# JeffWang987/MVSTER

Hardware: AMD Instinct MI355X
Metric: depth-maps/sec (DTU 512×640, 5-view, 4-stage) at 1/2/4/8 MI355X (higher is better)
Workload: dtype f32; 1 GPU; DTU mid 512x640, 5 views, 4-stage cascade 8/8/4/4 hyp, B=1 eval, 1 depth map(s) per step per GPU; launch=hipGraph replay, parallelism=replicas x1, depth_maps_in_flight_per_gpu=2

## Files before the change

include/mvster_hip.h:

```cpp
#ifndef MVSTER_HIP_H
#define MVSTER_HIP_H

#ifdef __cplusplus
extern "C" {
#endif

#define MVSTER_OK 0
#define MVSTER_ERR_NULL (-1)
#define MVSTER_ERR_SHAPE (-2)
#define MVSTER_ERR_UNSUPPORTED (-3)
#define MVSTER_ERR_LAUNCH (-4)

int mvster_relative_projection(const float* proj_matrices, float* rt, int B, int N, void* stream);

int mvster_relative_projection_multi(const float* const* proj_matrices, int nstage, float* rt, int B, int N,
                                     void* stream);

int mvster_pack_images(const float* const* imgs, int N, float* out, int B, int H, int W, void* stream);

int mvster_pack_images_u8(const unsigned char* imgs, float* out, int V, int H, int W, void* stream);

int mvster_load_pack_images_u8(const unsigned char* buf, long buf_bytes, const int* desc_host, const int* desc, const void* tables,
                               long table_words, float* out, unsigned char* out_u8, int V, int Hd, int Wd, void* stream);

int mvster_forward_prologue(const float* const* imgs, int N, float* packed, int B, int H, int W,
                            const float* const* proj_matrices, int nstage, float* rt, const float* depth_values, int ndv,
                            float* hypo, int D, int h, int w, int inverse, void* stream);

int mvster_warp_agg_fwd(const float* ref_feat, const float* src_feat, const float* rt, const float* hypo,
                        float* out, float* wsum_out, int B, int NV, int C, int G, int D, int h, int w, int Hs,
                        int Ws, long ref_batch_stride, long src_view_stride, long src_batch_stride, int group_cor,
                        int attn_fuse_d, float attn_temp, int variant, void* stream);

int mvster_warp_agg_fwd_indexed(const float* store, const int* views, const float* rt, const float* hypo, float* out,
                                float* wsum_out, int V, int B, int NV, int C, int G, int D, int h, int w, int group_cor,
                                int attn_fuse_d, float attn_temp, int variant, void* stream);

int mvster_warp_agg_fwd_counted(const float* ref_feat, const float* src_feat, const float* rt, const float* hypo,
                                float* out, float* wsum_out, int B, int NV, int C, int G, int D, int h, int w, int Hs,
                                int Ws, long ref_batch_stride, long src_view_stride, long src_batch_stride, int group_cor,
                                int attn_fuse_d, float attn_temp, int variant, const int* nsrc, void* stream);
int mvster_warp_agg_fwd_indexed_counted(const float* store, const int* views, const float* rt, const float* hypo, float* out,
                                        float* wsum_out, int V, int B, int NV, int C, int G, int D, int h, int w,
                                        int group_cor, int attn_fuse_d, float attn_temp, int variant, const int* nsrc,
                                        void* stream);

int mvster_gather_views(const float* store, const int* views, float* out, int V, int B, int N, long map_floats, void* stream);

int mvster_warp_agg_fwd_sched(const float* ref_feat, const float* src_feat, const float* rt, const float* inv_min,
                              const float* inv_max, const float* depth_values, int ndv, float* hypo_out, float* out,
                              float* wsum_out, int B, int NV, int C, int G, int D, int h, int w, int Hs, int Ws,
                              long ref_batch_stride, long src_view_stride, long src_batch_stride, int attn_fuse_d,
                              float attn_temp, int mode, void* stream);

int mvster_warp_agg_bwd(const float* ref_feat, const float* src_feat, const float* rt, const float* hypo,
                        const float* out, const float* wsum, const float* grad_out, float* grad_ref,
                        float* grad_src, float* windows, int* win_org, int B, int NV, int C, int G, int D, int h, int w,
                        int Hs, int Ws, long ref_batch_stride, long src_view_stride, long src_batch_stride, int group_cor,
                        int attn_fuse_d, float attn_temp, void* stream);
int mvster_warp_agg_bwd_scratch(int B, int NV, int C, int G, int D, int h, int w, int attn_fuse_d, long* window_floats,
                                long* origin_ints);

int mvster_warp_agg_bwd_sorted_scratch(int B, int NV, int C, int D, int h, int w, int Hs, int Ws, long* rec_floats, long* ints);
int mvster_warp_agg_bwd_sorted(const float* ref_feat, const float* src_feat, const float* rt, const float* hypo,
                               const float* out, const float* wsum, const float* grad_out, float* grad_ref, float* grad_src,
                               float* rec, int* ints, int B, int NV, int C, int G, int D, int h, int w, int Hs, int Ws,
                               long ref_batch_stride, long src_view_stride, long src_batch_stride, int group_cor,
                               int attn_fuse_d, float attn_temp, void* stream);

int mvster_init_range(const float* depth_values, int ndv, float* out, int B, int D, int h, int w, int inverse,
                      void* stream);

int mvster_schedule_inverse_range(const float* inv_min, const float* inv_max, float* out, int B, int D, int h,
                                  int w, void* stream);

int mvster_schedule_range(const float* cur_depth, const float* interval, float* out, int B, int D, int h, int w,
                          void* stream);

int mvster_select_depth(const float* logits, const float* feat, const float* prob_w, const float* prob_b, int CF,
                        const float* hypo, float* attn, float* depth, float* conf, float* inv_min, float* inv_max,
                        float* logits_out, int B, int D, int h, int w, float split_itv, void* stream);

int mvster_select_depth_bwd(const float* attn, const float* gattn, const float* feat, const float* prob_w, float* dfeat,
                            float* partial, int B, int D, int h, int w, int CF, void* stream);

int mvster_upsample_bilinear(const float* in, float* out, int B, int hi, int wi, int ho, int wo, void* stream);

int mvster_upsample_bilinear_multi(const float* const* ins, float* const* outs, const int* his, const int* wis, int n, int B,
                                   int ho, int wo, void* stream);

int mvster_conv_mfma(const float* in, const float* wpk, const float* scale, const float* shift, const float* skip,
                     const float* zeros, const float* prob_w, const float* prob_b, float* out, const int* geom,
                     int ngeom, const long* woff, int cin, int mt, int nt, int variant, void* stream);

int mvster_conv_small(const float* in, const float* w, const float* scale, const float* shift, const float* skip,
                      float* out, int NB, int H, int W, int cin, int relu, void* stream);

int mvster_conv_narrow(const float* in, const float* w, const float* scale, const float* shift, const float* skip,
                       float* out, int NB, int H, int W, int cin, int relu, int mt, int wpc, void* stream);

int mvster_conv_narrow4(const float* in, const float* w, const float* scale, const float* shift, float* out, int NB, int H,
                        int W, int relu, int mt, int wpc, void* stream);

int mvster_conv_narrow_pair(const float* in, const float* w1, const float* scale1, const float* shift1, const float* w2,
                            const float* scale2, const float* shift2, float* out, int NB, int H, int W, int relu1, int relu2,
                            int wpc, void* stream);

int mvster_deconv_small(const float* in, const float* w, const float* scale, const float* shift, const float* skip,
                        const float* prob_w, const float* prob_b, float* out, int NB, int Hi, int Wi, int cin,
                        int cout, int relu, void* stream);

int mvster_deconv_select(const float* in, const float* w, const float* scale, const float* shift, const float* skip,
                         const float* prob_w, const float* prob_b, const float* hypo, float* attn, float* depth, float* conf,
                         float* inv_min, float* inv_max, float* logits_out, int B, int D, int Hi, int Wi, int cin, int relu,
                         float split_itv, void* stream);

int mvster_fpn_tail_gather(const float* G, const float* vb, float* P, float* workspace, int NB, int H, int W,
                           int CO, void* stream);

int mvster_fpn_tail_gather_bwd(const float* gP, float* gG, int NB, int H, int W, int CO, int pitch, void* stream);

int mvster_fpn_lateral_up(const float* x, const float* A, const float* bias, const float* q, float* out, int NB,
                          int H, int W, int CI, int CO, void* stream);

int mvster_fpn_tail_fused(const float* x, const float* A, const float* bias, const float* q, const float* vb, float* P,
                          int NB, int H, int W, int CI, void* stream);

int mvster_pack_conv_weights(const float* w, float* wpk, int cout, int cin, int cin_pad, int kd, int kh, int kw, long s_n,
                             long s_c, long s_z, long s_y, long s_x, int flip, void* stream);

int mvster_pack_wino_weights(const float* w, float* wpk, int cout, int cin, int cin_pad, int kd, long s_n, long s_c, long s_z,
                             long s_y, long s_x, int flip, void* stream);

int mvster_pack_wino_batch(const void* descs, int ndesc, int total_blocks, void* stream);

int mvster_pack_conv_weights_classes(const float* w, float* wpk, int cout, int cin, int cin_pad, int ktot, int nclass,
                                     const int* ntaps, const long* woff, const int* taps, void* stream);

int mvster_conv_wgrad(const float* x, const float* gy, float* partial, int nblk, int B, int Di, int Hi, int Wi, int CI,
                      int Do, int Ho, int Wo, int CO, int kd, int kh, int kw, int sd, int sh, int sw, int pd, int ph,
                      int pw, int packed, void* stream);

int mvster_conv_wgrad_slots(int CI, int CO, int kd, int kh, int kw, int sd, int sh, int sw, int pd, int ph, int pw, int packed);

int mvster_conv_wgrad_finish(const float* partial, float* dw, int nblk, int ngrp, int cop, int width, int ntaps, int cip,
                             int co_lim, int ci_lim, int swap, int flip, void* stream);

int mvster_conv_wgrad_finish_batch(const void* recs, int count, void* stream);

int mvster_bn_relu_fwd(const float* x, const float* scale, const float* shift, const float* skip, float* y, long rows,
                       int C, int relu, int groups, void* stream);
int mvster_bn_slots(long rows, int C, int groups);
int mvster_bn_relu_bwd_reduce(const float* x, const float* gy, const float* scale, const float* shift, const float* mean,
                              const float* rstd, float* partial, float* sums, float* dgamma, float* dbeta, int* ticket,
                              long rows, int C, int relu, int groups, void* stream);
int mvster_bn_relu_bwd_apply(const float* x, const float* gy, const float* scale, const float* shift, const float* mean,
                             const float* rstd, const float* sums, float* dx, long rows, int C, int relu, int groups,
                             int frozen, void* stream);

int mvster_col_sum(const float* x, float* partial, float* out, int* ticket, long rows, int C, void* stream);

int mvster_bn_train_slots(long rows, int C, int groups);
int mvster_bn_train_fwd(const float* x, const float* weight, const float* bias, float* running_mean, float* running_var,
                        long* num_batches_tracked, const float* skip, float* partial, float* y, float* out, long rows, int C,
                        int relu, int groups, float eps, float momentum, void* stream);
int mvster_bn_train_bwd(const float* x, const float* gy, const float* pack, float* partial, float* dgamma, float* dbeta, float* dx,
                        long rows, int C, int relu, int groups, void* stream);

int mvster_upsample2x_cl_fwd(const float* in, float* out, int B, int h, int w, int C, void* stream);
int mvster_upsample2x_cl_bwd(const float* gout, float* gin, int B, int h, int w, int C, void* stream);
int mvster_upsample2x_nearest_cl(const float* in, float* out, int B, int h, int w, int C, int backward, void* stream);

int mvster_sinkhorn(const float* attn, const float* hypo, const float* gt, float* loss_pix, float* jac, int B, int D,
                    long HW, int iters, float eps, void* stream);
int mvster_sinkhorn_continuous(const float* attn, const float* hypo, const float* gt, const float* mask, float* loss_pix,
                               float* jac, int B, int D, long HW, int iters, float eps, void* stream);

int mvster_stage_loss_terms(const float* hypo, const float* gt, const float* mask, const float* loss_pix,
                            const float* mono, float* terms, int B, int D, long HW, int inverse_depth, void* stream);

int mvster_geo_filter(const float* depth_ref, const float* depth_src, const double* ref_mats, const double* view_mats,
                      int* mask_sum, float* depth_sum, unsigned char* view_mask, float* view_depth, float* x_src,
                      float* y_src, int NS, int H, int W, float pix_thres, float rel_thres, void* stream);


int mvster_geo_scene_blocks(int R, int H, int W);

int mvster_geo_scene_filter(const float* depth, const float* confidence, const int* pairs, const int* ref_view,
                            const double* ref_mats, const double* view_mats, int* mask_sum, double* depth_avg,
                            unsigned char* photo_mask, unsigned char* geo_mask, unsigned char* final_mask, int* wg_counts,
                            long* wg_offsets, int R, int Smax, int V, int H, int W, float conf_thres, int thres_view,
                            float pix_thres, float rel_thres, void* stream);

int mvster_geo_scene_filter_dynamic(const float* depth, const float* confidence, const int* pairs, const int* ref_view,
                                    const double* ref_mats, const double* view_mats, int* mask_sum, double* depth_avg,
                                    unsigned char* photo_mask, unsigned char* geo_mask, unsigned char* final_mask,
                                    unsigned char* geo_level, int* wg_counts, long* wg_offsets, int R, int Smax, int V,
                                    int H, int W, float conf_thres, int thres_view, float pix_base, float rel_base,
                                    void* stream);

int mvster_geo_scene_emit(const double* depth_avg, const unsigned char* final_mask, const int* ref_view,
                          const double* ref_mats, const void* images, int image_kind, const long* wg_offsets, float* points,
                          unsigned char* colors, long M, int R, int V, int H, int W, void* stream);


int mvster_stage_loss_slots(long n);
int mvster_stage_loss_fwd(const float* hypo, const float* gt, const float* mask, const float* loss_pix, const float* mono,
                          const float* total_in, float* planes, float* partial, float* out, int B, int D, long HW,
                          int inverse_depth, float w_l1, float w_ot, float w_stage, void* stream);

int mvster_stage_loss_bwd(const float* jac, const float* planes, const float* out, const float* g_total, const float* g_l1,
                          const float* g_ot, float w_l1, float w_ot, float* g_attn, float* g_mono, int B, int D, long HW,
                          void* stream);

int mvster_mono_depth_fwd(const float* z, const float* dmin, const float* dmax, float* depth, float* sig, int B, long HW,
                          void* stream);
int mvster_mono_depth_bwd(const float* g, const float* depth, const float* sig, const float* dmin, const float* dmax, float* gz,
                          int B, long HW, void* stream);

int mvster_upcat_fwd(const float* a, const float* b, float* out, int NB, int H, int W, int Ca, int Cb, void* stream);
int mvster_upcat_bwd(const float* g, float* ga, float* gb, int NB, int H, int W, int Ca, int Cb, void* stream);

int mvster_fine_weights_fwd(const float* wo, const float* wi, const float* bi, float* wg, float* wc, float* vb, int CO, int CM,
                            int CI, void* stream);
int mvster_fine_weights_bwd(const float* wo, const float* wi, const float* bi, const float* g_wg, const float* g_wc,
                            const float* g_vb, float* g_wo, float* g_wi, float* g_bi, int CO, int CM, int CI, void* stream);

int mvster_fused_adam(const void* const* params, const void* const* grads, const int* sizes, const int* state_offs, int count,
                      float* exp_avg, float* exp_avg_sq, float* step_cells, const float* lr, double beta1, double beta2,
                      double eps, double weight_decay, void* stream);

int mvster_gather_batch(const void* descs, int ndesc, int total_blocks, void* stream);


int mvster_voxel_thin_blocks(long M);

int mvster_voxel_thin_insert(const float* points, long M, float voxel, unsigned long long* keys, int* first, long table_slots,
                             int* slot, int* wg_counts, long* wg_offsets, void* stream);

int mvster_voxel_thin_emit(const float* points, const unsigned char* colors, long M, float voxel, int reduce, int* first,
                           const int* slot, const long* wg_offsets, unsigned long long* sums, float* out_points,
                           unsigned char* out_colors, int* out_counts, long* out_first, long U, void* stream);


int mvster_depth_metrics_slots(long hw);
int mvster_depth_metrics(const float* est, const float* gt, const float* mask, const float* scale, const float* thres, int K,
                         int N, long HW, double* partial, double* raw, float* out, void* stream);

int mvster_pooled_metrics(const float* est, const float* gt, const float* mask, const float* scale, const float* thres, int K,
                          int N, long HW, double* partial, double* raw, float* out, void* stream);

int mvster_scalar_accumulate(const float* row, int n, double* sums, long* count, void* stream);
int mvster_scalar_reset(double* sums, int n, long* count, void* stream);

int mvster_scalar_gather_accumulate(const void* const* ptrs, int n, float* row, double* sums, long* count, void* stream);

const char* mvster_last_kernel(void);

int mvster_build_flags(void);

int mvster_mfma_probe(const float* A, const float* B, float* D, void* stream);

#ifdef __cplusplus
}
#endif
#endif
```

mvster_amd/_lib.py:

```python
import ctypes
import os

_HERE = os.path.dirname(os.path.abspath(__file__))
LIB_PATH = os.environ.get("MVSTER_LIB") or os.path.join(_HERE, "csrc", "libmvster_hip.so")

ERR_NULL, ERR_SHAPE, ERR_UNSUPPORTED, ERR_LAUNCH = -1, -2, -3, -4
ERRORS = {-1: "NULL pointer", -2: "bad shape", -3: "unsupported channel/tile combination", -4: "kernel launch failed"}

_f = ctypes.c_void_p
_i = ctypes.c_int
_l = ctypes.c_long
_fl = ctypes.c_float

SIGNATURES = {
    "mvster_relative_projection": [_f, _f, _i, _i, _f],
    "mvster_relative_projection_multi": [_f, _i, _f, _i, _i, _f],
    "mvster_pack_images": [_f, _i, _f, _i, _i, _i, _f],
    "mvster_pack_images_u8": [_f, _f, _i, _i, _i, _f],
    "mvster_load_pack_images_u8": [_f, _l, _f, _f, _f, _l, _f, _f, _i, _i, _i, _f],
    "mvster_forward_prologue": [_f, _i, _f, _i, _i, _i, _f, _i, _f, _f, _i, _f, _i, _i, _i, _i, _f],
    "mvster_warp_agg_fwd": [_f, _f, _f, _f, _f, _f] + [_i] * 9 + [_l] * 3 + [_i, _i, _fl, _i, _f],
    "mvster_warp_agg_fwd_indexed": [_f, _f, _f, _f, _f, _f] + [_i] * 10 + [_fl, _i, _f],
    "mvster_warp_agg_fwd_counted": [_f, _f, _f, _f, _f, _f] + [_i] * 9 + [_l] * 3 + [_i, _i, _fl, _i, _f, _f],
    "mvster_warp_agg_fwd_indexed_counted": [_f, _f, _f, _f, _f, _f] + [_i] * 10 + [_fl, _i, _f, _f],
    "mvster_gather_views": [_f, _f, _f, _i, _i, _i, _l, _f],
    "mvster_warp_agg_fwd_sched": [_f] * 6 + [_i, _f, _f, _f] + [_i] * 9 + [_l] * 3 + [_i, _fl, _i, _f],
    "mvster_warp_agg_bwd": [_f] * 11 + [_i] * 9 + [_l] * 3 + [_i, _i, _fl, _f],
    "mvster_warp_agg_bwd_scratch": [_i] * 8 + [_f, _f],
    "mvster_warp_agg_bwd_sorted_scratch": [_i] * 8 + [_f, _f],
    "mvster_warp_agg_bwd_sorted": [_f] * 11 + [_i] * 9 + [_l] * 3 + [_i, _i, _fl, _f],
    "mvster_init_range": [_f, _i, _f, _i, _i, _i, _i, _i, _f],
    "mvster_schedule_inverse_range": [_f, _f, _f, _i, _i, _i, _i, _f],
    "mvster_schedule_range": [_f, _f, _f, _i, _i, _i, _i, _f],
    "mvster_select_depth": [_f, _f, _f, _f, _i, _f, _f, _f, _f, _f, _f, _f, _i, _i, _i, _i, _fl, _f],
    "mvster_select_depth_bwd": [_f, _f, _f, _f, _f, _f, _i, _i, _i, _i, _i, _f],
    "mvster_upsample_bilinear": [_f, _f, _i, _i, _i, _i, _i, _f],
    "mvster_upsample_bilinear_multi": [_f, _f, _f, _f, _i, _i, _i, _i, _f],
    "mvster_conv_mfma": [_f, _f, _f, _f, _f, _f, _f, _f, _f, _f, _i, _f, _i, _i, _i, _i, _f],
    "mvster_conv_small": [_f, _f, _f, _f, _f, _f, _i, _i, _i, _i, _i, _f],
    "mvster_conv_narrow": [_f, _f, _f, _f, _f, _f, _i, _i, _i, _i, _i, _i, _i, _f],
    "mvster_conv_narrow4": [_f, _f, _f, _f, _f, _i, _i, _i, _i, _i, _i, _f],
    "mvster_conv_narrow_pair": [_f, _f, _f, _f, _f, _f, _f, _f, _i, _i, _i, _i, _i, _i, _f],
    "mvster_deconv_select": [_f] * 14 + [_i] * 6 + [_fl, _f],
    "mvster_deconv_small": [_f, _f, _f, _f, _f, _f, _f, _f, _i, _i, _i, _i, _i, _i, _f],
    "mvster_fpn_tail_gather": [_f, _f, _f, _f, _i, _i, _i, _i, _f],
    "mvster_fpn_lateral_up": [_f, _f, _f, _f, _f, _i, _i, _i, _i, _i, _f],
    "mvster_fpn_tail_fused": [_f, _f, _f, _f, _f, _f, _i, _i, _i, _i, _f],
    "mvster_fpn_tail_gather_bwd": [_f, _f, _i, _i, _i, _i, _i, _f],
    "mvster_pack_conv_weights": [_f, _f] + [_i] * 6 + [_l] * 5 + [_i, _f],
    "mvster_pack_wino_weights": [_f, _f, _i, _i, _i, _i, _l, _l, _l, _l, _l, _i, _f],
    "mvster_pack_wino_batch": [_f, _i, _i, _f],
    "mvster_pack_conv_weights_classes": [_f, _f, _i, _i, _i, _i, _i, _f, _f, _f, _f],
    "mvster_conv_wgrad": [_f, _f, _f] + [_i] * 20 + [_f],
    "mvster_conv_wgrad_slots": [_i] * 12,
    "mvster_bn_relu_fwd": [_f, _f, _f, _f, _f, _l, _i, _i, _i, _f],
    "mvster_conv_wgrad_finish": [_f, _f] + [_i] * 10 + [_f],
    "mvster_bn_slots": [_l, _i, _i],
    "mvster_col_sum": [_f, _f, _f, _f, _l, _i, _f],
    "mvster_bn_train_slots": [_l, _i, _i],
    "mvster_bn_train_fwd": [_f] * 10 + [_l, _i, _i, _i, _fl, _fl, _f],
    "mvster_bn_train_bwd": [_f] * 7 + [_l, _i, _i, _i, _f],
    "mvster_conv_wgrad_finish_batch": [_f, _i, _f],
    "mvster_bn_relu_bwd_reduce": [_f] * 11 + [_l, _i, _i, _i, _f],
    "mvster_bn_relu_bwd_apply": [_f] * 8 + [_l, _i, _i, _i, _i, _f],
    "mvster_upsample2x_cl_fwd": [_f, _f, _i, _i, _i, _i, _f],
    "mvster_upsample2x_cl_bwd": [_f, _f, _i, _i, _i, _i, _f],
    "mvster_upsample2x_nearest_cl": [_f, _f, _i, _i, _i, _i, _i, _f],
    "mvster_sinkhorn": [_f, _f, _f, _f, _f, _i, _i, _l, _i, _fl, _f],
    "mvster_sinkhorn_continuous": [_f, _f, _f, _f, _f, _f, _i, _i, _l, _i, _fl, _f],
    "mvster_stage_loss_terms": [_f, _f, _f, _f, _f, _f, _i, _i, _l, _i, _f],
    "mvster_stage_loss_slots": [_l],
    "mvster_stage_loss_fwd": [_f] * 9 + [_i, _i, _l, _i, _fl, _fl, _fl, _f],
    "mvster_stage_loss_bwd": [_f] * 6 + [_fl, _fl, _f, _f, _i, _i, _l, _f],
    "mvster_mono_depth_fwd": [_f] * 5 + [_i, _l, _f],
    "mvster_mono_depth_bwd": [_f] * 6 + [_i, _l, _f],
    "mvster_upcat_fwd": [_f, _f, _f, _i, _i, _i, _i, _i, _f],
    "mvster_upcat_bwd": [_f, _f, _f, _i, _i, _i, _i, _i, _f],
    "mvster_fine_weights_fwd": [_f] * 6 + [_i, _i, _i, _f],
    "mvster_fine_weights_bwd": [_f] * 9 + [_i, _i, _i, _f],
    "mvster_fused_adam": [_f, _f, _f, _f, _i, _f, _f, _f, _f] + [ctypes.c_double] * 4 + [_f],
    "mvster_geo_filter": [_f] * 10 + [_i, _i, _i, _fl, _fl, _f],
    "mvster_geo_scene_blocks": [_i, _i, _i],
    "mvster_geo_scene_filter": [_f] * 13 + [_i] * 5 + [_fl, _i, _fl, _fl, _f],
    "mvster_geo_scene_filter_dynamic": [_f] * 14 + [_i] * 5 + [_fl, _i, _fl, _fl, _f],
    "mvster_geo_scene_emit": [_f] * 5 + [_i, _f, _f, _f, _l, _i, _i, _i, _i, _f],
    "mvster_voxel_thin_blocks": [_l],
    "mvster_voxel_thin_insert": [_f, _l, _fl, _f, _f, _l, _f, _f, _f, _f],
    "mvster_voxel_thin_emit": [_f, _f, _l, _fl, _i] + [_f] * 8 + [_l, _f],
    "mvster_depth_metrics_slots": [_l],
    "mvster_depth_metrics": [_f] * 5 + [_i, _i, _l, _f, _f, _f, _f],
    "mvster_pooled_metrics": [_f] * 5 + [_i, _i, _l, _f, _f, _f, _f],
    "mvster_scalar_accumulate": [_f, _i, _f, _f, _f],
    "mvster_scalar_gather_accumulate": [_f, _i, _f, _f, _f, _f],
    "mvster_scalar_reset": [_f, _i, _f, _f],
    "mvster_mfma_probe": [_f, _f, _f, _f],
    "mvster_gather_batch": [_f, _i, _i, _f],
    "mvster_last_kernel": [],
    "mvster_build_flags": [],
}
RESTYPES = {"mvster_last_kernel": ctypes.c_char_p}

_lib = None


def load():
    global _lib
    if _lib is None:
        if not os.path.exists(LIB_PATH):
            raise RuntimeError(
                "mvster_amd: %s not found. Build it with `python -c 'import __graft_entry__ as g; g.build()'` "
                "(hipcc --offload-arch=gfx950). There is no PyTorch fallback for the HIP path." % LIB_PATH)
        lib = ctypes.CDLL(LIB_PATH)
        lax = bool(os.environ.get("MVSTER_LIB")) and bool(os.environ.get("MVSTER_LIB_LAX"))
        for name, argtypes in SIGNATURES.items():
            if lax and not hasattr(lib, name):
                continue
            fn = getattr(lib, name)
            fn.argtypes = argtypes
            fn.restype = RESTYPES.get(name, ctypes.c_int)
        _lib = lib
    return _lib


def check(rc, what):
    if rc != 0:
        raise RuntimeError("%s failed: %s (code %d)" % (what, ERRORS.get(rc, "unknown error"), rc))


def has_probes():
    lib = load()
    return hasattr(lib, "mvster_build_flags") and bool(lib.mvster_build_flags() & 1)


def last_kernel():
    return load().mvster_last_kernel().decode()
```

mvster_amd/conv_plan.py:

```python
import ctypes

import numpy as np
import torch

from . import _lib, ops

GEOM = ("B", "Di", "Hi", "Wi", "Do", "Ho", "Wo", "DoF", "HoF", "WoF", "sd", "sh", "sw", "cout", "ntile_total", "relu",
        "skip_mode", "osd", "osh", "osw", "nclass")
GEOM_CLASS = ("kd", "kh", "kw", "pd", "ph", "pw", "od", "oh", "ow", "nsteps")

SKIP_NONE, SKIP_ADD, SKIP_UPSAMPLE_ADD = 0, 1, 2


def _pack_gemm(wk):
    K, N = wk.shape
    Kp, Np = (K + 15) // 16 * 16, (N + 15) // 16 * 16
    full = wk.new_zeros(Kp, Np)
    full[:K, :N] = wk
    return full.view(Kp // 16, 4, 4, Np // 16, 16).permute(0, 3, 1, 4, 2).contiguous().view(-1), Kp // 16


def fold_bn(bn, cout, device):
    if bn is None:
        return torch.ones(cout, device=device), torch.zeros(cout, device=device)
    scale = bn.weight.detach() / torch.sqrt(bn.running_var.detach() + bn.eps)
    shift = bn.bias.detach() - bn.running_mean.detach() * scale
    return scale.float(), shift.float()


_TUNING = None


def _tuning():
    global _TUNING
    if _TUNING is None:
        import json
        import os
        path = os.environ.get("MVSTER_TUNING") or os.path.join(os.path.dirname(os.path.abspath(__file__)), "tuning_gfx950.json")
        try:
            with open(path) as f:
                _TUNING = json.load(f)
        except (OSError, ValueError):
            _TUNING = {}
    return _TUNING


def layer_signature(layer, B, Di, Hi, Wi, skip_mode):
    return "%s%d-%d_k%dx%dx%d_s%dx%dx%d_%dx%dx%dx%d_sk%d" % (
        "T" if layer.transposed else "C", layer.cin, layer.cout, *layer.kernel, *layer.stride, B, Di, Hi, Wi, skip_mode)


FAMILY_REACH = 2.0
_FAMILIES = None
_SIG = None


def _families():
    global _FAMILIES, _SIG
    if _FAMILIES is None:
        import math
        import re
        _SIG = re.compile(r"^([CT]\d+-\d+_k\dx\dx\d_s\dx\dx\d)_(\d+)x(\d+)x(\d+)x(\d+)_sk([012])$")
        fam = {}
        for sig, val in _tuning().items():
            m = _SIG.match(sig)
            if not m:
                continue
            B, D, H, W = (int(m.group(i)) for i in (2, 3, 4, 5))
            fam.setdefault((m.group(1), int(m.group(6))), []).append((math.log2(B * D * H * W), math.log2(D), math.log2(B), list(val)))
        for lst in fam.values():
            lst.sort(key=lambda e: e[:3])
        _FAMILIES = fam
    return _FAMILIES


def tuned_choice(layer, B, Di, Hi, Wi, skip_mode):
    import math
    sig = layer_signature(layer, B, Di, Hi, Wi, skip_mode)
    hit = _tuning().get(sig)
    if hit:
        return hit, "exact"
    if skip_mode == SKIP_ADD:
        hit = _tuning().get(sig[:-1] + "0")
        if hit:
            return hit, "exact (without skip)"
    lst = _families().get((sig[:sig.index("_", sig.index("_s") + 1)], skip_mode))
    if lst:
        lv, ld, lb = math.log2(max(1, B * Di * Hi * Wi)), math.log2(max(1, Di)), math.log2(max(1, B))
        d, val = min(((abs(e[0] - lv) + abs(e[1] - ld) + 0.25 * abs(e[2] - lb), e[3]) for e in lst), key=lambda t: t[0])
        if d <= FAMILY_REACH:
            return list(val), "family"
    return None, None


FUSE_TAIL = True
FUSE_SELECT = True
LDS_BUDGET = 12 * 256 * 16
FORCE_VARIANT = None
TPERS16_MIN_VOXELS = 40960
FUSE_CONV0 = True
NARROW_PAIR_WPC = 1
NARROW_PAIR_MIN_PIXELS = 512 * 14 * 64
NARROW_MIN_VOXELS = 64 * 256


def _lds_plan(B, Do, Ho, Wo, kernel, stride, ntile_total):
    kd, kh, kw = kernel
    if kw not in (3, 5) or Wo < 24:
        return None
    for mt in (4, 2):
        ty = 2 * mt
        patch = kd * ((ty - 1) * stride[1] + kh) * (31 * stride[2] + kw) * 64
        if patch > LDS_BUDGET or (mt == 4 and Ho < 6):
            continue
        blocks = -(-Wo // 32) * -(-Ho // ty) * Do * B
        nt = max(n for n in (4, 2, 1) if n <= ntile_total and ntile_total % n == 0)
        while nt > 1 and blocks * (ntile_total // nt) < 512:
            nt //= 2
        return mt, nt
    return None


WINO_RING_INSTANCES = {(0, 1, 3), (0, 2, 3), (1, 2, 3), (2, 2, 3), (0, 4, 3), (1, 4, 3), (2, 4, 3),
                       (0, 4, 1), (1, 4, 1), (2, 4, 1), (0, 2, 1), (1, 2, 1), (2, 2, 1), (0, 1, 1), (2, 1, 1)}
WINO_INSTANCES = {(1, 1), (2, 1), (2, 2), (1, 2)}


def _wino_plan(layer, B, Do, Ho, Wo):
    tiles = B * Do * -(-Ho // 8) * -(-Wo // 32)
    kd = layer.kernel[0]
    if kd == 1 and layer.cin in (16, 32):
        nt = 2 if layer.ntile_total % 2 == 0 else 1
        if tiles * (layer.ntile_total // nt) >= 192:
            return 8 | (1 << 8), 2, nt
        return None
    nt = 2 if (layer.ntile_total % 2 == 0 and tiles * (layer.ntile_total // 2) >= 224) else 1
    if (1, layer.cin // 16, kd) not in WINO_RING_INSTANCES:
        nt = 1
    if tiles * (layer.ntile_total // nt) >= 160 and (0 if nt == 1 else 1, layer.cin // 16, kd) in WINO_RING_INSTANCES:
        return 9, 2, nt
    return None


def _tiles(M, ntile_total, nclass):
    best = None
    for nt in (5, 4, 3, 2, 1):
        if nt > ntile_total or ntile_total % nt:
            continue
        for mt in (4, 2, 1):
            waves = -(-M // (16 * mt)) * (ntile_total // nt) * nclass
            if waves >= 2048:
                return mt, nt
            if best is None or waves > best[0]:
                best = (waves, mt, nt)
    return best[1], best[2]


class ConvLayer:

    def __init__(self, weight, transposed, stride, padding, bn=None, bias=None, relu=False, cin_pad=None, prob=None):
        w = weight.detach().float()
        dev = w.device
        if w.dim() == 4:
            w = w.unsqueeze(2)
            stride = (1,) + tuple(stride)
            padding = (0,) + tuple(padding)
        self.transposed = transposed
        self.stride = tuple(stride)
        self.padding = tuple(padding)
        if transposed:
            cin, cout = w.shape[0], w.shape[1]
        else:
            cout, cin = w.shape[0], w.shape[1]
        self.cin = cin_pad or cin
        if self.cin not in (4, 8, 16, 32, 64, 80):
            raise RuntimeError("conv_mfma: unsupported input channel count %d" % self.cin)
        self.cout = cout
        self.relu = relu
        kd, kh, kw = w.shape[2:]
        self.kernel = (kd, kh, kw)
        self._cin_raw = cin
        self.classes, self.woff = self._class_table()
        self.wpk = None
        self.w_small = self.w_small4 = self.w_deconv = self.wpk_wino = self.wpk_b3 = self._b3_src = None
        self._pack(w)
        self.ntile_total = (cout + 15) // 16
        npad = self.ntile_total * 16
        scale, shift = fold_bn(bn, cout, dev)
        if bias is not None:
            shift = shift + bias.detach().float() * scale
        self.scale = torch.zeros(npad, device=dev)
        self.shift = torch.zeros(npad, device=dev)
        self.scale[:cout] = scale
        self.shift[:cout] = shift
        self.zeros = torch.zeros(64, device=dev)
        self._geom_cache = {}
        self.prob = None
        if prob is not None:
            if cout != 8:
                raise RuntimeError("conv_mfma: the fused prob head needs 8 channels")
            self.prob = (prob[0].detach().float().reshape(-1).contiguous().to(dev),
                         prob[1].detach().float().reshape(-1).contiguous().to(dev))
    @staticmethod
    def _axis_classes(k, s, p):
        if s == 1:
            if k != 1 or p != 0:
                raise RuntimeError("conv_mfma: transposed stride-1 axis must have kernel 1")
            return [(0, [0], 0)]
        if (k, s, p) not in ((3, 2, 1), (5, 2, 2)):
            raise RuntimeError("conv_mfma: transposed conv must be k=3, s=2, p=1 or k=5, s=2, p=2")
        out = []
        for phase in range(s):
            taps = sorted(((phase + p - kk) // s, kk) for kk in range(k) if (phase + p - kk) % s == 0)
            out.append((phase, [kk for _, kk in taps], -taps[0][0]))
        return out

    def _class_table(self):
        kd, kh, kw = self.kernel
        if not self.transposed:
            nsteps = (kd * kh * kw * self.cin + 15) // 16
            return [dict(kd=kd, kh=kh, kw=kw, pd=self.padding[0], ph=self.padding[1], pw=self.padding[2], od=0, oh=0,
                         ow=0, nsteps=nsteps, taps=None)], np.zeros(1, dtype=np.int64)
        classes, woff, off = [], [], 0
        npad = (self.cout + 15) // 16 * 16
        for pz, kzs, qz in self._axis_classes(kd, self.stride[0], self.padding[0]):
            for py, kys, qy in self._axis_classes(kh, self.stride[1], self.padding[1]):
                for px, kxs, qx in self._axis_classes(kw, self.stride[2], self.padding[2]):
                    nsteps = (len(kzs) * len(kys) * len(kxs) * self.cin + 15) // 16
                    classes.append(dict(kd=len(kzs), kh=len(kys), kw=len(kxs), pd=qz, ph=qy, pw=qx, od=pz, oh=py,
                                        ow=px, nsteps=nsteps, taps=(kzs, kys, kxs)))
                    woff.append(off)
                    off += nsteps * 16 * npad
        return classes, np.asarray(woff, dtype=np.int64)

    def _pack(self, w):
        dev = w.device
        kd, kh, kw = self.kernel
        cin, cout = self._cin_raw, self.cout
        packed = []
        if not self.transposed:
            wk = w.permute(2, 3, 4, 1, 0)
            if self.cin != cin:
                wk = torch.nn.functional.pad(wk, (0, 0, 0, self.cin - cin))
            packed.append(_pack_gemm(wk.reshape(kd * kh * kw * self.cin, cout))[0])
        else:
            if self.cin != cin:
                w = torch.nn.functional.pad(w, (0, 0, 0, 0, 0, 0, 0, 0, 0, self.cin - cin))
            wf = w.reshape(w.shape[0], w.shape[1], kd * kh * kw)
            for c in self.classes:
                idx = c.get("tap_index")
                if idx is None or idx.device != dev:
                    kzs, kys, kxs = c["taps"]
                    idx = c["tap_index"] = torch.tensor([(z * kh + y) * kw + x for z in kzs for y in kys for x in kxs],
                                                        dtype=torch.long, device=dev)
                sub = wf.index_select(2, idx)
                packed.append(_pack_gemm(sub.permute(2, 0, 1).reshape(-1, cout))[0])
        self.wpk = torch.cat(packed).contiguous()
        self.w_deconv = None
        if (self.transposed and self.kernel == (1, 3, 3) and self.stride == (1, 2, 2) and self.padding == (0, 1, 1)
                and (self.cin, cout) in ((16, 8),)):
            self.w_deconv = w[:, :, 0].permute(2, 3, 0, 1).contiguous().to(dev)
        self.w_small = None
        if (not self.transposed and self.kernel == (1, 3, 3) and self.stride == (1, 1, 1) and self.padding == (0, 1, 1)
                and cout == 8 and self.cin in (4, 8)):
            ws = w[:, :, 0].permute(2, 3, 1, 0)
            if self.cin != cin:
                ws = torch.nn.functional.pad(ws, (0, 0, 0, self.cin - cin))
            self.w_small = ws.contiguous().to(dev)
        self.w_small4 = None
        if (not self.transposed and self.kernel == (1, 3, 3) and self.stride == (1, 1, 1) and self.padding == (0, 1, 1)
                and cout == 4 and self.cin == 8):
            ws = w[:, :, 0].permute(2, 3, 1, 0)
            ws = torch.nn.functional.pad(ws, (0, 4, 0, self.cin - cin))
            self.w_small4 = ws.contiguous().to(dev)
        self._pack_wino(w)
        self._pack_b3(w)

    def b3_eligible(self):
        return (not self.transposed and self.kernel in ((1, 3, 3), (3, 3, 3)) and self.stride == (1, 1, 1)
                and self.padding == (self.kernel[0] // 2, 1, 1) and self.cin in (16, 32, 64) and self.cout in (16, 32, 64))

    def _pack_b3(self, w):
        self.wpk_b3 = None
        self._b3_src = w if (self.b3_eligible() and w.is_cuda) else None

    def wino_eligible(self):
        return (not self.transposed and self.kernel in ((1, 3, 3), (3, 3, 3)) and self.stride == (1, 1, 1)
                and self.padding == (self.kernel[0] // 2, 1, 1) and self.cin in (16, 32, 64) and self.cout % 16 == 0)

    def _pack_wino(self, w, swap=False, flip=False):
        if not self.wino_eligible() or not w.is_cuda:
            self.wpk_wino = None
            return
        if self.wpk_wino is None:
            self.wpk_wino = torch.empty(self.kernel[0] * 16 * self.cin * ((self.cout + 15) // 16) * 16, device=w.device,
                                        dtype=torch.float32)
        st = w.stride()
        s_n, s_c = (st[1], st[0]) if swap else (st[0], st[1])
        rc = _lib.load().mvster_pack_wino_weights(w.data_ptr(), self.wpk_wino.data_ptr(), self.cout, self._cin_raw, self.cin,
                                                  self.kernel[0], s_n, s_c, st[2], st[3], st[4], int(flip), ops._stream())
        _lib.check(rc, "pack_wino_weights")

    def repack_on_device(self, weight, swap=False, flip=False):
        w = weight.detach()
        if w.dim() == 4:
            w = w.unsqueeze(2)
        if w.dtype != torch.float32 or not w.is_cuda:
            raise RuntimeError("repack_on_device: fp32 CUDA parameter expected")
        if self.transposed:
            return self._repack_classes_on_device(w)
        st = w.stride()
        s_n, s_c = (st[1], st[0]) if swap else (st[0], st[1])
        kd, kh, kw = self.kernel
        rc = _lib.load().mvster_pack_conv_weights(w.data_ptr(), self.wpk.data_ptr(), self.cout, self._cin_raw, self.cin, kd,
                                                  kh, kw, s_n, s_c, st[2], st[3], st[4], int(flip),
                                                  ops._stream())
        _lib.check(rc, "pack_conv_weights")
        self.wpk_b3 = self._b3_src = None
        if self.wpk_wino is not None:
            self._pack_wino(w, swap, flip)
        if self.w_small is not None:
            wv = w.transpose(0, 1) if swap else w
            if flip:
                wv = wv.flip(2, 3, 4)
            ws = wv[:, :, 0].permute(2, 3, 1, 0)
            if self.cin != self._cin_raw:
                ws = torch.nn.functional.pad(ws, (0, 0, 0, self.cin - self._cin_raw))
            self.w_small.copy_(ws)
        if getattr(self, "w_small4", None) is not None:
            wv = w.transpose(0, 1) if swap else w
            if flip:
                wv = wv.flip(2, 3, 4)
            self.w_small4[:, :, :self._cin_raw, :4].copy_(wv[:, :, 0].permute(2, 3, 1, 0))

    def _repack_classes_on_device(self, w):
        kd, kh, kw = self.kernel
        if not w.is_contiguous() or tuple(w.shape[:2]) != (self._cin_raw, self.cout):
            raise RuntimeError("repack_on_device: contiguous [cin, cout, kd, kh, kw] weight expected")
        tab = getattr(self, "_class_pack", None)
        if tab is None:
            ntaps = np.zeros(len(self.classes), dtype=np.int32)
            taps = np.zeros((len(self.classes), 27), dtype=np.int32)
            for i, c in enumerate(self.classes):
                kzs, kys, kxs = c["taps"]
                flat = [(z * kh + y) * kw + x for z in kzs for y in kys for x in kxs]
                ntaps[i] = len(flat)
                taps[i, :len(flat)] = flat
            tab = self._class_pack = (ntaps, np.ascontiguousarray(self.woff, dtype=np.int64), taps)
        ntaps, woff, taps = tab
        rc = _lib.load().mvster_pack_conv_weights_classes(
            w.data_ptr(), self.wpk.data_ptr(), self.cout, self._cin_raw, self.cin, kd * kh * kw, len(self.classes),
            ntaps.ctypes.data_as(ctypes.c_void_p), woff.ctypes.data_as(ctypes.c_void_p), taps.ctypes.data_as(ctypes.c_void_p),
            ops._stream())
        _lib.check(rc, "pack_conv_weights_classes")
        if self.w_deconv is not None:
            self.w_deconv.copy_(w[:, :, 0].permute(2, 3, 0, 1))

    def repack(self, weight, bias=None):
        w = weight.detach().float()
        if w.dim() == 4:
            w = w.unsqueeze(2)
        self._pack(w)
        if bias is not None:
            self.shift[:self.cout] = bias.detach().float() * self.scale[:self.cout]

    def out_shape(self, B, Di, Hi, Wi):
        kd, kh, kw = self.kernel
        s, p = self.stride, self.padding
        if self.transposed:
            return (B, Di * s[0], Hi * s[1], Wi * s[2])
        return (B, (Di + 2 * p[0] - kd) // s[0] + 1, (Hi + 2 * p[1] - kh) // s[1] + 1, (Wi + 2 * p[2] - kw) // s[2] + 1)

    def _geom(self, B, Di, Hi, Wi, skip_mode):
        key = (B, Di, Hi, Wi, skip_mode)
        g = self._geom_cache.get(key)
        if g is None:
            _, DoF, HoF, WoF = self.out_shape(B, Di, Hi, Wi)
            s = self.stride
            if self.transposed:
                Do, Ho, Wo = Di, Hi, Wi
                sd = sh = sw = 1
                osd, osh, osw = s
            else:
                Do, Ho, Wo = DoF, HoF, WoF
                sd, sh, sw = s
                osd = osh = osw = 1
            vals = dict(B=B, Di=Di, Hi=Hi, Wi=Wi, Do=Do, Ho=Ho, Wo=Wo, DoF=DoF, HoF=HoF, WoF=WoF, sd=sd, sh=sh, sw=sw,
                        cout=self.cout, ntile_total=self.ntile_total, relu=int(self.relu), skip_mode=skip_mode,
                        osd=osd, osh=osh, osw=osw, nclass=len(self.classes))
            arr = [vals[k] for k in GEOM]
            for c in self.classes:
                arr += [c[k] for k in GEOM_CLASS]
            mt, nt = _tiles(B * Do * Ho * Wo, self.ntile_total, len(self.classes))
            variant = 0
            lds = None
            if not self.transposed and self.cin % 16 == 0 and skip_mode in (SKIP_NONE, SKIP_ADD):
                lds = _lds_plan(B, Do, Ho, Wo, self.kernel, self.stride, self.ntile_total)
            if lds is not None and FORCE_VARIANT != 0:
                variant, (mt, nt) = 1, lds
            if variant == 0 and self.cin >= 16 and FORCE_VARIANT is None:
                tiles16 = -(-(B * Do * Ho * Wo) // 16)
                waves = -(-tiles16 // mt) * (self.ntile_total // nt) * len(self.classes)
                if waves < 1024 and min(c["nsteps"] for c in self.classes) >= 8:
                    variant, mt = 2, 1
                    nt = 1
                    for cand in (4, 2):
                        if self.ntile_total % cand == 0 and tiles16 * (self.ntile_total // cand) * len(self.classes) >= 512:
                            nt = cand
                            break
            if (FORCE_VARIANT is None and self.wpk_wino is not None and self.prob is None
                    and skip_mode in (SKIP_NONE, SKIP_ADD)):
                wv = _wino_plan(self, B, Do, Ho, Wo)
                if wv is not None:
                    variant, mt, nt = wv
            tuned = tuned_choice(self, B, Di, Hi, Wi, skip_mode)[0] if FORCE_VARIANT is None else None
            if tuned and (tuned[0] & 0xff) in (8, 9) and (self.wpk_wino is None or self.prob is not None):
                tuned = None
            if tuned:
                variant, mt, nt = tuned
            if self.w_small is not None and skip_mode in (SKIP_NONE, SKIP_ADD) and FORCE_VARIANT in (None, 3, 10):
                if FORCE_VARIANT is not None:
                    variant, mt, nt = FORCE_VARIANT, 0, 0
                elif tuned and tuned[0] in (3, 10):
                    variant, mt, nt = tuned
                else:
                    variant, mt, nt = (10, 0, 0) if B * Do * Ho * Wo >= NARROW_MIN_VOXELS else (3, 0, 0)
                if variant == 10 and not hasattr(_lib.load(), "mvster_conv_narrow"):
                    variant = 3
            if (getattr(self, "w_small4", None) is not None and skip_mode == SKIP_NONE and FORCE_VARIANT is None
                    and self.prob is None and B * Do * Ho * Wo >= NARROW_MIN_VOXELS and hasattr(_lib.load(), "mvster_conv_narrow4")):
                variant, mt, nt = 10, 0, 0
            if self.w_deconv is not None and skip_mode in (SKIP_NONE, SKIP_ADD) and FORCE_VARIANT in (None, 4):
                variant = 4
                if (FORCE_VARIANT is None and self.prob is None and self.cin == 16 and self.cout == 8
                        and B * Di * Hi * Wi >= TPERS16_MIN_VOXELS):
                    variant, mt, nt = 5, 2, 1
            if (FORCE_VARIANT is None and self.transposed and self.kernel == (1, 5, 5) and self.stride == (1, 2, 2)
                    and self.padding == (0, 2, 2) and self.cin in (16, 32) and self.prob is None
                    and skip_mode in (SKIP_NONE, SKIP_ADD) and B * Di * Hi * Wi >= TPERS16_MIN_VOXELS):
                variant, mt, nt = 5, 2, 1
            g = (np.asarray(arr, dtype=np.int32), mt, nt, (B, DoF, HoF, WoF), variant)
            self._geom_cache[key] = g
        return g

    def __call__(self, x, skip=None, skip_mode=SKIP_NONE, tiles=None):
        B, Di, Hi, Wi, C = x.shape
        if C != self.cin or not x.is_contiguous() or x.dtype != torch.float32 or not x.is_cuda:
            raise RuntimeError("conv_mfma: bad input (shape %s, cin %d)" % (tuple(x.shape), self.cin))
        if skip is None:
            skip_mode = SKIP_NONE
        geom, mt, nt, oshape, variant = self._geom(B, Di, Hi, Wi, skip_mode)
        if tiles is not None:
            mt, nt = tiles[0], tiles[1]
            variant = tiles[2] if len(tiles) > 2 else 0
        if variant == 4:
            if self.w_deconv is None or skip_mode == SKIP_UPSAMPLE_ADD:
                raise RuntimeError("deconv_small: layer not eligible")
            out = torch.empty(oshape + ((self.cout,) if self.prob is None else ()), device=x.device, dtype=torch.float32)
            if skip is not None and tuple(skip.shape) != tuple(oshape + (self.cout,)):
                raise RuntimeError("deconv_small: skip shape %s" % (tuple(skip.shape),))
            rc = _lib.load().mvster_deconv_small(
                x.data_ptr(), self.w_deconv.data_ptr(), self.scale.data_ptr(), self.shift.data_ptr(),
                None if skip is None else skip.data_ptr(),
                None if self.prob is None else self.prob[0].data_ptr(), None if self.prob is None else self.prob[1].data_ptr(),
                out.data_ptr(), B * Di, Hi, Wi, self.cin, self.cout, int(self.relu), ops._stream())
            _lib.check(rc, "deconv_small")
            return out
        if self.prob is not None and variant in (1, 3, 10):
            variant = 0
            mt, nt = _tiles(B * geom[4] * geom[5] * geom[6], self.ntile_total, len(self.classes))
        out = torch.empty(oshape + ((self.cout,) if self.prob is None else ()), device=x.device, dtype=torch.float32)
        if skip is not None:
            if not skip.is_contiguous():
                raise RuntimeError("conv_mfma: skip must be contiguous")
            want = (oshape + (self.cout,)) if skip_mode == SKIP_ADD else (B, 1, oshape[2] // 2, oshape[3] // 2, self.cout)
            if tuple(skip.shape) != tuple(want):
                raise RuntimeError("conv_mfma: skip shape %s, expected %s" % (tuple(skip.shape), tuple(want)))
        if variant == 10 and self.w_small is None and getattr(self, "w_small4", None) is not None:
            if skip is not None:
                raise RuntimeError("conv_narrow4: the four-channel form has no skip path")
            rc = _lib.load().mvster_conv_narrow4(
                x.data_ptr(), self.w_small4.data_ptr(), self.scale.data_ptr(), self.shift.data_ptr(), out.data_ptr(), B * Di, Hi, Wi,
                int(self.relu), mt if mt in (2, 4) else 0, nt & 31, ops._stream())
            _lib.check(rc, "conv_narrow4")
            return out
        if variant == 10:
            if self.w_small is None or skip_mode == SKIP_UPSAMPLE_ADD:
                raise RuntimeError("conv_narrow: layer not eligible")
            rc = _lib.load().mvster_conv_narrow(
                x.data_ptr(), self.w_small.data_ptr(), self.scale.data_ptr(), self.shift.data_ptr(),
                None if skip is None else skip.data_ptr(), out.data_ptr(), B * Di, Hi, Wi, self.cin, int(self.relu),
                mt if mt in (2, 4) else 0, nt & 31, ops._stream())
            _lib.check(rc, "conv_narrow")
            return out
        if variant == 3:
            if self.w_small is None or skip_mode == SKIP_UPSAMPLE_ADD:
                raise RuntimeError("conv_small: layer not eligible")
            rc = _lib.load().mvster_conv_small(
                x.data_ptr(), self.w_small.data_ptr(), self.scale.data_ptr(), self.shift.data_ptr(),
                None if skip is None else skip.data_ptr(), out.data_ptr(), B * Di, Hi, Wi, self.cin, int(self.relu),
                ops._stream())
            _lib.check(rc, "conv_small")
            return out
        wpk = self.wpk
        if (variant & 0xff) in (8, 9):
            if self.wpk_wino is None:
                raise RuntimeError("conv_wino: layer not eligible")
            wpk = self.wpk_wino
        if (variant & 0xff) == 11:
            if self._b3_src is None or skip_mode == SKIP_UPSAMPLE_ADD or self.prob is not None:
                raise RuntimeError("conv_b3: layer not eligible")
            stamp = (self._b3_src._version, self._b3_src.data_ptr())
            if self.wpk_b3 is None or getattr(self, "_b3_stamp", None) != stamp:
                self.wpk_b3 = pack_b3(self._b3_src, self.cin, self.cout, self.kernel[0])
                self._b3_stamp = stamp
            wpk, nt = self.wpk_b3, 1
        rc = _lib.load().mvster_conv_mfma(
            x.data_ptr(), wpk.data_ptr(), self.scale.data_ptr(), self.shift.data_ptr(),
            None if skip is None else skip.data_ptr(), self.zeros.data_ptr(),
            None if self.prob is None else self.prob[0].data_ptr(), None if self.prob is None else self.prob[1].data_ptr(),
            out.data_ptr(), geom.ctypes.data_as(ctypes.c_void_p), int(geom.size), self.woff.ctypes.data_as(ctypes.c_void_p), self.cin,
            mt, nt, variant, ops._stream())
        if rc == _lib.ERR_UNSUPPORTED and tiles is None and variant != 0:
            mt, nt = _tiles(B * geom[4] * geom[5] * geom[6], self.ntile_total, len(self.classes))
            rc = _lib.load().mvster_conv_mfma(
                x.data_ptr(), self.wpk.data_ptr(), self.scale.data_ptr(), self.shift.data_ptr(),
                None if skip is None else skip.data_ptr(), self.zeros.data_ptr(),
                None if self.prob is None else self.prob[0].data_ptr(), None if self.prob is None else self.prob[1].data_ptr(),
                out.data_ptr(), geom.ctypes.data_as(ctypes.c_void_p), int(geom.size), self.woff.ctypes.data_as(ctypes.c_void_p),
                self.cin, mt, nt, 0, ops._stream())
        _lib.check(rc, "conv_mfma")
        return out

    def flops(self, B, Di, Hi, Wi):
        _, Do, Ho, Wo = self.out_shape(B, Di, Hi, Wi)
        kd, kh, kw = self.kernel
        if self.transposed:
            return 2 * B * Di * Hi * Wi * kd * kh * kw * self.cin * self.cout
        return 2 * B * Do * Ho * Wo * kd * kh * kw * self.cin * self.cout


def pack_b3(w, cin, cout, kd):
    if w.shape[1] != cin:
        w = torch.nn.functional.pad(w, (0, 0, 0, 0, 0, 0, 0, cin - w.shape[1]))
    w = w.reshape(cout, cin, kd, 9).float()
    w1 = w.to(torch.bfloat16)
    r = w - w1.float()
    w2 = r.to(torch.bfloat16)
    w3 = (r - w2.float()).to(torch.bfloat16)
    planes = torch.nn.functional.pad(torch.stack([w1, w2, w3]), (0, 1))
    ntw = 1 if cout == 16 else 2
    nsplit = cout // (16 * ntw)
    t = planes.reshape(3, nsplit, ntw, 16, cin // 16, 2, 8, kd, 5, 2).permute(7, 4, 1, 8, 2, 0, 9, 5, 3, 6)
    t = t.reshape(kd, cin // 16, nsplit, 5 * ntw * 3 * 64 * 8)
    return torch.nn.functional.pad(t, (0, 1024 * ntw * 8 - t.shape[-1])).contiguous()


def _cbr3d(m, **kw):
    return ConvLayer(m.conv.weight, False, m.conv.stride, m.conv.padding, bn=m.bn, relu=True, **kw)


def _up3d(seq, prob=None):
    ct, bn = seq[0], seq[1]
    return ConvLayer(ct.weight, True, ct.stride, ct.padding, bn=bn, relu=True, prob=prob)


def fused_conv11_select(L, t, c0, hypo, split_itv, inverse_depth, want_logits=False):
    B, D, hi, wi, _ = t.shape
    dev = t.device
    hypo = hypo.contiguous()
    attn = torch.empty(B, D, 2 * hi, 2 * wi, device=dev, dtype=torch.float32)
    depth = torch.empty(B, 2 * hi, 2 * wi, device=dev, dtype=torch.float32)
    conf = torch.empty_like(depth)
    imin = torch.empty_like(depth) if inverse_depth else None
    imax = torch.empty_like(depth) if inverse_depth else None
    lo = torch.empty_like(attn) if want_logits else None
    rc = _lib.load().mvster_deconv_select(
        t.data_ptr(), L.w_deconv.data_ptr(), L.scale.data_ptr(), L.shift.data_ptr(), c0.data_ptr(),
        L.prob[0].data_ptr(), L.prob[1].data_ptr(), hypo.data_ptr(), attn.data_ptr(), depth.data_ptr(), conf.data_ptr(),
        None if imin is None else imin.data_ptr(), None if imax is None else imax.data_ptr(),
        None if lo is None else lo.data_ptr(), B, D, hi, wi, L.cin, int(L.relu), float(split_itv), ops._stream())
    _lib.check(rc, "deconv_select")
    out = {"attn_weight": attn, "depth": depth, "conf": conf}
    if inverse_depth:
        out["inverse_min_depth"], out["inverse_max_depth"] = imin, imax
    if want_logits:
        out["logits"] = lo
    return out


class Reg2dPlan:

    def __init__(self, m, fuse_prob_into_conv11=True):
        self.conv0, self.conv1, self.conv2 = _cbr3d(m.conv0), _cbr3d(m.conv1), _cbr3d(m.conv2)
        self.conv3, self.conv4 = _cbr3d(m.conv3), _cbr3d(m.conv4)
        self.conv5, self.conv6 = _cbr3d(m.conv5), _cbr3d(m.conv6)
        self.conv7, self.conv9 = _up3d(m.conv7), _up3d(m.conv9)
        self.prob_w = m.prob.weight.detach().float().reshape(-1).contiguous()
        self.prob_b = m.prob.bias.detach().float().reshape(-1).contiguous()
        self.conv11 = _up3d(m.conv11, prob=(self.prob_w, self.prob_b) if fuse_prob_into_conv11 else None)
        self.fused_prob = not fuse_prob_into_conv11

    def layers(self):
        return [self.conv0, self.conv1, self.conv2, self.conv3, self.conv4, self.conv5, self.conv6, self.conv7,
                self.conv9, self.conv11]

    def __call__(self, x):
        c0 = self.conv0(x)
        c2 = self.conv2(self.conv1(c0))
        c4 = self.conv4(self.conv3(c2))
        t = self.conv6(self.conv5(c4))
        t = self.conv7(t, skip=c4, skip_mode=SKIP_ADD)
        t = self.conv9(t, skip=c2, skip_mode=SKIP_ADD)
        return self.conv11(t, skip=c0, skip_mode=SKIP_ADD)

    def select(self, x, hypo, split_itv, inverse_depth, want_logits=False):
        c0 = self.conv0(x)
        c2 = self.conv2(self.conv1(c0))
        c4 = self.conv4(self.conv3(c2))
        t = self.conv6(self.conv5(c4))
        t = self.conv7(t, skip=c4, skip_mode=SKIP_ADD)
        t = self.conv9(t, skip=c2, skip_mode=SKIP_ADD)
        L = self.conv11
        B, D, hi, wi, _ = t.shape
        if (FUSE_SELECT and L.w_deconv is not None and L.prob is not None and L.cin == 16 and FORCE_VARIANT in (None, 4)
                and 2 <= D <= 16 and t.is_contiguous() and c0.is_contiguous()):
            return fused_conv11_select(L, t, c0, hypo, split_itv, inverse_depth, want_logits)
        res = self.conv11(t, skip=c0, skip_mode=SKIP_ADD)
        if self.fused_prob:
            return ops.select_depth(hypo, split_itv, inverse_depth, feat_cl=res, prob_w=self.prob_w, prob_b=self.prob_b,
                                    want_logits=want_logits)
        return ops.select_depth(hypo, split_itv, inverse_depth, logits=res, want_logits=want_logits)

    def flops(self, B, D, h, w):
        tot, shp = 0, None
        dims = {"conv0": (D, h, w), "conv1": (D, h, w), "conv2": (D, h // 2, w // 2), "conv3": (D, h // 2, w // 2),
                "conv4": (D, h // 4, w // 4), "conv5": (D, h // 4, w // 4), "conv6": (D, h // 8, w // 8),
                "conv7": (D, h // 8, w // 8), "conv9": (D, h // 4, w // 4), "conv11": (D, h // 2, w // 2)}
        for k, (d_, h_, w_) in dims.items():
            tot += getattr(self, k).flops(B, d_, h_, w_)
        return tot + 2 * B * D * h * w * 8


class Reg3dPlan:

    def __init__(self, m):
        self.down_size = m.down_size
        self.conv0, self.conv1, self.conv2 = _cbr3d(m.conv0), _cbr3d(m.conv1), _cbr3d(m.conv2)
        if m.down_size >= 2:
            self.conv3, self.conv4 = _cbr3d(m.conv3), _cbr3d(m.conv4)
            self.conv9 = _up3d(m.conv9)
        if m.down_size >= 3:
            self.conv5, self.conv6 = _cbr3d(m.conv5), _cbr3d(m.conv6)
            self.conv7 = _up3d(m.conv7)
        self.conv11 = _up3d(m.conv11)
        self.prob = ConvLayer(m.prob.weight, False, m.prob.stride, m.prob.padding)
        self.fused_prob = False

    def __call__(self, x):
        c0 = self.conv0(x)
        c2 = self.conv2(self.conv1(c0))
        if self.down_size == 3:
            c4 = self.conv4(self.conv3(c2))
            t = self.conv6(self.conv5(c4))
            t = self.conv7(t, skip=c4, skip_mode=SKIP_ADD)
            t = self.conv9(t, skip=c2, skip_mode=SKIP_ADD)
        elif self.down_size == 2:
            t = self.conv4(self.conv3(c2))
            t = self.conv9(t, skip=c2, skip_mode=SKIP_ADD)
        else:
            t = c2
        t = self.conv11(t, skip=c0, skip_mode=SKIP_ADD)
        return self.prob(t).squeeze(-1)


def _cbr2d(m, **kw):
    c = m.conv
    return ConvLayer(c.weight, False, c.stride, c.padding, bn=m.bn, relu=m.relu, **kw)


def _plain2d(c):
    return ConvLayer(c.weight, False, c.stride, c.padding, bias=c.bias)


class FpnPlan:

    def __init__(self, m):
        self.conv0 = [_cbr2d(m.conv0[0], cin_pad=4), _cbr2d(m.conv0[1])]
        self.conv1 = [_cbr2d(l) for l in m.conv1]
        self.conv2 = [_cbr2d(l) for l in m.conv2]
        self.conv3 = [_cbr2d(l) for l in m.conv3]
        self.inner1 = _plain2d(m.inner1)
        self.out1, self.out2 = _plain2d(m.out1), _plain2d(m.out2)
        w2 = m.inner2.weight.detach().double()[:, :, 0, 0]
        b2 = m.inner2.bias.detach().double()
        self.mid_g, self.mid_c, self.mid_vb, _ = self._reassociate(m.out3, w2, b2)
        w3 = m.inner3.weight.detach().double()[:, :, 0, 0]
        b3 = m.inner3.bias.detach().double()
        self.tail_g, self.tail_c, self.tail_vb, wg4 = self._reassociate(m.out4, w3, b3)
        self.tail_a = (wg4 @ w2).float().contiguous()
        self.tail_ab = (wg4 @ b2).float().contiguous()

    @staticmethod
    def _reassociate(out, wi, bi):
        wo = out.weight.detach().double()
        co = wo.shape[0]
        wg = wo.permute(2, 3, 0, 1).reshape(9 * co, wo.shape[1])
        wc = torch.einsum("ocyx,ci->oiyx", wo, wi)
        g = ConvLayer(wg.float().reshape(9 * co, wo.shape[1], 1, 1), False, (1, 1), (0, 0))
        c = ConvLayer(wc.float(), False, (1, 1), (1, 1), bias=out.bias)
        vb = torch.einsum("ocyx,c->yxo", wo, bi).reshape(9, co).float().contiguous()
        return g, c, vb, wg

    @staticmethod
    def _seq(layers, x):
        for l in layers:
            x = l(x)
        return x

    def trunk(self, x):
        c0 = self._conv0(x)
        c1 = self._seq(self.conv1, c0)
        c2 = self._seq(self.conv2, c1)
        c3 = self._seq(self.conv3, c2)
        f1 = self.inner1(c2, skip=c3, skip_mode=SKIP_UPSAMPLE_ADD)
        return c0, c1, c3, f1

    def _conv0(self, x):
        a, b = self.conv0
        N, D, H, W, _ = x.shape
        if (FUSE_CONV0 and FORCE_VARIANT is None and a.w_small is not None and b.w_small is not None and a.cin == 4 and b.cin == 8
                and D == 1 and N * H * W >= NARROW_PAIR_MIN_PIXELS and x.is_cuda and a.w_small.device == x.device and x.is_contiguous() and x.dtype == torch.float32
                and hasattr(_lib.load(), "mvster_conv_narrow_pair")):
            out = torch.empty((N, 1, H, W, 8), device=x.device, dtype=torch.float32)
            rc = _lib.load().mvster_conv_narrow_pair(
                x.data_ptr(), a.w_small.data_ptr(), a.scale.data_ptr(), a.shift.data_ptr(), b.w_small.data_ptr(),
                b.scale.data_ptr(), b.shift.data_ptr(), out.data_ptr(), N, H, W, int(a.relu), int(b.relu), NARROW_PAIR_WPC, ops._stream())
            _lib.check(rc, "conv_narrow_pair")
            return out
        return self._seq(self.conv0, x)

    def coarse(self, c3, f1):
        return self.out1(c3), self.out2(f1)

    def head(self, x):
        c0, c1, c3, f1 = self.trunk(x)
        o1, o2 = self.coarse(c3, f1)
        return c0, c1, f1, o1, o2

    def tail(self, c0, c1, f1):
        return self.tail_mid(c0, c1, f1), self.tail_fine(c0, c1, f1)

    def tail_mid(self, c0, c1, f1):
        H, W = c0.shape[2], c0.shape[3]
        p3 = ops.fpn_tail_gather(self.mid_g(f1), self.mid_vb, H // 2, W // 2)
        return self.mid_c(c1, skip=p3, skip_mode=SKIP_ADD)

    def tail_fine(self, c0, c1, f1):
        H, W = c0.shape[2], c0.shape[3]
        q4 = self.tail_g(f1)
        p4 = ops.fpn_tail_fused(c1, self.tail_a, self.tail_ab, q4, self.tail_vb, H, W) if FUSE_TAIL else None
        if p4 is None:
            p4 = ops.fpn_tail_gather(ops.fpn_lateral_up(c1, self.tail_a, self.tail_ab, q4), self.tail_vb, H, W)
        return self.tail_c(c0, skip=p4, skip_mode=SKIP_ADD)

    def __call__(self, x):
        c0, c1, f1, o1, o2 = self.head(x)
        o3, o4 = self.tail(c0, c1, f1)
        return [o1, o2, o3, o4]
```

mvster_amd/csrc/conv_args.hpp:

```cpp
#pragma once
#include "common.hpp"
#include "conv_taps.h"

namespace mvconv {

typedef float f32x4v __attribute__((ext_vector_type(4)));

constexpr int kMaxTaps = 128;
constexpr int kMaxClasses = 8;

struct ConvArgs {
    const float* in;
    const float* wpk;
    const float* scale;
    const float* shift;
    const float* skip;
    const float* zeros;
    const float* prob_w;
    const float* prob_b;
    float* out;
    int B, Di, Hi, Wi;
    int Do, Ho, Wo;
    int DoF, HoF, WoF;
    int sd, sh, sw;
    int cin;
    int cout;
    int ntile_total;
    int relu;
    int skip_mode;
    int nclass;
    int kd[kMaxClasses], kh[kMaxClasses], kw[kMaxClasses];
    int pd[kMaxClasses], ph[kMaxClasses], pw[kMaxClasses];
    int od[kMaxClasses], oh[kMaxClasses], ow[kMaxClasses];
    int osd, osh, osw;
    int nsteps[kMaxClasses];
    int all_inside[kMaxClasses];
    long woff[kMaxClasses];
    unsigned div_mul[3], div_shr[3];
    unsigned in_bytes;
    mvtaps::TapDivs tapdiv[kMaxClasses];
};

__device__ __forceinline__ unsigned fast_div(unsigned n, unsigned d, unsigned mul, unsigned shr) {
    return d == 1 ? n : (__umulhi(n, mul) >> shr);
}

static inline void find_divisor(unsigned d, unsigned& mul, unsigned& shr) {
    if (d <= 1) { mul = 0; shr = 0; return; }
    int lg = 31 - __builtin_clz(d);
    if (d & (d - 1)) ++lg;
    const int p = 31 + lg;
    mul = (unsigned)(((1ull << p) + d - 1) / d);
    shr = (unsigned)(p - 32);
}

typedef __attribute__((address_space(3))) void lds_void;
typedef unsigned u32x4v __attribute__((ext_vector_type(4)));

struct PersArgs {
    unsigned tiles_x, tiles_y, ntiles;
    unsigned out_bytes;
    int prio;
    unsigned mul[3], shr[3], one[3];
};

struct TilePos { int b, zo, ty0, tx0; };

template <int MT, int KW, int SW, int KD>
struct PersGeom {
    static constexpr int TY = 2 * MT;
    static constexpr int KH = KW;
    static constexpr int PW = 31 * SW + KW;
    static constexpr int PH = (TY - 1) * SW + KH;
    static constexpr int ROWS = KD * PH;
    static constexpr int PWH = (PW + 1) / 2;
    static constexpr int ROWSLOTS = SW == 1 ? PW * 2 : PWH * 4;
    static constexpr int USED = ROWS * ROWSLOTS;
    static constexpr int NBLK = (USED + 63) / 64;
    static constexpr int PLANE = ((NBLK * 64 + 7) & ~7) + 4;
};

static inline bool fill_pers_args(const ConvArgs& a, int TY, PersArgs& p) {
    p.tiles_x = (unsigned)((a.Wo + 31) / 32);
    p.tiles_y = (unsigned)((a.Ho + TY - 1) / TY);
    const long ntiles = (long)p.tiles_x * p.tiles_y * a.Do * a.B;
    const long out_bytes = (long)a.B * a.DoF * a.HoF * a.WoF * a.cout * 4;
    if (ntiles >= (1L << 30) || a.in_bytes >= (1u << 31) || out_bytes >= (1L << 31)) return false;
    p.ntiles = (unsigned)ntiles;
    p.out_bytes = (unsigned)out_bytes;
    p.prio = 0;
    const unsigned divisors[3] = {p.tiles_x, p.tiles_y, (unsigned)a.Do};
    for (int i = 0; i < 3; ++i) {
        find_divisor(divisors[i], p.mul[i], p.shr[i]);
        p.one[i] = divisors[i] == 1 ? ~0u : 0u;
    }
    return true;
}

int num_cus();

static inline bool allow_big_lds(const void* kern, unsigned long& done) {
    int dev = 0;
    if (hipGetDevice(&dev) != hipSuccess) return false;
    if (dev >= 0 && dev < 64 && ((done >> dev) & 1ul)) return true;
    if (hipFuncSetAttribute(kern, hipFuncAttributeMaxDynamicSharedMemorySize, 160 * 1024) != hipSuccess) return false;
    if (dev >= 0 && dev < 64) done |= 1ul << dev;
    return true;
}

int dispatch_pers(const ConvArgs& a, int mt, int nt, int wpc, hipStream_t s);
int dispatch_pp(const ConvArgs& a, int mt, int nt, hipStream_t s);
int dispatch_wino(const ConvArgs& a, int nt, int wpc, bool ring, hipStream_t s);
int dispatch_b3(const ConvArgs& a, int mt, int wpc, hipStream_t s);
int dispatch_1x1(const ConvArgs& a, int mt, int wpc, hipStream_t s);

int dispatch_deconv_select_mfma(const float* in, const float* w, const float* scale, const float* shift, const float* skip,
                                const float* prob_w, const float* prob_b, const float* hypo, float* attn, float* depth,
                                float* conf, float* inv_min, float* inv_max, float* logits_out, int B, int D, int Hi, int Wi,
                                int relu, float split_itv, hipStream_t s);

}
```

mvster_amd/csrc/conv_narrow.hip:

```cpp
#include "conv_args.hpp"

namespace {

using mvconv::f32x4v;
using mvconv::lds_void;
using mvconv::u32x4v;

struct NarrowArgs {
    const float* in;
    const float* w;
    const float* scale;
    const float* shift;
    const float* skip;
    float* out;
    int NB, H, W, relu;
    unsigned in_bytes, out_bytes, ntiles;
    FastDiv tiles_x, tiles_y;
};

template <int CIN, int MT, int R, bool SKIP>
struct NarrowGeom {
    static constexpr int Q = CIN / 4;
    static constexpr int TY = 4 * MT, PH = TY + 2, PW = 34;
    static constexpr int PSLOTS = PH * PW * Q;
    static constexpr int NBLK = (PSLOTS + 63) / 64;
    static constexpr int SBLK = SKIP ? TY : 0;
    static constexpr int NI = NBLK + SBLK;
    static constexpr int NIW = (NI + 3) / 4;
    static constexpr int STAGE = NI * 64;
    static constexpr size_t LDS = (size_t)(R * STAGE + 64) * 16;
};

template <int CIN, int MT, int R, bool SKIP, bool CO4 = false>
__global__ void __launch_bounds__(512) conv_narrow_kernel(NarrowArgs a) {
    static_assert(!(CO4 && SKIP), "the four-channel form has no skip path");
    using G = NarrowGeom<CIN, MT, R, SKIP>;
    constexpr int Q = G::Q, TY = G::TY, PW = G::PW, NBLK = G::NBLK, NI = G::NI, NIW = G::NIW;
    constexpr int NKS = 3 * Q;
    static_assert((R - 2) * NIW <= 63, "vmcnt is a 6-bit counter");
    extern __shared__ __attribute__((aligned(16))) float lds_raw[];
    f32x4v* const lds = reinterpret_cast<f32x4v*>(lds_raw);
    f32x4v* const scratch = lds + R * G::STAGE;

    const int lane = threadIdx.x & 63;
    const int wave8 = __builtin_amdgcn_readfirstlane(threadIdx.x >> 6);
    const int wave = wave8 & 3;
    const bool loader = wave8 >= 4;
    const int lm = lane & 15, lq = lane >> 4;
    const unsigned nwg = gridDim.x;
    unsigned tile = xcd_remap(blockIdx.x, nwg);

    auto decode = [&](unsigned t, int& nb, int& y0, int& x0) {
        unsigned txu, tyu;
        nb = (int)fdivmod(fdivmod(t, a.tiles_x, txu), a.tiles_y, tyu);
        y0 = (int)tyu * TY;
        x0 = (int)txu * 32;
    };

    if (loader) {
        const __amdgpu_buffer_rsrc_t in_rsrc =
            __builtin_amdgcn_make_buffer_rsrc(const_cast<float*>(a.in), (short)0, (int)a.in_bytes, 0x00020000);
        const __amdgpu_buffer_rsrc_t skip_rsrc = __builtin_amdgcn_make_buffer_rsrc(
            const_cast<float*>(SKIP ? a.skip : a.in), (short)0, SKIP ? (int)a.out_bytes : 0, 0x00020000);
        unsigned dbase[NIW];
        int dpos[NIW];
#pragma unroll
        for (int n = 0; n < NIW; ++n) {
            const int i = wave + 4 * n;
            if (i < NBLK) {
                const int s = i * 64 + lane;
                const int quad = s % Q, pp = s / Q;
                const int prow = pp / PW, pl = pp - prow * PW;
                const int px = CIN == 8 ? pl ^ ((pl >> 3) & 1) : pl;
                dpos[n] = px | (prow << 8);
                dbase[n] = s < G::PSLOTS ? (unsigned)(((prow * a.W + px) * CIN + quad * 4) * 4) : 0x80000000u;
            } else {
                const int s = (i - NBLK) * 64 + lane;
                const int row = s >> 6, x = (s >> 1) & 31, quad = s & 1;
                dpos[n] = x | (row << 8);
                dbase[n] = i < NI ? (unsigned)(((row * a.W + x) * 8 + quad * 4) * 4) : 0x80000000u;
            }
        }
        auto dma_tile = [&](unsigned t, int stage, bool live) {
            int nb, y0, x0;
            decode(t, nb, y0, x0);
            const unsigned porigin = (unsigned)((((nb * a.H + y0 - 1) * a.W) + x0 - 1) * (CIN * 4));
            const unsigned sorigin = (unsigned)((((nb * a.H + y0) * a.W) + x0) * 32);
            const unsigned wlim = live ? (unsigned)a.W : 0u;
            f32x4v* const dst0 = lds + stage * G::STAGE;
#pragma unroll
            for (int n = 0; n < NIW; ++n) {
                const int i = wave + 4 * n;
                const bool sk = SKIP && i >= NBLK;
                const int ix = x0 + (dpos[n] & 255) - (sk ? 0 : 1), iy = y0 + (dpos[n] >> 8) - (sk ? 0 : 1);
                const bool ok = (unsigned)iy < (unsigned)a.H && (unsigned)ix < wlim;
                const unsigned off = ok ? dbase[n] + (sk ? sorigin : porigin) : 0x80000000u;
                f32x4v* const dst = i < NI ? dst0 + i * 64 : scratch;
                if (sk) {
                    __builtin_amdgcn_raw_ptr_buffer_load_lds(skip_rsrc, (lds_void*)dst, 16, off, 0, 0, 0);
                } else {
                    __builtin_amdgcn_raw_ptr_buffer_load_lds(in_rsrc, (lds_void*)dst, 16, off, 0, 0, 0);
                }
            }
        };
#pragma unroll
        for (int k = 0; k < R - 1; ++k) {
            const unsigned t = tile + (unsigned)k * nwg;
            dma_tile(t < a.ntiles ? t : 0u, k, t < a.ntiles);
        }
        asm volatile("s_waitcnt vmcnt(%0)" ::"n"((R - 2) * NIW) : "memory");
        __builtin_amdgcn_s_barrier();
        int st = R - 1;
        for (; tile < a.ntiles; tile += nwg) {
            const unsigned t = tile + (unsigned)(R - 1) * nwg;
            dma_tile(t < a.ntiles ? t : 0u, st, t < a.ntiles);
            st = st + 1 == R ? 0 : st + 1;
            asm volatile("s_waitcnt vmcnt(%0)" ::"n"((R - 2) * NIW) : "memory");
            __builtin_amdgcn_s_barrier();
        }
        return;
    }

    f32x4v wfrag[NKS];
    int toff[NKS];
    {
        const int delta = lm >> 3, co = lm & 7;
#pragma unroll
        for (int s = 0; s < NKS; ++s) {
            int ky, kxp, c0;
            if (CIN == 8) {
                const int t = 2 * s + (lq >> 1);
                ky = t >> 2; kxp = t & 3; c0 = (lq & 1) * 4;
                const int pxl = 2 * lm + kxp;
                toff[s] = (ky * PW + (pxl ^ ((pxl >> 3) & 1))) * 2 + (lq & 1);
            } else {
                ky = s; kxp = lq; c0 = 0;
                toff[s] = ky * PW + 2 * lm + kxp;
            }
            const int kx = kxp - delta;
            const bool nz = kx >= 0 && kx <= 2;
#pragma unroll
            for (int j = 0; j < 4; ++j) {
                const float v = a.w[nz ? ((ky * 3 + kx) * CIN + c0 + j) * 8 + co : 0];
                wfrag[s][j] = nz ? v : 0.0f;
            }
        }
    }
    const f32x4v scv = *reinterpret_cast<const f32x4v*>(a.scale + (lq & 1) * 4);
    const f32x4v shv = *reinterpret_cast<const f32x4v*>(a.shift + (lq & 1) * 4);
    const int col = 2 * lm + (lq >> 1);
    const __amdgpu_buffer_rsrc_t out_rsrc = __builtin_amdgcn_make_buffer_rsrc(a.out, (short)0, (int)a.out_bytes, 0x00020000);
    __builtin_amdgcn_s_barrier();
    int st = 0;
    for (; tile < a.ntiles; tile += nwg) {
        int nb, y0, x0;
        decode(tile, nb, y0, x0);
        const f32x4v* const stage = lds + st * G::STAGE;
        st = st + 1 == R ? 0 : st + 1;
        f32x4v acc[MT], skv[MT];
#pragma unroll
        for (int mt = 0; mt < MT; ++mt) {
            acc[mt] = (f32x4v){0.f, 0.f, 0.f, 0.f};
            skv[mt] = SKIP ? stage[NBLK * 64 + (wave * MT + mt) * 64 + 4 * lm + lq] : (f32x4v){0.f, 0.f, 0.f, 0.f};
        }
#pragma unroll
        for (int h = 0; h < MT; h += 2) {
            f32x4v A[2][NKS];
#pragma unroll
            for (int s = 0; s < NKS; ++s)
#pragma unroll
                for (int m = 0; m < 2; ++m) A[m][s] = stage[(wave * MT + h + m) * PW * Q + toff[s]];
            __builtin_amdgcn_sched_barrier(0);
#pragma unroll
            for (int s = 0; s < NKS; ++s)
#pragma unroll
                for (int j = 0; j < 4; ++j) {
#pragma unroll
                    for (int m = 0; m < 2; ++m)
                        acc[h + m] = __builtin_amdgcn_mfma_f32_16x16x4f32(wfrag[s][j], A[m][s][j], acc[h + m], 0, 0, 0);
                    __builtin_amdgcn_sched_barrier(0);
                }
        }
        const unsigned oorigin = (unsigned)((((nb * a.H + y0) * a.W) + x0) * (CO4 ? 16 : 32));
#pragma unroll
        for (int mt = 0; mt < MT; ++mt) {
            const int row = wave * MT + mt;
            f32x4v v = acc[mt];
#pragma unroll
            for (int j = 0; j < 4; ++j) {
                v[j] = fmaf(v[j], scv[j], shv[j]);
                if (a.relu) v[j] = fmaxf(v[j], 0.0f);
                if (SKIP) v[j] += skv[mt][j];
            }
            const bool ok = y0 + row < a.H && x0 + col < a.W && !(CO4 && (lq & 1));
            const unsigned off = ok ? oorigin + (unsigned)(((row * a.W + col) * (CO4 ? 4 : 8) + (lq & 1) * 4) * 4) : 0x80000000u;
            __builtin_amdgcn_raw_buffer_store_b128(__builtin_bit_cast(u32x4v, v), out_rsrc, off, 0, MV_STORE_AUX);
        }
        __builtin_amdgcn_s_waitcnt(0xc07f);
        __builtin_amdgcn_s_barrier();
    }
}

template <int CIN, int MT, int R, bool SKIP, bool CO4 = false>
int launch_narrow(NarrowArgs& a, int wpc, hipStream_t s) {
    using G = NarrowGeom<CIN, MT, R, SKIP>;
    auto kern = conv_narrow_kernel<CIN, MT, R, SKIP, CO4>;
    static unsigned long attr_done = 0;
    if (G::LDS > 64 * 1024 && !mvconv::allow_big_lds(reinterpret_cast<const void*>(kern), attr_done)) return MVSTER_ERR_LAUNCH;
    const int ncu = mvconv::num_cus();
    if (ncu <= 0) return MVSTER_ERR_LAUNCH;
    const unsigned tx = (unsigned)((a.W + 31) / 32), ty = (unsigned)((a.H + G::TY - 1) / G::TY);
    const long ntiles = (long)tx * ty * a.NB;
    if (ntiles >= (1L << 30)) return MVSTER_ERR_SHAPE;
    a.ntiles = (unsigned)ntiles;
    a.tiles_x = mv_fastdiv(tx);
    a.tiles_y = mv_fastdiv(ty);
    const int by_lds = (int)((160 * 1024) / G::LDS);
    int per_cu = wpc > 0 ? wpc : 2;
    if (per_cu > by_lds) per_cu = by_lds;
    if (per_cu > 2) per_cu = 2;
    if (per_cu < 1) per_cu = 1;
    const long gmax = (long)ncu * per_cu;
    const long rounds = (ntiles + gmax - 1) / gmax;
    const long gx = (ntiles + rounds - 1) / rounds;
    if (CO4) {
        MV_NOTE_KERNEL("conv_narrow_kernel<%d, %d, %d, false, true>", CIN, MT, R);
    } else {
        MV_NOTE_KERNEL("conv_narrow_kernel<%d, %d, %d, %s>", CIN, MT, R, SKIP ? "true" : "false");
    }
    hipLaunchKernelGGL(kern, dim3((unsigned)gx), dim3(512), G::LDS, s, a);
    return mv_check_launch();
}


#define PAIR_DBG DBG
struct NarrowPairArgs {
    const float* in;
    const float* w1;
    const float* scale1;
    const float* shift1;
    const float* w2;
    const float* scale2;
    const float* shift2;
    float* out;
    int NB, H, W, relu1, relu2, dbg;
    unsigned in_bytes, out_bytes, ntiles;
    FastDiv tiles_x, tiles_y;
};

struct PairGeom {
    static constexpr int TY = 14, TX = 64;
    static constexpr int MH = TY + 2, MW = TX + 2;
    static constexpr int PH = TY + 4, PW = TX + 4;
    static constexpr int PSLOTS = PH * PW;
    static constexpr int NIW = ((PSLOTS + 63) / 64 + 3) / 4;
    static constexpr int STAGE = NIW * 4 * 64;
    static constexpr int R = 2;
    static constexpr int MID = MH * MW * 2;
    static constexpr size_t LDS = (size_t)(R * STAGE + MID + 8) * 16;
};

template <int DBG>
__global__ void __launch_bounds__(512, 4) conv_narrow_pair_kernel(NarrowPairArgs a) {
    using G = PairGeom;
    constexpr int TY = G::TY, PW = G::PW, MW = G::MW, NIW = G::NIW;
    static_assert(G::MH == 16, "the extra pixel pairs of the mid tile's rows form exactly one 16-row MFMA unit");
    extern __shared__ __attribute__((aligned(16))) float lds_raw[];
    f32x4v* const lds = reinterpret_cast<f32x4v*>(lds_raw);
    f32x4v* const mid = lds + G::R * G::STAGE;

    const int lane = threadIdx.x & 63;
    const int wave8 = __builtin_amdgcn_readfirstlane(threadIdx.x >> 6);
    const int wave = wave8 & 3;
    const bool loader = wave8 >= 4;
    const int lm = lane & 15, lq = lane >> 4;
    const unsigned nwg = gridDim.x;
    unsigned tile = xcd_remap(blockIdx.x, nwg);
    if (PAIR_DBG & 16) tile = a.ntiles;

    auto decode = [&](unsigned t, int& nb, int& y0, int& x0) {
        unsigned txu, tyu;
        nb = (int)fdivmod(fdivmod(t, a.tiles_x, txu), a.tiles_y, tyu);
        y0 = (int)tyu * TY;
        x0 = (int)txu * G::TX;
    };

    if (loader) {
        const __amdgpu_buffer_rsrc_t in_rsrc =
            __builtin_amdgcn_make_buffer_rsrc(const_cast<float*>(a.in), (short)0, (int)a.in_bytes, 0x00020000);
        unsigned dbase[NIW];
        int dpos[NIW];
#pragma unroll
        for (int n = 0; n < NIW; ++n) {
            const int s = (wave + 4 * n) * 64 + lane;
            const int prow = s / PW, pl = s - prow * PW;
            dpos[n] = s < G::PSLOTS ? (pl | (prow << 8)) : -1;
            dbase[n] = (unsigned)((prow * a.W + pl) * 16);
        }
        auto dma_tile = [&](unsigned t, int stage, bool live) {
            int nb, y0, x0;
            decode(t, nb, y0, x0);
            const unsigned porigin = (unsigned)((((nb * a.H + y0 - 2) * a.W) + x0 - 2) * 16);
            const unsigned wlim = live ? (unsigned)a.W : 0u;
            f32x4v* const dst0 = lds + stage * G::STAGE;
#pragma unroll
            for (int n = 0; n < NIW; ++n) {
                const int ix = x0 + (dpos[n] & 255) - 2, iy = y0 + (dpos[n] >> 8) - 2;
                const bool ok = dpos[n] >= 0 && (unsigned)iy < (unsigned)a.H && (unsigned)ix < wlim && !(PAIR_DBG & 8);
                const unsigned off = ok ? dbase[n] + porigin : 0x80000000u;
                f32x4v* const dst = dst0 + (wave + 4 * n) * 64;
                __builtin_amdgcn_raw_ptr_buffer_load_lds(in_rsrc, (lds_void*)dst, 16, off, 0, 0, 0);
            }
        };
        dma_tile(tile < a.ntiles ? tile : 0u, 0, tile < a.ntiles);
        {
            const unsigned t = tile + nwg;
            dma_tile(t < a.ntiles ? t : 0u, 1, t < a.ntiles);
        }
        asm volatile("s_waitcnt vmcnt(%0)" ::"n"(NIW) : "memory");
        int st = 0;
        for (; tile < a.ntiles; tile += nwg) {
            __builtin_amdgcn_s_barrier();
            __builtin_amdgcn_s_barrier();
            const unsigned t = tile + 2u * nwg;
            dma_tile(t < a.ntiles ? t : 0u, st, t < a.ntiles);
            st ^= 1;
            asm volatile("s_waitcnt vmcnt(%0)" ::"n"(NIW) : "memory");
        }
        return;
    }

    const int delta = lm >> 3, co = lm & 7;
    const int half = wave & 1, grp = wave >> 1;
    f32x4v wf1[3];
    const int p1 = 32 * half + 2 * lm + lq;
    const int px1 = lm * PW + 64 + lq;
#pragma unroll
    for (int s = 0; s < 3; ++s) {
        const int kx = lq - delta;
        const bool nz = kx >= 0 && kx <= 2;
#pragma unroll
        for (int j = 0; j < 4; ++j) {
            const float v = a.w1[nz ? ((s * 3 + kx) * 4 + j) * 8 + co : 0];
            wf1[s][j] = nz ? v : 0.0f;
        }
    }
    f32x4v wf2[6];
    int p2[2];
#pragma unroll
    for (int e = 0; e < 2; ++e) {
        const int pxl = 2 * lm + 2 * e + (lq >> 1);
        p2[e] = 64 * half + (pxl ^ ((pxl >> 3) & 1)) * 2 + (lq & 1);
    }
#pragma unroll
    for (int s = 0; s < 6; ++s) {
        const int t = 2 * s + (lq >> 1);
        const int ky = t >> 2, kxp = t & 3, c0 = (lq & 1) * 4;
        const int kx = kxp - delta;
        const bool nz = kx >= 0 && kx <= 2;
#pragma unroll
        for (int j = 0; j < 4; ++j) {
            const float v = a.w2[nz ? ((ky * 3 + kx) * 8 + c0 + j) * 8 + co : 0];
            wf2[s][j] = nz ? v : 0.0f;
        }
    }
    f32x4v* const consts = mid + G::MID;
    if (wave == 0 && lane < 32) {
        const float* const src = lane < 8 ? a.scale1 : lane < 16 ? a.shift1 : lane < 24 ? a.scale2 : a.shift2;
        reinterpret_cast<float*>(consts)[lane] = src[lane & 7];
        __builtin_amdgcn_s_waitcnt(0xc07f);
    }
    const int hi = lq & 1;
    const float floor1 = a.relu1 ? 0.0f : -__builtin_inff(), floor2 = a.relu2 ? 0.0f : -__builtin_inff();
    const int col = 32 * half + 2 * lm + (lq >> 1);
    const int pc = 2 * lm + (lq >> 1);
    const int mcol = 64 * half + (pc ^ ((pc >> 3) & 1)) * 2 + hi;
    const unsigned ocol = (unsigned)((col * 8 + hi * 4) * 4);
    const __amdgpu_buffer_rsrc_t out_rsrc = __builtin_amdgcn_make_buffer_rsrc(a.out, (short)0, (int)a.out_bytes, 0x00020000);
    int st = 0;
    unsigned turn = 0;
    for (; tile < a.ntiles; tile += nwg, ++turn) {
        int nb, y0, x0;
        decode(tile, nb, y0, x0);
        const f32x4v* const stage = lds + st * G::STAGE;
        st ^= 1;
        const bool colok1 = (unsigned)(x0 - 1 + col) < (unsigned)a.W;
        const bool colok2 = x0 + col < a.W;
        __builtin_amdgcn_s_barrier();
        {
            const int R0 = grp * 8;
            const f32x4v* const xs = stage + R0 * PW + p1;
            f32x4v* const ms = mid + R0 * MW * 2 + mcol;
            f32x4v X[4], N[2], pend[2], sc, sh;
#pragma unroll
            for (int i = 0; i < 4; ++i) X[i] = xs[i * PW];
            auto epi1 = [&](int q, int row) {
                if (PAIR_DBG & 32) return;
                if (q == 0) { sc = consts[hi]; sh = consts[2 + hi]; }
                if (q == 2 || q == 4) {
                    f32x4v& v = pend[(q - 2) >> 1];
#pragma unroll
                    for (int j = 0; j < 4; ++j) v[j] = fmaxf(fmaf(v[j], sc[j], sh[j]), floor1);
                }
                if (q == 3 || q == 5) {
                    const int m = (q - 3) >> 1;
                    const bool in_img = colok1 && (unsigned)(y0 - 1 + R0 + row + m) < (unsigned)a.H;
                    ms[(row + m) * MW * 2] = in_img ? pend[m] : (f32x4v){0.f, 0.f, 0.f, 0.f};
                }
            };
#pragma unroll
            for (int k = 0; k < 4; ++k) {
                if (k < 3) {
                    N[0] = xs[(2 * k + 4) * PW];
                    N[1] = xs[(2 * k + 5) * PW];
                }
                f32x4v acc[2];
                acc[0] = acc[1] = (f32x4v){0.f, 0.f, 0.f, 0.f};
                __builtin_amdgcn_sched_barrier(0);
#pragma unroll
                for (int s = 0; s < 3; ++s)
#pragma unroll
                    for (int j = 0; j < 4; ++j) {
                        if (!(PAIR_DBG & 1)) {
                            acc[0] = __builtin_amdgcn_mfma_f32_16x16x4f32(wf1[s][j], X[s][j], acc[0], 0, 0, 0);
                            acc[1] = __builtin_amdgcn_mfma_f32_16x16x4f32(wf1[s][j], X[s + 1][j], acc[1], 0, 0, 0);
                        }
                        if (k > 0) epi1(s * 4 + j, 2 * (k - 1));
                        __builtin_amdgcn_sched_barrier(0);
                    }
                pend[0] = acc[0];
                pend[1] = acc[1];
                X[0] = X[2];
                X[1] = X[3];
                X[2] = N[0];
                X[3] = N[1];
            }
            if (wave == (int)(turn & 3)) {
                f32x4v E[3], acc = (f32x4v){0.f, 0.f, 0.f, 0.f};
#pragma unroll
                for (int s = 0; s < 3; ++s) E[s] = stage[s * PW + px1];
                __builtin_amdgcn_sched_barrier(0);
#pragma unroll
                for (int s = 0; s < 3; ++s)
#pragma unroll
                    for (int j = 0; j < 4; ++j) {
                        if (!(PAIR_DBG & 1)) acc = __builtin_amdgcn_mfma_f32_16x16x4f32(wf1[s][j], E[s][j], acc, 0, 0, 0);
                        epi1(s * 4 + j, 6);
                        __builtin_amdgcn_sched_barrier(0);
                    }
                if (!(PAIR_DBG & 32)) {
#pragma unroll
                    for (int j = 0; j < 4; ++j) acc[j] = fmaxf(fmaf(acc[j], sc[j], sh[j]), floor1);
                    const bool in_img = (unsigned)(y0 - 1 + lm) < (unsigned)a.H && (unsigned)(x0 + 63 + (lq >> 1)) < (unsigned)a.W;
                    mid[lm * MW * 2 + (64 + (lq >> 1)) * 2 + hi] = in_img ? acc : (f32x4v){0.f, 0.f, 0.f, 0.f};
                }
            } else {
#pragma unroll
                for (int q = 0; q < 6; ++q) epi1(q, 6);
            }
        }
        __builtin_amdgcn_s_waitcnt(0xc07f);
        __builtin_amdgcn_s_barrier();
        {
            const int Q0 = grp * 7;
            const f32x4v* const ys = mid + Q0 * MW * 2;
            const unsigned oorigin = (unsigned)((((nb * a.H + y0 + Q0) * a.W) + x0) * 32) + ocol;
            f32x4v Y[4][2], N[2][2], pend[2], sc, sh;
#pragma unroll
            for (int i = 0; i < 4; ++i)
#pragma unroll
                for (int e = 0; e < 2; ++e) Y[i][e] = ys[i * MW * 2 + p2[e]];
            auto epi2 = [&](int q, int row, int nrows) {
                if (PAIR_DBG & 32) return;
                if (q == 0) { sc = consts[4 + hi]; sh = consts[6 + hi]; }
                if (q == 2 || (q == 4 && nrows == 2)) {
                    f32x4v& v = pend[(q - 2) >> 1];
#pragma unroll
                    for (int j = 0; j < 4; ++j) v[j] = fmaxf(fmaf(v[j], sc[j], sh[j]), floor2);
                }
                if (q == 3 || (q == 5 && nrows == 2)) {
                    const int m = (q - 3) >> 1;
                    const bool ok = colok2 && y0 + Q0 + row + m < a.H && !(PAIR_DBG & 4);
                    const unsigned off = ok ? oorigin + (unsigned)((row + m) * a.W * 32) : 0x80000000u;
                    __builtin_amdgcn_raw_buffer_store_b128(__builtin_bit_cast(u32x4v, pend[m]), out_rsrc, off, 0, MV_STORE_AUX);
                }
            };
#pragma unroll
            for (int k = 0; k < 4; ++k) {
                if (k < 2) {
#pragma unroll
                    for (int i = 0; i < 2; ++i)
#pragma unroll
                        for (int e = 0; e < 2; ++e) N[i][e] = ys[(2 * k + 4 + i) * MW * 2 + p2[e]];
                } else if (k == 2) {
#pragma unroll
                    for (int e = 0; e < 2; ++e) N[0][e] = ys[8 * MW * 2 + p2[e]];
                }
                f32x4v acc[2];
                acc[0] = acc[1] = (f32x4v){0.f, 0.f, 0.f, 0.f};
                __builtin_amdgcn_sched_barrier(0);
#pragma unroll
                for (int s = 0; s < 6; ++s)
#pragma unroll
                    for (int j = 0; j < 4; ++j) {
                        if (!(PAIR_DBG & 2)) {
                            acc[0] = __builtin_amdgcn_mfma_f32_16x16x4f32(wf2[s][j], Y[s >> 1][s & 1][j], acc[0], 0, 0, 0);
                            if (k < 3)
                                acc[1] = __builtin_amdgcn_mfma_f32_16x16x4f32(wf2[s][j], Y[(s >> 1) + 1][s & 1][j], acc[1], 0, 0, 0);
                        }
                        if (k > 0) epi2(s * 4 + j, 2 * (k - 1), 2);
                        __builtin_amdgcn_sched_barrier(0);
                    }
                pend[0] = acc[0];
                pend[1] = acc[1];
#pragma unroll
                for (int e = 0; e < 2; ++e) {
                    Y[0][e] = Y[2][e];
                    Y[1][e] = Y[3][e];
                    Y[2][e] = N[0][e];
                    Y[3][e] = N[1][e];
                }
            }
#pragma unroll
            for (int q = 0; q < 4; ++q) epi2(q, 6, 1);
        }
        __builtin_amdgcn_s_waitcnt(0xc07f);
    }
}

int launch_narrow_pair(NarrowPairArgs& a, int wpc, hipStream_t s) {
    using G = PairGeom;
    auto kern = conv_narrow_pair_kernel<0>;
    int slot = 0;
#ifdef MVSTER_PROBES
    switch (a.dbg) {
#define PAIR_CASE(n, m) case m: kern = conv_narrow_pair_kernel<m>; slot = n; break;
        PAIR_CASE(1, 1) PAIR_CASE(2, 2) PAIR_CASE(3, 3) PAIR_CASE(4, 4) PAIR_CASE(5, 8) PAIR_CASE(6, 12) PAIR_CASE(7, 15)
        PAIR_CASE(8, 16) PAIR_CASE(9, 32) PAIR_CASE(10, 35) PAIR_CASE(11, 47) PAIR_CASE(12, 44)
#undef PAIR_CASE
        case 0: break;
        default: return MVSTER_ERR_UNSUPPORTED;
    }
#endif
    static unsigned long attr_done_all[13] = {0};
    unsigned long& attr_done = attr_done_all[slot];
    if (G::LDS > 64 * 1024 && !mvconv::allow_big_lds(reinterpret_cast<const void*>(kern), attr_done)) return MVSTER_ERR_LAUNCH;
    const int ncu = mvconv::num_cus();
    if (ncu <= 0) return MVSTER_ERR_LAUNCH;
    const unsigned tx = (unsigned)((a.W + G::TX - 1) / G::TX), ty = (unsigned)((a.H + G::TY - 1) / G::TY);
    const long ntiles = (long)tx * ty * a.NB;
    if (ntiles >= (1L << 30)) return MVSTER_ERR_SHAPE;
    a.ntiles = (unsigned)ntiles;
    a.tiles_x = mv_fastdiv(tx);
    a.tiles_y = mv_fastdiv(ty);
    const int by_lds = (int)((160 * 1024) / G::LDS);
    int per_cu = wpc > 0 ? wpc : 2;
    if (per_cu > by_lds) per_cu = by_lds;
    if (per_cu > 2) per_cu = 2;
    if (per_cu < 1) per_cu = 1;
    const long gmax = (long)ncu * per_cu;
    const long rounds = (ntiles + gmax - 1) / gmax;
    const long gx = (ntiles + rounds - 1) / rounds;
    MV_NOTE_KERNEL("conv_narrow_pair_kernel");
    hipLaunchKernelGGL(kern, dim3((unsigned)gx), dim3(512), G::LDS, s, a);
    return mv_check_launch();
}

}

extern "C" int mvster_conv_narrow(const float* in, const float* w, const float* scale, const float* shift,
                                  const float* skip, float* out, int NB, int H, int W, int cin, int relu, int mt,
                                  int wpc, void* stream) {
    if (!in || !w || !scale || !shift || !out) return MVSTER_ERR_NULL;
    if (NB <= 0 || H <= 0 || W <= 0) return MVSTER_ERR_SHAPE;
    if (cin != 4 && cin != 8) return MVSTER_ERR_UNSUPPORTED;
    const long in_bytes = (long)NB * H * W * cin * 4, out_bytes = (long)NB * H * W * 32;
    if (in_bytes >= (1L << 31) || out_bytes >= (1L << 31)) return MVSTER_ERR_SHAPE;
    NarrowArgs a;
    a.in = in; a.w = w; a.scale = scale; a.shift = shift; a.skip = skip; a.out = out;
    a.NB = NB; a.H = H; a.W = W; a.relu = relu;
    a.in_bytes = (unsigned)in_bytes; a.out_bytes = (unsigned)out_bytes;
    if (mt == 0) mt = (long)NB * H * W >= (1L << 20) ? 4 : 2;
    hipStream_t s = (hipStream_t)stream;
    if (cin == 8) {
        if (mt == 2) return skip ? launch_narrow<8, 2, 4, true>(a, wpc, s) : launch_narrow<8, 2, 4, false>(a, wpc, s);
        if (mt == 4) return skip ? launch_narrow<8, 4, 3, true>(a, wpc, s) : launch_narrow<8, 4, 3, false>(a, wpc, s);
    } else {
        if (mt == 2) return skip ? launch_narrow<4, 2, 4, true>(a, wpc, s) : launch_narrow<4, 2, 4, false>(a, wpc, s);
        if (mt == 4) return skip ? launch_narrow<4, 4, 4, true>(a, wpc, s) : launch_narrow<4, 4, 4, false>(a, wpc, s);
    }
    return MVSTER_ERR_UNSUPPORTED;
}

extern "C" int mvster_conv_narrow4(const float* in, const float* w, const float* scale, const float* shift, float* out, int NB,
                                   int H, int W, int relu, int mt, int wpc, void* stream) {
    if (!in || !w || !scale || !shift || !out) return MVSTER_ERR_NULL;
    if (NB <= 0 || H <= 0 || W <= 0) return MVSTER_ERR_SHAPE;
    const long in_bytes = (long)NB * H * W * 32, out_bytes = (long)NB * H * W * 16;
    if (in_bytes >= (1L << 31)) return MVSTER_ERR_SHAPE;
    NarrowArgs a;
    a.in = in; a.w = w; a.scale = scale; a.shift = shift; a.skip = nullptr; a.out = out;
    a.NB = NB; a.H = H; a.W = W; a.relu = relu;
    a.in_bytes = (unsigned)in_bytes; a.out_bytes = (unsigned)out_bytes;
    if (mt == 0) mt = (long)NB * H * W >= (1L << 20) ? 4 : 2;
    hipStream_t s = (hipStream_t)stream;
    if (mt == 2) return launch_narrow<8, 2, 4, false, true>(a, wpc, s);
    if (mt == 4) return launch_narrow<8, 4, 3, false, true>(a, wpc, s);
    return MVSTER_ERR_UNSUPPORTED;
}

extern "C" int mvster_conv_narrow_pair(const float* in, const float* w1, const float* scale1, const float* shift1,
                                       const float* w2, const float* scale2, const float* shift2, float* out, int NB, int H,
                                       int W, int relu1, int relu2, int wpc, void* stream) {
    if (!in || !w1 || !scale1 || !shift1 || !w2 || !scale2 || !shift2 || !out) return MVSTER_ERR_NULL;
    if (NB <= 0 || H <= 0 || W <= 0) return MVSTER_ERR_SHAPE;
    const long in_bytes = (long)NB * H * W * 16, out_bytes = (long)NB * H * W * 32;
    if (out_bytes >= (1L << 31)) return MVSTER_ERR_SHAPE;
    NarrowPairArgs a;
    a.in = in; a.w1 = w1; a.scale1 = scale1; a.shift1 = shift1; a.w2 = w2; a.scale2 = scale2; a.shift2 = shift2; a.out = out;
    a.NB = NB; a.H = H; a.W = W; a.relu1 = relu1; a.relu2 = relu2;
    a.in_bytes = (unsigned)in_bytes; a.out_bytes = (unsigned)out_bytes;
    a.dbg = wpc >> 4;
    return launch_narrow_pair(a, wpc & 15, (hipStream_t)stream);
}
```

mvster_amd/csrc/conv_small.hip:

```cpp
#include "conv_args.hpp"

namespace {

typedef float f32x4v __attribute__((ext_vector_type(4)));
typedef float f32x2v __attribute__((ext_vector_type(2)));

struct SmallArgs {
    const float* in;
    const float* w;
    const float* scale;
    const float* shift;
    const float* skip;
    float* out;
    int NB, H, W, relu;
    unsigned in_bytes;
};

template <int CIN>
__global__ void __launch_bounds__(256) conv_small_kernel(SmallArgs a, FastDiv tiles_x, FastDiv tiles_y) {
    constexpr int TY = 8, TX = 32, PH = TY + 2, PW = TX + 2, Q = CIN / 4;
    __shared__ f32x4v patch[PH * PW * Q];
    unsigned txu, tyu;
    const int nb = (int)fdivmod(fdivmod(xcd_remap(blockIdx.x, gridDim.x), tiles_x, txu), tiles_y, tyu);
    const int y0 = (int)tyu * TY, x0 = (int)txu * TX;
    const int tx = threadIdx.x & 31, ty = threadIdx.x >> 5;

    const __amdgpu_buffer_rsrc_t rsrc =
        __builtin_amdgcn_make_buffer_rsrc(const_cast<float*>(a.in), (short)0, (int)a.in_bytes, 0x00020000);
    constexpr int NST = (PH * PW * Q + 255) / 256;
    f32x4v tmp[NST];
#pragma unroll
    for (int i = 0; i < NST; ++i) {
        const int idx = threadIdx.x + i * 256;
        const int q = idx % Q, pix = idx / Q;
        const int px = pix % PW, py = pix / PW;
        const int iy = y0 - 1 + py, ix = x0 - 1 + px;
        const bool ok = idx < PH * PW * Q && (unsigned)iy < (unsigned)a.H && (unsigned)ix < (unsigned)a.W;
        const unsigned off = ok ? (unsigned)(((nb * a.H + iy) * a.W + ix) * CIN + q * 4) * 4u : 0xFFFFFFF0u;
        tmp[i] = __builtin_bit_cast(f32x4v, __builtin_amdgcn_raw_buffer_load_b128(rsrc, off, 0, 0));
    }
#pragma unroll
    for (int i = 0; i < NST; ++i) {
        const int idx = threadIdx.x + i * 256;
        if (idx < PH * PW * Q) patch[(idx % Q) * (PH * PW) + idx / Q] = tmp[i];
    }
    __syncthreads();

    f32x2v acc[4];
#pragma unroll
    for (int j = 0; j < 4; ++j) acc[j] = (f32x2v){0.f, 0.f};
    const f32x2v* w2 = reinterpret_cast<const f32x2v*>(a.w);
#pragma unroll
    for (int ky = 0; ky < 3; ++ky)
#pragma unroll
        for (int kx = 0; kx < 3; ++kx) {
            const f32x4v* p = patch + (ty + ky) * PW + tx + kx;
#pragma unroll
            for (int q = 0; q < Q; ++q) {
                const f32x4v xv = p[q * (PH * PW)];
#pragma unroll
                for (int c = 0; c < 4; ++c) {
                    const int ci = q * 4 + c;
                    const f32x2v xx = {xv[c], xv[c]};
                    const f32x2v* wr = w2 + ((ky * 3 + kx) * CIN + ci) * 4;
#pragma unroll
                    for (int j = 0; j < 4; ++j) acc[j] = __builtin_elementwise_fma(xx, wr[j], acc[j]);
                }
            }
        }

    const int y = y0 + ty, x = x0 + tx;
    if (y >= a.H || x >= a.W) return;
    const long o = (((long)nb * a.H + y) * a.W + x) * 8;
    float v[8];
#pragma unroll
    for (int j = 0; j < 4; ++j) { v[2 * j] = acc[j][0]; v[2 * j + 1] = acc[j][1]; }
#pragma unroll
    for (int c = 0; c < 8; ++c) {
        v[c] = fmaf(v[c], a.scale[c], a.shift[c]);
        if (a.relu) v[c] = fmaxf(v[c], 0.0f);
    }
    if (a.skip) {
        const f32x4v s0 = ld4(a.skip + o), s1 = ld4(a.skip + o + 4);
#pragma unroll
        for (int c = 0; c < 4; ++c) { v[c] += s0[c]; v[4 + c] += s1[c]; }
    }
    st4(a.out + o, (f32x4v){v[0], v[1], v[2], v[3]});
    st4(a.out + o + 4, (f32x4v){v[4], v[5], v[6], v[7]});
}

}

extern "C" int mvster_conv_small(const float* in, const float* w, const float* scale, const float* shift,
                                 const float* skip, float* out, int NB, int H, int W, int cin, int relu,
                                 void* stream) {
    if (!in || !w || !scale || !shift || !out) return MVSTER_ERR_NULL;
    if (NB <= 0 || H <= 0 || W <= 0) return MVSTER_ERR_SHAPE;
    const long in_elems = (long)NB * H * W * cin;
    if (in_elems >= (1L << 30)) return MVSTER_ERR_SHAPE;
    SmallArgs a;
    a.in = in; a.w = w; a.scale = scale; a.shift = shift; a.skip = skip; a.out = out;
    a.NB = NB; a.H = H; a.W = W; a.relu = relu; a.in_bytes = (unsigned)(in_elems * 4);
    const int tiles_x = (W + 31) / 32, tiles_y = (H + 7) / 8;
    const long blocks = (long)tiles_x * tiles_y * NB;
    if (blocks >= (1L << 31)) return MVSTER_ERR_SHAPE;
    dim3 grid((unsigned)blocks), block(256);
    if (cin == 8) {
        MV_NOTE_KERNEL("conv_small_kernel<8>");
        hipLaunchKernelGGL(conv_small_kernel<8>, grid, block, 0, (hipStream_t)stream, a, mv_fastdiv(tiles_x), mv_fastdiv(tiles_y));
    } else if (cin == 4) {
        MV_NOTE_KERNEL("conv_small_kernel<4>");
        hipLaunchKernelGGL(conv_small_kernel<4>, grid, block, 0, (hipStream_t)stream, a, mv_fastdiv(tiles_x), mv_fastdiv(tiles_y));
    } else {
        return MVSTER_ERR_UNSUPPORTED;
    }
    return mv_check_launch();
}

namespace {

struct DeconvArgs {
    const float* in;
    const float* w;
    const float* scale;
    const float* shift;
    const float* skip;
    const float* prob_w;
    const float* prob_b;
    float* out;
    int NB, Hi, Wi, relu;
    unsigned in_bytes;
};

template <int CIN, int COUT>
__device__ __forceinline__ void deconv_voxel(const DeconvArgs& a, int nb, int i, int j, float (&v)[4][COUT]) {
    const __amdgpu_buffer_rsrc_t rsrc =
        __builtin_amdgcn_make_buffer_rsrc(const_cast<float*>(a.in), (short)0, (int)a.in_bytes, 0x00020000);
    const unsigned base = (unsigned)((nb * a.Hi + i) * a.Wi + j) * CIN * 4u;
    const bool jn = j + 1 < a.Wi, in_ = i + 1 < a.Hi;
    const unsigned o01 = jn ? base + CIN * 4u : 0xFFFFFFF0u;
    const unsigned o10 = in_ ? base + (unsigned)a.Wi * CIN * 4u : 0xFFFFFFF0u;
    const unsigned o11 = (jn && in_) ? base + (unsigned)(a.Wi + 1) * CIN * 4u : 0xFFFFFFF0u;

    f32x2v acc[4][COUT / 2];
#pragma unroll
    for (int q = 0; q < 4; ++q)
#pragma unroll
        for (int c = 0; c < COUT / 2; ++c) acc[q][c] = (f32x2v){0.f, 0.f};

    const f32x2v* w2 = reinterpret_cast<const f32x2v*>(a.w);
    auto wrow = [&](int ky, int kx, int ci) { return w2 + ((ky * 3 + kx) * CIN + ci) * (COUT / 2); };
    auto load4 = [&](int c4, f32x4v (&x)[4]) {
        const unsigned c4b = (unsigned)c4 * 4u;
        x[0] = __builtin_bit_cast(f32x4v, __builtin_amdgcn_raw_buffer_load_b128(rsrc, base + c4b, 0, 0));
        x[1] = __builtin_bit_cast(f32x4v, __builtin_amdgcn_raw_buffer_load_b128(rsrc, o01 == 0xFFFFFFF0u ? o01 : o01 + c4b, 0, 0));
        x[2] = __builtin_bit_cast(f32x4v, __builtin_amdgcn_raw_buffer_load_b128(rsrc, o10 == 0xFFFFFFF0u ? o10 : o10 + c4b, 0, 0));
        x[3] = __builtin_bit_cast(f32x4v, __builtin_amdgcn_raw_buffer_load_b128(rsrc, o11 == 0xFFFFFFF0u ? o11 : o11 + c4b, 0, 0));
    };
    f32x4v xn[4];
    load4(0, xn);
#pragma unroll 1
    for (int c4 = 0; c4 < CIN; c4 += 4) {
        const f32x4v x00 = xn[0], x01 = xn[1], x10 = xn[2], x11 = xn[3];
        load4(c4 + 4 < CIN ? c4 + 4 : c4, xn);
#pragma unroll
        for (int k = 0; k < 4; ++k) {
            const int ci = c4 + k;
            const f32x2v a00 = {x00[k], x00[k]}, a01 = {x01[k], x01[k]}, a10 = {x10[k], x10[k]}, a11 = {x11[k], x11[k]};
#pragma unroll
            for (int co = 0; co < COUT / 2; ++co) {
                acc[0][co] = __builtin_elementwise_fma(a00, wrow(1, 1, ci)[co], acc[0][co]);
                acc[1][co] = __builtin_elementwise_fma(a00, wrow(1, 2, ci)[co], acc[1][co]);
                acc[1][co] = __builtin_elementwise_fma(a01, wrow(1, 0, ci)[co], acc[1][co]);
                acc[2][co] = __builtin_elementwise_fma(a00, wrow(2, 1, ci)[co], acc[2][co]);
                acc[2][co] = __builtin_elementwise_fma(a10, wrow(0, 1, ci)[co], acc[2][co]);
                acc[3][co] = __builtin_elementwise_fma(a00, wrow(2, 2, ci)[co], acc[3][co]);
                acc[3][co] = __builtin_elementwise_fma(a01, wrow(2, 0, ci)[co], acc[3][co]);
                acc[3][co] = __builtin_elementwise_fma(a10, wrow(0, 2, ci)[co], acc[3][co]);
                acc[3][co] = __builtin_elementwise_fma(a11, wrow(0, 0, ci)[co], acc[3][co]);
            }
        }
    }
    const int Ho = 2 * a.Hi, Wo = 2 * a.Wi;
#pragma unroll
    for (int q = 0; q < 4; ++q) {
        const int oy = 2 * i + (q >> 1), ox = 2 * j + (q & 1);
        const long opix = ((long)nb * Ho + oy) * Wo + ox;
#pragma unroll
        for (int c = 0; c < COUT; ++c) {
            v[q][c] = fmaf(acc[q][c >> 1][c & 1], a.scale[c], a.shift[c]);
            if (a.relu) v[q][c] = fmaxf(v[q][c], 0.0f);
        }
        if (a.skip) {
#pragma unroll
            for (int c = 0; c < COUT; c += 4) {
                const f32x4v s4 = ld4(a.skip + opix * COUT + c);
#pragma unroll
                for (int k = 0; k < 4; ++k) v[q][c + k] += s4[k];
            }
        }
    }
}

__device__ __forceinline__ float prob_logit(const float (&v)[8], const float* prob_w, const float* prob_b) {
    float lo = v[0] * prob_w[0], hi = v[4] * prob_w[4];
#pragma unroll
    for (int k = 1; k < 4; ++k) { lo = fmaf(v[k], prob_w[k], lo); hi = fmaf(v[4 + k], prob_w[4 + k], hi); }
    return (lo + hi) + prob_b[0];
}

template <int CIN, int COUT>
__global__ void __launch_bounds__(256) deconv_small_kernel(DeconvArgs a) {
    const int pix = xcd_remap(blockIdx.x, gridDim.x) * 256 + threadIdx.x;
    const int nb = blockIdx.y;
    if (pix >= a.Hi * a.Wi) return;
    const int i = pix / a.Wi, j = pix - i * a.Wi;
    float v[4][COUT];
    deconv_voxel<CIN, COUT>(a, nb, i, j, v);
    const int Ho = 2 * a.Hi, Wo = 2 * a.Wi;
#pragma unroll
    for (int q = 0; q < 4; ++q) {
        const int oy = 2 * i + (q >> 1), ox = 2 * j + (q & 1);
        const long opix = ((long)nb * Ho + oy) * Wo + ox;
        if constexpr (COUT == 8) {
            if (a.prob_w) {
                a.out[opix] = prob_logit(v[q], a.prob_w, a.prob_b);
                continue;
            }
        }
#pragma unroll
        for (int c = 0; c < COUT; c += 4) st4(a.out + opix * COUT + c, (f32x4v){v[q][c], v[q][c + 1], v[q][c + 2], v[q][c + 3]});
    }
}

struct SelectOut {
    const float* hypo;
    float *attn, *depth, *conf, *inv_min, *inv_max, *logits_out;
    int D;
    float split_itv;
};

template <int CIN>
__global__ void __launch_bounds__(1024) deconv_select_kernel(DeconvArgs a, SelectOut so) {
    __shared__ float lg[mv::kSelMaxD][4][64];
    const int px = threadIdx.x, d = threadIdx.y;
    const int pix = xcd_remap(blockIdx.x, gridDim.x) * 64 + px;
    const int b = blockIdx.y;
    const bool inside = pix < a.Hi * a.Wi;
    const int pc = inside ? pix : a.Hi * a.Wi - 1;
    const int i = pc / a.Wi, j = pc - i * a.Wi;
    {
        float v[4][8];
        deconv_voxel<CIN, 8>(a, b * so.D + d, i, j, v);
#pragma unroll
        for (int q = 0; q < 4; ++q) lg[d][q][px] = prob_logit(v[q], a.prob_w, a.prob_b);
    }
    __syncthreads();
    if (!inside) return;
    const int Ho = 2 * a.Hi, Wo = 2 * a.Wi;
    const long hw = (long)Ho * Wo;
    auto finish = [&](int q) {
        const long p = (long)(2 * i + (q >> 1)) * Wo + (2 * j + (q & 1));
        float l[mv::kSelMaxD];
#pragma unroll
        for (int dd = 0; dd < mv::kSelMaxD; ++dd) {
            if (dd >= so.D) break;
            l[dd] = lg[dd][q][px];
            if (so.logits_out) so.logits_out[((long)b * so.D + dd) * hw + p] = l[dd];
        }
        const long vol = (long)b * so.D * hw, img = (long)b * hw;
        mv::select_from_logits(l, so.hypo + vol, so.attn + vol, so.depth + img, so.conf ? so.conf + img : nullptr,
                               so.inv_min ? so.inv_min + img : nullptr, so.inv_max ? so.inv_max + img : nullptr, so.D, hw, p,
                               so.split_itv);
    };
    if (d < 4) finish(d);
    if (d + so.D < 4) finish(d + so.D);
}

}

extern "C" int mvster_deconv_small(const float* in, const float* w, const float* scale, const float* shift,
                                   const float* skip, const float* prob_w, const float* prob_b, float* out, int NB,
                                   int Hi, int Wi, int cin, int cout, int relu, void* stream) {
    if (!in || !w || !scale || !shift || !out) return MVSTER_ERR_NULL;
    if ((prob_w == nullptr) != (prob_b == nullptr)) return MVSTER_ERR_NULL;
    if (NB <= 0 || Hi <= 0 || Wi <= 0) return MVSTER_ERR_SHAPE;
    if (prob_w && cout != 8) return MVSTER_ERR_UNSUPPORTED;
    const long in_elems = (long)NB * Hi * Wi * cin;
    if (in_elems >= (1L << 30) || (long)NB * Hi * Wi * 4 * cout >= (1L << 31)) return MVSTER_ERR_SHAPE;
    DeconvArgs a;
    a.in = in; a.w = w; a.scale = scale; a.shift = shift; a.skip = skip; a.prob_w = prob_w; a.prob_b = prob_b;
    a.out = out; a.NB = NB; a.Hi = Hi; a.Wi = Wi; a.relu = relu; a.in_bytes = (unsigned)(in_elems * 4);
    dim3 grid((Hi * Wi + 255) / 256, NB), block(256);
    hipStream_t s = (hipStream_t)stream;
    if (cin == 16 && cout == 8) {
        MV_NOTE_KERNEL("deconv_small_kernel<16, 8>");
        hipLaunchKernelGGL((deconv_small_kernel<16, 8>), grid, block, 0, s, a);
    } else if (cin == 32 && cout == 16) {
        MV_NOTE_KERNEL("deconv_small_kernel<32, 16>");
        hipLaunchKernelGGL((deconv_small_kernel<32, 16>), grid, block, 0, s, a);
    } else {
        return MVSTER_ERR_UNSUPPORTED;
    }
    return mv_check_launch();
}

extern "C" int mvster_deconv_select(const float* in, const float* w, const float* scale, const float* shift, const float* skip,
                                    const float* prob_w, const float* prob_b, const float* hypo, float* attn, float* depth,
                                    float* conf, float* inv_min, float* inv_max, float* logits_out, int B, int D, int Hi,
                                    int Wi, int cin, int relu, float split_itv, void* stream) {
    if (!in || !w || !scale || !shift || !prob_w || !prob_b || !hypo || !attn || !depth) return MVSTER_ERR_NULL;
    if ((inv_min == nullptr) != (inv_max == nullptr)) return MVSTER_ERR_NULL;
    if (B <= 0 || D < 2 || D > mv::kSelMaxD || Hi <= 0 || Wi <= 0 || (inv_min && D < 3)) return MVSTER_ERR_SHAPE;
    if (cin != 16) return MVSTER_ERR_UNSUPPORTED;
    const long in_elems = (long)B * D * Hi * Wi * cin;
    if (in_elems >= (1L << 30) || (long)B * D * Hi * Wi * 4 * 8 >= (1L << 31)) return MVSTER_ERR_SHAPE;
    {
        const int rc = mvconv::dispatch_deconv_select_mfma(in, w, scale, shift, skip, prob_w, prob_b, hypo, attn, depth, conf, inv_min,
                                                           inv_max, logits_out, B, D, Hi, Wi, relu, split_itv, (hipStream_t)stream);
        if (rc != MVSTER_ERR_UNSUPPORTED) return rc;
    }
    DeconvArgs a;
    a.in = in; a.w = w; a.scale = scale; a.shift = shift; a.skip = skip; a.prob_w = prob_w; a.prob_b = prob_b;
    a.out = nullptr; a.NB = B * D; a.Hi = Hi; a.Wi = Wi; a.relu = relu; a.in_bytes = (unsigned)(in_elems * 4);
    SelectOut so;
    so.hypo = hypo; so.attn = attn; so.depth = depth; so.conf = conf; so.inv_min = inv_min; so.inv_max = inv_max;
    so.logits_out = logits_out; so.D = D; so.split_itv = split_itv;
    MV_NOTE_KERNEL("deconv_select_kernel<16>");
    hipLaunchKernelGGL(deconv_select_kernel<16>, dim3((Hi * Wi + 63) / 64, B), dim3(64, D), 0, (hipStream_t)stream, a, so);
    return mv_check_launch();
}
```

mvster_amd/csrc/deconv_select.hip:

```cpp
#include "conv_args.hpp"

namespace {

using mvconv::f32x4v;
using mvconv::lds_void;
using mvconv::u32x4v;

struct DselArgs {
    const float *in, *w, *scale, *shift, *skip, *prob_w, *prob_b, *hypo;
    float *attn, *depth, *conf, *inv_min, *inv_max, *logits_out;
    int B, Hi, Wi, relu;
    float split_itv;
    unsigned in_bytes, skip_bytes, ntiles;
    FastDiv tiles_x, tiles_y;
};

template <int D, int RI, int R>
struct DselGeom {
    static constexpr int PSL = (RI + 1) * 17 * 4;
    static constexpr int PSLOTS = D * PSL;
    static constexpr int NBLK = (PSLOTS + 63) / 64;
    static constexpr int SBLK = D * 2 * RI;
    static constexpr int NI = NBLK + SBLK;
    static constexpr int NIW = (NI + 3) / 4;
    static constexpr int STAGE = NI * 64;
    static constexpr int LG = D * 2 * RI * 32;
    static constexpr size_t LDS = (size_t)(R * STAGE + 64) * 16 + (size_t)2 * LG * 4;
};

template <int D, int RI, int R>
__global__ void __launch_bounds__(512) deconv_select_mfma_kernel(DselArgs a) {
    using G = DselGeom<D, RI, R>;
    constexpr int NBLK = G::NBLK, NI = G::NI, NIW = G::NIW, PSL = G::PSL;
    constexpr int SPW = D / 4;
    static_assert(D % 4 == 0 && D <= mv::kSelMaxD && RI <= 4 && (R - 2) * NIW <= 63, "");
    extern __shared__ __attribute__((aligned(16))) float lds_raw[];
    f32x4v* const lds = reinterpret_cast<f32x4v*>(lds_raw);
    f32x4v* const scratch = lds + R * G::STAGE;
    float* const lgbuf = lds_raw + (size_t)(R * G::STAGE + 64) * 4;

    const int lane = threadIdx.x & 63;
    const int wave8 = __builtin_amdgcn_readfirstlane(threadIdx.x >> 6);
    const int wave = wave8 & 3;
    const bool loader = wave8 >= 4;
    const int lm = lane & 15, lq = lane >> 4;
    const int Ho = 2 * a.Hi, Wo = 2 * a.Wi;
    const unsigned nwg = gridDim.x;
    unsigned tile = xcd_remap(blockIdx.x, nwg);

    auto decode = [&](unsigned t, int& b, int& i0, int& j0) {
        unsigned txu, tyu;
        b = (int)fdivmod(fdivmod(t, a.tiles_x, txu), a.tiles_y, tyu);
        i0 = (int)tyu * RI;
        j0 = (int)txu * 16;
    };

    if (loader) {
        const __amdgpu_buffer_rsrc_t in_rsrc =
            __builtin_amdgcn_make_buffer_rsrc(const_cast<float*>(a.in), (short)0, (int)a.in_bytes, 0x00020000);
        const __amdgpu_buffer_rsrc_t skip_rsrc = __builtin_amdgcn_make_buffer_rsrc(
            const_cast<float*>(a.skip ? a.skip : a.in), (short)0, a.skip ? (int)a.skip_bytes : 0, 0x00020000);
        unsigned dbase[NIW];
        int dpos[NIW];
#pragma unroll
        for (int n = 0; n < NIW; ++n) {
            const int i = wave + 4 * n;
            if (i < NBLK) {
                const int s = i * 64 + lane;
                const int d = s / PSL, r1 = s - d * PSL;
                const int prow = r1 / 68, r2 = r1 - prow * 68;
                const int v = r2 >> 2, quad = (r2 & 3) ^ ((v >> 2) & 3);
                dpos[n] = v | (prow << 8);
                dbase[n] = s < G::PSLOTS ? (unsigned)((((d * a.Hi + prow) * a.Wi + v) * 16 + quad * 4) * 4) : 0x80000000u;
            } else {
                const int s = (i - NBLK) * 64 + lane;
                const int rowall = s >> 6, d = rowall / (2 * RI), orow = rowall - d * 2 * RI;
                const int ox = (s >> 1) & 31, half = s & 1;
                dpos[n] = ox | (orow << 8);
                dbase[n] = i < NI ? (unsigned)((((d * Ho + orow) * Wo + ox) * 8 + half * 4) * 4) : 0x80000000u;
            }
        }
        auto dma_tile = [&](unsigned t, int stage, bool live) {
            int b, i0, j0;
            decode(t, b, i0, j0);
            const unsigned porigin = (unsigned)((((b * D * a.Hi + i0) * a.Wi) + j0) * 64);
            const unsigned sorigin = (unsigned)((((b * D * Ho + 2 * i0) * Wo) + 2 * j0) * 32);
            const unsigned wlim = live ? (unsigned)a.Wi : 0u;
            f32x4v* const dst0 = lds + stage * G::STAGE;
#pragma unroll
            for (int n = 0; n < NIW; ++n) {
                const int i = wave + 4 * n;
                const bool sk = i >= NBLK;
                const int cx = dpos[n] & 255, cy = dpos[n] >> 8;
                const bool ok = sk ? (2 * i0 + cy < Ho && (unsigned)(2 * j0 + cx) < 2 * wlim) : (i0 + cy < a.Hi && (unsigned)(j0 + cx) < wlim);
                const unsigned off = ok ? dbase[n] + (sk ? sorigin : porigin) : 0x80000000u;
                f32x4v* const dst = i < NI ? dst0 + i * 64 : scratch;
                if (sk) {
                    __builtin_amdgcn_raw_ptr_buffer_load_lds(skip_rsrc, (lds_void*)dst, 16, off, 0, 0, 0);
                } else {
                    __builtin_amdgcn_raw_ptr_buffer_load_lds(in_rsrc, (lds_void*)dst, 16, off, 0, 0, 0);
                }
            }
        };
#pragma unroll
        for (int k = 0; k < R - 1; ++k) {
            const unsigned t = tile + (unsigned)k * nwg;
            dma_tile(t < a.ntiles ? t : 0u, k, t < a.ntiles);
        }
        asm volatile("s_waitcnt vmcnt(%0)" ::"n"((R - 2) * NIW) : "memory");
        __builtin_amdgcn_s_barrier();
        int st = R - 1;
        for (; tile < a.ntiles; tile += nwg) {
            const unsigned t = tile + (unsigned)(R - 1) * nwg;
            dma_tile(t < a.ntiles ? t : 0u, st, t < a.ntiles);
            st = st + 1 == R ? 0 : st + 1;
            asm volatile("s_waitcnt vmcnt(%0)" ::"n"((R - 2) * NIW) : "memory");
            __builtin_amdgcn_s_barrier();
        }
        return;
    }

    f32x4v wf[2][4];
    {
        const int dx = lm >> 3, co = lm & 7, di = lq >> 1, dj = lq & 1;
#pragma unroll
        for (int dy = 0; dy < 2; ++dy) {
            const int ky = dy + 1 - 2 * di, kx = dx + 1 - 2 * dj;
            const bool nz = ky >= 0 && ky <= 2 && kx >= 0 && kx <= 2;
#pragma unroll
            for (int s = 0; s < 4; ++s)
#pragma unroll
                for (int j = 0; j < 4; ++j) {
                    const float v = a.w[nz ? ((ky * 3 + kx) * 16 + 4 * s + j) * 8 + co : 0];
                    wf[dy][s][j] = nz ? v : 0.0f;
                }
        }
    }
    const int c0 = (lq & 1) * 4;
    const f32x4v scv = *reinterpret_cast<const f32x4v*>(a.scale + c0), shv = *reinterpret_cast<const f32x4v*>(a.shift + c0);
    const f32x4v pwv = *reinterpret_cast<const f32x4v*>(a.prob_w + c0);
    const float pb = a.prob_b[0];
    const int vpos = lm + (lq & 1);
    const int abase = ((lq >> 1) * 17 + vpos) * 4, aswz = (vpos >> 2) & 3;
    const int tsel = wave * 64 + lane, sy = tsel >> 5, sx = tsel & 31;
    const long hw = (long)Ho * Wo;
    const bool has_skip = a.skip != nullptr;

    __builtin_amdgcn_s_barrier();
    int st = 0, it = 0;
    for (; tile < a.ntiles; tile += nwg, ++it) {
        int b, i0, j0;
        decode(tile, b, i0, j0);
        const f32x4v* const stage = lds + st * G::STAGE;
        st = st + 1 == R ? 0 : st + 1;
        float* const lg = lgbuf + (it & 1) * G::LG;
        const int oy = 2 * i0 + sy, ox = 2 * j0 + sx;
        const bool sel = tsel < 64 * RI && oy < Ho && ox < Wo;
        const long p = (long)oy * Wo + ox, vol = (long)b * D * hw;
        float hv[mv::kSelMaxD];
#pragma unroll
        for (int d = 0; d < D; ++d) hv[d] = sel ? a.hypo[vol + d * hw + p] : 1.0f;

#pragma unroll
        for (int sl = 0; sl < SPW; ++sl) {
            const int d = wave + 4 * sl;
            const f32x4v* const patch = stage + d * PSL;
#pragma unroll
            for (int r = 0; r < RI; ++r) {
                f32x4v X[4];
#pragma unroll
                for (int s = 0; s < 4; ++s) X[s] = patch[r * 68 + abase + (s ^ aswz)];
                f32x4v sk[2];
#pragma unroll
                for (int dy = 0; dy < 2; ++dy)
                    sk[dy] = has_skip ? stage[NBLK * 64 + (d * 2 * RI + 2 * r + dy) * 64 + 4 * lm + lq] : (f32x4v){0.f, 0.f, 0.f, 0.f};
                f32x4v acc[2] = {(f32x4v){0.f, 0.f, 0.f, 0.f}, (f32x4v){0.f, 0.f, 0.f, 0.f}};
#pragma unroll
                for (int s = 0; s < 4; ++s)
#pragma unroll
                    for (int j = 0; j < 4; ++j)
#pragma unroll
                        for (int dy = 0; dy < 2; ++dy)
                            acc[dy] = __builtin_amdgcn_mfma_f32_16x16x4f32(wf[dy][s][j], X[s][j], acc[dy], 0, 0, 0);
#pragma unroll
                for (int dy = 0; dy < 2; ++dy) {
                    float v[4];
#pragma unroll
                    for (int k = 0; k < 4; ++k) {
                        v[k] = fmaf(acc[dy][k], scv[k], shv[k]);
                        if (a.relu) v[k] = fmaxf(v[k], 0.0f);
                        if (has_skip) v[k] += sk[dy][k];
                    }
                    float part = v[0] * pwv[0];
#pragma unroll
                    for (int k = 1; k < 4; ++k) part = fmaf(v[k], pwv[k], part);
                    const float other = __shfl_xor(part, 16);
                    const float logit = ((lq & 1) ? other + part : part + other) + pb;
                    if (!(lq & 1)) lg[(d * 2 * RI + 2 * r + dy) * 32 + 2 * lm + (lq >> 1)] = logit;
                }
            }
        }
        __builtin_amdgcn_s_waitcnt(0xc07f);
        __builtin_amdgcn_s_barrier();
        if (sel) {
            float l[mv::kSelMaxD];
#pragma unroll
            for (int d = 0; d < D; ++d) {
                l[d] = lg[(d * 2 * RI + sy) * 32 + sx];
                if (a.logits_out) a.logits_out[vol + d * hw + p] = l[d];
            }
            const long img = (long)b * hw;
            mv::select_from_logits_vals(l, hv, a.attn + vol, a.depth + img, a.conf ? a.conf + img : nullptr,
                                        a.inv_min ? a.inv_min + img : nullptr, a.inv_max ? a.inv_max + img : nullptr, D, hw, p,
                                        a.split_itv);
        }
    }
}

template <int D, int RI, int R>
int launch_dsel(DselArgs& a, hipStream_t s) {
    using G = DselGeom<D, RI, R>;
    auto kern = deconv_select_mfma_kernel<D, RI, R>;
    static unsigned long attr_done = 0;
    if (G::LDS > 160 * 1024) return MVSTER_ERR_UNSUPPORTED;
    if (G::LDS > 64 * 1024 && !mvconv::allow_big_lds(reinterpret_cast<const void*>(kern), attr_done)) return MVSTER_ERR_LAUNCH;
    const int ncu = mvconv::num_cus();
    if (ncu <= 0) return MVSTER_ERR_LAUNCH;
    const unsigned tx = (unsigned)((a.Wi + 15) / 16), ty = (unsigned)((a.Hi + RI - 1) / RI);
    const long ntiles = (long)tx * ty * a.B;
    if (ntiles >= (1L << 30)) return MVSTER_ERR_SHAPE;
    a.ntiles = (unsigned)ntiles;
    a.tiles_x = mv_fastdiv(tx);
    a.tiles_y = mv_fastdiv(ty);
    int per_cu = (int)((160 * 1024) / G::LDS);
    if (per_cu > 2) per_cu = 2;
    const long gmax = (long)ncu * per_cu;
    const long rounds = (ntiles + gmax - 1) / gmax;
    const long gx = (ntiles + rounds - 1) / rounds;
    MV_NOTE_KERNEL("deconv_select_mfma_kernel<%d, %d, %d>", D, RI, R);
    hipLaunchKernelGGL(kern, dim3((unsigned)gx), dim3(512), G::LDS, s, a);
    return mv_check_launch();
}

}

namespace mvconv {

int dispatch_deconv_select_mfma(const float* in, const float* w, const float* scale, const float* shift, const float* skip,
                                const float* prob_w, const float* prob_b, const float* hypo, float* attn, float* depth,
                                float* conf, float* inv_min, float* inv_max, float* logits_out, int B, int D, int Hi, int Wi,
                                int relu, float split_itv, hipStream_t s) {
    const long in_bytes = (long)B * D * Hi * Wi * 64, skip_bytes = (long)B * D * Hi * Wi * 4 * 32;
    if (in_bytes >= (1L << 31) || skip_bytes >= (1L << 31)) return MVSTER_ERR_UNSUPPORTED;
    DselArgs a;
    a.in = in; a.w = w; a.scale = scale; a.shift = shift; a.skip = skip; a.prob_w = prob_w; a.prob_b = prob_b; a.hypo = hypo;
    a.attn = attn; a.depth = depth; a.conf = conf; a.inv_min = inv_min; a.inv_max = inv_max; a.logits_out = logits_out;
    a.B = B; a.Hi = Hi; a.Wi = Wi; a.relu = relu; a.split_itv = split_itv;
    a.in_bytes = (unsigned)in_bytes; a.skip_bytes = (unsigned)skip_bytes;
    const int ncu = num_cus();
    if (D == 4) {
        const long t4 = (long)((Wi + 15) / 16) * ((Hi + 3) / 4) * B;
        return t4 >= 2L * ncu ? launch_dsel<4, 2, 2>(a, s) : launch_dsel<4, 2, 3>(a, s);
    }
    if (D == 8) {
        const long t2 = (long)((Wi + 15) / 16) * ((Hi + 1) / 2) * B;
        return t2 >= ncu ? launch_dsel<8, 2, 2>(a, s) : launch_dsel<8, 1, 2>(a, s);
    }
    return MVSTER_ERR_UNSUPPORTED;
}

}
```

mvster_amd/net.py:

```python
import contextlib

import torch
import torch.nn as nn
import torch.nn.functional as F

from . import ops
from .conv_plan import FpnPlan, Reg2dPlan, Reg3dPlan
from .modules import FPN4, mono_depth_decoder, reg2d, reg3d


class _WarpAggPyr(torch.autograd.Function):

    @staticmethod
    def forward(ctx, pyr, B, rt, hypo, G, group_cor, attn_fuse_d, attn_temp):
        pyr = pyr.contiguous()
        ref_cl, src_cl = _WarpAggPyr._parts(pyr, B)
        out, wsum = ops.warp_agg_fwd_cl(ref_cl, src_cl, rt, hypo, G, group_cor, attn_fuse_d, attn_temp, want_wsum=True)
        ctx.save_for_backward(pyr, rt, hypo, out, wsum)
        ctx.cfg = (B, G, group_cor, attn_fuse_d, attn_temp)
        ctx.set_materialize_grads(False)
        return out, pyr[:B]

    @staticmethod
    def _parts(pyr, B):
        n, _, h, w, C = pyr.shape
        return pyr[:B].view(B, h, w, C), pyr[B:].view(n // B - 1, B, h, w, C)

    @staticmethod
    def backward(ctx, grad, grad_ref_maps):
        pyr, rt, hypo, out, wsum = ctx.saved_tensors
        B, G, group_cor, attn_fuse_d, attn_temp = ctx.cfg
        if pyr.is_cuda:
            pyr.record_stream(torch.cuda.current_stream(pyr.device))
        if grad is None:
            g_pyr = torch.zeros_like(pyr)
        else:
            g_pyr = torch.empty_like(pyr)
            g_ref, g_src = _WarpAggPyr._parts(g_pyr, B)
            ref_cl, src_cl = _WarpAggPyr._parts(pyr, B)
            n_src, _, hs, ws, c_ = src_cl.shape
            if not (ops.SORTED_SCATTER and ops.warp_agg_bwd_sorted_scratch(B, n_src, c_, hypo.shape[1], hypo.shape[2],
                                                                           hypo.shape[3], hs, ws) is not None):
                g_src.zero_()
            ops.warp_agg_bwd_cl(ref_cl, src_cl, rt, hypo, out, wsum, grad.contiguous(), G, group_cor, attn_fuse_d,
                                attn_temp, into=(g_ref, g_src))
        if grad_ref_maps is not None:
            g_pyr[:B].add_(grad_ref_maps)
        return g_pyr, None, None, None, None, None, None, None


class _SelectDepthCL(torch.autograd.Function):

    @staticmethod
    def forward(ctx, feat_cl, prob_w, prob_b, hypo, split_itv, inverse_depth):
        feat_cl = feat_cl.contiguous()
        w = prob_w.detach().reshape(-1).contiguous()
        sel = ops.select_depth(hypo, split_itv, inverse_depth, feat_cl=feat_cl, prob_w=w, prob_b=prob_b.detach().reshape(-1))
        ctx.save_for_backward(sel["attn_weight"], feat_cl, w)
        ctx.shapes = (prob_w.shape, prob_b.shape)
        ctx.set_materialize_grads(False)
        outs = (sel["attn_weight"], sel["depth"]) + ((sel["inverse_min_depth"], sel["inverse_max_depth"]) if inverse_depth else ())
        ctx.mark_non_differentiable(*outs[1:])
        return outs

    @staticmethod
    def backward(ctx, gattn, *unused):
        if gattn is None:
            return (None,) * 6
        attn, feat_cl, w = ctx.saved_tensors
        dfeat, dw, db = ops.select_depth_bwd(attn, gattn, feat_cl, w)
        return dfeat, dw.reshape(ctx.shapes[0]), db.reshape(ctx.shapes[1]), None, None, None


def _invalidate_after_load(module, incompatible):
    module.invalidate_plans()


class MVS4net(nn.Module):
    MAX_HYPOTHESES = 64
    MAX_HYPOTHESES_TRAIN = 16
    _stream_warning_off = False

    def __init__(self, arch_mode="fpn", reg_net="reg2d", num_stage=4, fpn_base_channel=8, reg_channel=8,
                 stage_splits=[8, 8, 4, 4], depth_interals_ratio=[0.5, 0.5, 0.5, 1], group_cor=False,
                 group_cor_dim=[8, 8, 8, 8], inverse_depth=False, agg_type="ConvBnReLU3D", dcn=False, pos_enc=0,
                 mono=False, asff=False, attn_temp=2, attn_fuse_d=True, vis_ETA=False, vis_mono=False):
        super().__init__()
        if arch_mode != "fpn":
            raise NotImplementedError("arch_mode %r (only 'fpn' exists in the reference too)" % arch_mode)
        if dcn or asff or pos_enc or vis_ETA or vis_mono:
            raise NotImplementedError("dcn / asff / pos_enc / vis_* ablation switches are out of scope "
                                      "(SURVEY.md section 2, #10): not enabled by the shipped scripts")
        lo = 3 if inverse_depth else 2
        if max(stage_splits) > self.MAX_HYPOTHESES or min(stage_splits) < lo:
            raise NotImplementedError("stage_splits %r: the kernels take %d..%d depth hypotheses per stage in evaluation "
                                      "(3..%d in training; the shipped cascade uses 8/8/4/4)"
                                      % (stage_splits, lo, self.MAX_HYPOTHESES, self.MAX_HYPOTHESES_TRAIN))
        if not group_cor:
            for s_, d_ in enumerate(stage_splits[:num_stage]):
                if d_ > 8 and fpn_base_channel * 2 ** (3 - s_) >= 32:
                    raise NotImplementedError("stage_splits %r with group_cor=False: stages with 32 or more feature channels "
                                              "take at most 8 hypotheses (stage %d has %d)" % (stage_splits, s_ + 1, d_))
        self.arch_mode = arch_mode
        self.num_stage = num_stage
        self.depth_interals_ratio = list(depth_interals_ratio)
        self.group_cor = group_cor
        self.group_cor_dim = list(group_cor_dim)
        self.inverse_depth = inverse_depth
        self.stage_splits = list(stage_splits)
        self.mono = mono
        self.attn_temp = attn_temp
        self.attn_fuse_d = attn_fuse_d
        self.reg_net = reg_net
        self.feature = FPN4(base_channels=fpn_base_channel)
        self.attn_ob = nn.ModuleList()
        self.pos_enc_func = nn.ModuleList()
        self.reg = nn.ModuleList()
        if self.mono:
            self.mono_depth_decoder = mono_depth_decoder()
        down_size = [3, 3, 2, 2]
        for idx in range(num_stage):
            in_dim = self.group_cor_dim[idx] if group_cor else self.feature.out_channels[idx]
            if reg_net == "reg2d":
                self.reg.append(reg2d(input_channel=in_dim, base_channel=reg_channel, conv_name=agg_type))
            elif reg_net == "reg3d":
                self.reg.append(reg3d(in_channels=in_dim, base_channels=reg_channel, down_size=down_size[idx]))
            else:
                raise NotImplementedError("reg_net %r" % reg_net)
        self._plans = {}
        self.overlap_streams = True
        self.train_side_stages = (0, 1, 2)
        self.train_side_separate = False
        self.train_fpn_tail_stream = True
        self._side_streams = {}
        self.warp_variant = 0
        self.fuse_hypotheses = False
        self.merge_launches = True
        self.graph_cache = True
        from .graph import ForwardCache
        self._fwd_cache = ForwardCache()
        self.register_load_state_dict_post_hook(_invalidate_after_load)

    def __getstate__(self):
        from .graph import ForwardCache
        state = dict(self.__dict__)
        state["_plans"], state["_side_streams"], state["_fwd_cache"] = {}, {}, ForwardCache()
        return state

    def invalidate_plans(self):
        self._plans.clear()
        self._fwd_cache.clear()
        from . import train_ops
        train_ops.CACHE.clear()

    def train(self, mode=True):
        if mode != self.training:
            self._plans.clear()
        return super().train(mode)

    def _apply(self, fn, *args, **kwargs):
        self._plans.clear()
        self._fwd_cache.clear()
        return super()._apply(fn, *args, **kwargs)

    def _state_stamp(self):
        import itertools
        from . import train_ops
        cells = train_ops.CACHE.cells
        acc = train_ops.CACHE.stat_writes * 15485863
        for t in itertools.chain(self.feature.parameters(), self.feature.buffers(), self.reg.parameters(), self.reg.buffers()):
            acc = (acc * 1000003 + t._version * 7919 + t.data_ptr()) & 0xFFFFFFFFFFFF
            if cells:
                c = cells.get(t)
                if c is not None:
                    acc += c[0] * 104729
        return acc

    def _get_plans(self):
        dev = next(self.parameters()).device
        hit = self._plans.get(dev)
        stamp = hit[2] if hit is not None and torch.cuda.is_current_stream_capturing() else self._state_stamp()
        if hit is None or hit[2] != stamp:
            with torch.no_grad():
                fpn = FpnPlan(self.feature)
                regs = [Reg2dPlan(m) if isinstance(m, reg2d) else Reg3dPlan(m) for m in self.reg]
            hit = self._plans[dev] = (fpn, regs, stamp)
        return hit[0], hit[1]

    def _hypotheses(self, stage_idx, depth_values, depth_interval, prev, H, W):
        D = self.stage_splits[stage_idx]
        if stage_idx == 0:
            return ops.init_range(depth_values, D, H, W, inverse=self.inverse_depth)
        if self.inverse_depth:
            return ops.schedule_inverse_range(prev["inverse_min_depth"].detach(), prev["inverse_max_depth"].detach(), D,
                                              H, W)
        return ops.schedule_range(prev["depth"].detach(), D, self.depth_interals_ratio[stage_idx] * depth_interval, H, W)

    def _check_inputs(self, imgs, proj_matrices, depth_values):
        if len(imgs) == 0 or not torch.is_tensor(imgs[0]):
            raise RuntimeError("imgs: a non-empty list of [B,3,H,W] tensors expected")
        if imgs[0].dim() != 4 or imgs[0].shape[1] != 3:
            raise RuntimeError("imgs: a list of [B,3,H,W] tensors expected, got %s" % (tuple(imgs[0].shape),))
        B, _, H, W = imgs[0].shape
        if H % 64 or W % 64:
            raise RuntimeError("image size %dx%d: H and W must be multiples of 64 (stage-1 is H/8 and reg2d "
                               "halves three more times)" % (H, W))
        N = len(imgs)
        for i, im in enumerate(imgs):
            if tuple(im.shape) != (B, 3, H, W) or im.device != imgs[0].device or im.dtype != torch.float32:
                raise RuntimeError("imgs[%d]: %s %s on %s, expected [%d,3,%d,%d] float32 (the path is fp32-only, like the "
                                   "reference's) on %s" % (i, tuple(im.shape), im.dtype, im.device, B, H, W, imgs[0].device))
        for s in range(self.num_stage):
            name = "stage%d" % (s + 1)
            if name not in proj_matrices:
                raise RuntimeError("proj_matrices has no %r entry (keys: %s)" % (name, sorted(proj_matrices.keys())))
            pm = proj_matrices[name]
            if tuple(pm.shape) != (B, N, 2, 4, 4):
                raise RuntimeError("proj_matrices[%r]: shape %s, expected [%d,%d,2,4,4] (batch, views = len(imgs))"
                                   % (name, tuple(pm.shape), B, N))
            if not pm.dtype.is_floating_point:
                raise RuntimeError("proj_matrices[%r]: floating-point tensor expected, got %s" % (name, pm.dtype))
        if N < 2:
            raise RuntimeError("at least one source view is needed (len(imgs) = %d)" % N)
        if depth_values.dim() != 2 or depth_values.shape[0] != B or depth_values.shape[1] < 2:
            raise RuntimeError("depth_values: shape %s, expected [%d, D >= 2] (the range is read from its first and last "
                               "column)" % (tuple(depth_values.shape), B))
        if not imgs[0].is_cuda:
            raise RuntimeError("mvster_amd.MVS4net runs on MI355X only: move the model and inputs to the GPU "
                               "(there is no CPU fallback; the CPU oracle lives in oracle/ for tests)")

    @torch.no_grad()
    def _forward_eval(self, imgs, proj_matrices, depth_values, teacher=None, capture=None):
        N = len(imgs)
        B, _, H, W = imgs[0].shape
        dev = imgs[0].device
        fpn, regs = self._get_plans()
        depth_values = depth_values.to(dev, torch.float32)
        depth_interval = None
        if not self.inverse_depth:
            depth_interval = (depth_values[:, -1] - depth_values[:, 0]) / depth_values.size(1)
        names = ["stage%d" % (s + 1) for s in range(self.num_stage)]
        pms = [proj_matrices[n].to(dev, torch.float32) for n in names]
        hypo0 = None
        if self.merge_launches and (teacher is None or "stage1" not in teacher) and not self.fuse_hypotheses:
            packed, rts, hypo0 = ops.forward_prologue(imgs, pms, depth_values, self.stage_splits[0], H // 8, W // 8,
                                                      self.inverse_depth)
        else:
            packed, rts = ops.pack_images(imgs), ops.relative_projection_multi(pms)
        c0, c1, c3, f1 = fpn.trunk(packed)
        main = torch.cuda.current_stream()
        side = None
        if self.overlap_streams and self.num_stage > 2:
            side = self._side_streams.get(dev)
            if side is None:
                side = self._side_streams[dev] = torch.cuda.Stream(device=dev)
            side.wait_stream(main)
            with torch.cuda.stream(side):
                o3, o4 = fpn.tail(c0, c1, f1)
            o1, o2 = fpn.coarse(c3, f1)
        else:
            o1, o2 = fpn.coarse(c3, f1)
            o3, o4 = fpn.tail(c0, c1, f1) if self.num_stage > 2 else (None, None)
        join = None
        if side is not None:
            def join():
                main.wait_stream(side)
                if not torch.cuda.is_current_stream_capturing():
                    for t in (o3, o4):
                        t.record_stream(main)
        return self._cascade_eval([o1, o2, o3, o4], regs, N, B, H, W, rts, depth_values, depth_interval, hypo0=hypo0,
                                  teacher=teacher, capture=capture, join=join)

    @torch.no_grad()
    def _cascade_eval(self, pyramid, regs, N, B, H, W, rts, depth_values, depth_interval, hypo0=None, teacher=None,
                      capture=None, join=None, views=None, nsrc=None):
        outputs = {}
        prev = None
        for s in range(self.num_stage):
            name = "stage%d" % (s + 1)
            if s == 2 and join is not None:
                join()
            f = pyramid[s]
            if views is None:
                h, w, C = f.shape[2], f.shape[3], f.shape[4]
                f = f.view(N, B, h, w, C)
                ref_cl, src_cl = f[0], f[1:]
            else:
                h, w, C = f.shape[1], f.shape[2], f.shape[3]
                ref_cl = src_cl = None
            G = self.group_cor_dim[s] if self.group_cor else C
            rt = rts[s]
            cor = hypo = None
            if teacher is not None and name in teacher:
                hypo = teacher[name].contiguous()
            elif (views is None and nsrc is None and self.inverse_depth and self.group_cor and self.warp_variant == 0
                  and self.fuse_hypotheses):
                fused = ops.warp_agg_fwd_sched_cl(
                    ref_cl.contiguous(), src_cl.contiguous(), rt, G, self.stage_splits[s], self.attn_fuse_d, float(self.attn_temp),
                    inv_min=None if s == 0 else prev["inverse_min_depth"], inv_max=None if s == 0 else prev["inverse_max_depth"],
                    depth_values=depth_values.contiguous() if s == 0 else None)
                if fused is not None:
                    cor, hypo = fused
            if hypo is None and s == 0 and hypo0 is not None:
                hypo = hypo0
            if hypo is None:
                hypo = self._hypotheses(s, depth_values, depth_interval, prev, h, w)
            if cor is None and views is not None:
                cor = ops.warp_agg_fwd_indexed_cl(f, views, rt, hypo, G, self.group_cor, self.attn_fuse_d,
                                                  float(self.attn_temp), variant=self.warp_variant, nsrc=nsrc)
            elif cor is None:
                cor = ops.warp_agg_fwd_cl(ref_cl, src_cl, rt, hypo, G, self.group_cor, self.attn_fuse_d,
                                          float(self.attn_temp), variant=self.warp_variant, nsrc=nsrc)
            plan = regs[s]
            want_logits = capture is not None
            if isinstance(plan, Reg2dPlan):
                sel = plan.select(cor, hypo, self.depth_interals_ratio[s], self.inverse_depth, want_logits=want_logits)
            elif plan.fused_prob:
                sel = ops.select_depth(hypo, self.depth_interals_ratio[s], self.inverse_depth, feat_cl=plan(cor),
                                       prob_w=plan.prob_w, prob_b=plan.prob_b, want_logits=want_logits)
            else:
                sel = ops.select_depth(hypo, self.depth_interals_ratio[s], self.inverse_depth, logits=plan(cor),
                                       want_logits=want_logits)
            if capture is not None:
                capture[name] = {"cor_feats": cor.permute(0, 4, 1, 2, 3), "logits": sel["logits"]}
                if views is None:
                    capture[name]["feats_cl"] = f
            if s == 3 or self.merge_launches:
                conf = sel["conf"]
            else:
                conf = ops.upsample_bilinear(sel["conf"], 2 ** (3 - s))
            st = {"depth": sel["depth"], "photometric_confidence": conf, "hypo_depth": hypo,
                  "attn_weight": sel["attn_weight"]}
            if self.inverse_depth:
                st["inverse_min_depth"] = sel["inverse_min_depth"]
                st["inverse_max_depth"] = sel["inverse_max_depth"]
            if self.mono and views is None:
                st["mono_feat"] = ref_cl.permute(0, 3, 1, 2)
            prev = st
            outputs[name] = st
            outputs.update(st)
        if self.merge_launches:
            coarse = [outputs["stage%d" % (k + 1)] for k in range(min(3, self.num_stage))]
            ups = ops.upsample_bilinear_multi([st["photometric_confidence"] for st in coarse], H, W)
            for st, u in zip(coarse, ups):
                st["photometric_confidence"] = u
            if self.num_stage < 4:
                outputs["photometric_confidence"] = ups[-1]
        return outputs

    def _stage_outputs(self, s, logits, hypo, dev):
        attn = F.softmax(logits, dim=1)
        idx = attn.max(1, keepdim=True)[1]
        depth = torch.gather(hypo, 1, idx).squeeze(1)
        if self.training:
            conf = torch.zeros((), dtype=torch.float32, device=dev)
        else:
            with torch.no_grad():
                conf = ops.upsample_bilinear(attn.max(1)[0].contiguous(), 2 ** (3 - s))
        st = {"depth": depth, "photometric_confidence": conf, "hypo_depth": hypo, "attn_weight": attn}
        if self.inverse_depth:
            itv = 1.0 / hypo[:, 2] - 1.0 / hypo[:, 1]
            st["inverse_min_depth"] = 1 / depth + self.depth_interals_ratio[s] * itv
            st["inverse_max_depth"] = 1 / depth - self.depth_interals_ratio[s] * itv
        return st

    @staticmethod
    def _no_stream_warning():
        if not MVS4net._stream_warning_off:
            off = getattr(torch.autograd.graph, "set_warn_on_accumulate_grad_stream_mismatch", None)
            if off is not None:
                off(False)
            MVS4net._stream_warning_off = True

    def _train_stream(self, dev):
        from .train_ops import side_stream
        return side_stream(dev, avoid=[torch.cuda.current_stream(dev)] + list(self._side_streams.values()))

    def _forward_train(self, imgs, proj_matrices, depth_values, teacher=None):
        dev = imgs[0].device
        depth_values = depth_values.to(dev, torch.float32)
        depth_interval = (depth_values[:, -1] - depth_values[:, 0]) / depth_values.size(1)
        nv, B = len(imgs), imgs[0].shape[0]
        if any(img.requires_grad for img in imgs):
            x = torch.cat([img.permute(0, 2, 3, 1).unsqueeze(1) for img in imgs], 0)
        else:
            x = ops.pack_images([img.to(dev, torch.float32) for img in imgs])
        tail = None
        if self.train_fpn_tail_stream and x.is_cuda and isinstance(self.feature, FPN4) and self.num_stage >= 3:
            tail = self._side_streams.get(("fpn_tail", dev))
            if tail is None:
                tail = self._side_streams[("fpn_tail", dev)] = self._train_stream(dev)
            self._no_stream_warning()
        if isinstance(self.feature, FPN4):
            self.feature.tail_stream = tail
        pyramid = self.feature.forward_cl(x, groups=nv)
        tail = getattr(self.feature, "tail_pending", None)
        if isinstance(self.feature, FPN4):
            self.feature.tail_stream = self.feature.tail_pending = None
        outputs = {}
        prev = None
        ref_feats = []
        for s in range(self.num_stage):
            name = "stage%d" % (s + 1)
            if tail is not None and s >= 2:
                torch.cuda.current_stream(dev).wait_stream(tail)
                tail = None
            pyr = pyramid[name]
            _, _, h, w, C = pyr.shape
            G = self.group_cor_dim[s] if self.group_cor else C
            side = cur = None
            if s in self.train_side_stages and pyr.is_cuda:
                self._no_stream_warning()
                cur = torch.cuda.current_stream(dev)
                key = ("train", dev, s if self.train_side_separate else 0)
                side = self._side_streams.get(key)
                if side is None:
                    side = self._side_streams[key] = self._train_stream(dev)
                side.wait_stream(cur)
            with (torch.cuda.stream(side) if side is not None else contextlib.nullcontext()):
                with torch.no_grad():
                    rt = ops.relative_projection(proj_matrices[name].to(dev, torch.float32))
                    if teacher is not None and name in teacher:
                        hypo = teacher[name].detach().contiguous()
                    else:
                        hypo = self._hypotheses(s, depth_values, depth_interval, prev, h, w)
                cor, ref_maps = _WarpAggPyr.apply(pyr, B, rt, hypo, G, self.group_cor, self.attn_fuse_d, float(self.attn_temp))
                reg = self.reg[s]
                if isinstance(reg, reg2d) and self.training and self.stage_splits[s] >= (3 if self.inverse_depth else 1):
                    res = _SelectDepthCL.apply(reg.forward_cl(cor, return_features=True), reg.prob.weight, reg.prob.bias, hypo,
                                               float(self.depth_interals_ratio[s]), self.inverse_depth)
                    st = {"depth": res[1], "photometric_confidence": torch.zeros((), dtype=torch.float32, device=dev),
                          "hypo_depth": hypo, "attn_weight": res[0]}
                    if self.inverse_depth:
                        st["inverse_min_depth"], st["inverse_max_depth"] = res[2], res[3]
                else:
                    st = self._stage_outputs(s, reg.forward_cl(cor), hypo, dev)
            if side is not None:
                cur.wait_stream(side)
            if self.mono:
                st["mono_feat"] = ref_maps.reshape(B, h, w, C).permute(0, 3, 1, 2)
                ref_feats.append(ref_maps)
            prev = st
            outputs[name] = st
            outputs.update(st)
        if self.mono and self.training:
            outputs = self.mono_depth_decoder.forward_cl(outputs, ref_feats, depth_values[:, 0], depth_values[:, 1])
        return outputs

    def forward_eager(self, imgs, proj_matrices, depth_values):
        self._check_inputs(imgs, proj_matrices, depth_values)
        return self._forward_eval(imgs, proj_matrices, depth_values)

    def forward(self, imgs, proj_matrices, depth_values, filename=None):
        if self.training and max(self.stage_splits) > self.MAX_HYPOTHESES_TRAIN:
            raise NotImplementedError("training with stage_splits %r: the backward kernels (warp / aggregation, stage "
                                      "selection, Sinkhorn) hold at most %d hypotheses per pixel; evaluation takes up to %d"
                                      % (self.stage_splits, self.MAX_HYPOTHESES_TRAIN, self.MAX_HYPOTHESES))
        if self.training and min(self.stage_splits) < 3:
            raise NotImplementedError("training with stage_splits %r: the loss (mvster_amd.loss.stage_losses, as "
                                      "MVS4net_loss in the reference) needs at least 3 hypotheses per stage; evaluation "
                                      "with inverse_depth=False takes 2" % (self.stage_splits,))
        self._check_inputs(imgs, proj_matrices, depth_values)
        if self.training:
            return self._forward_train(imgs, proj_matrices, depth_values)
        if (not self.graph_cache or getattr(self, "_is_replica", False) or torch.cuda.is_current_stream_capturing()):
            return self._forward_eval(imgs, proj_matrices, depth_values)
        return self._fwd_cache(self, imgs, proj_matrices, depth_values)
```

Measured before the change: 1171 depth-maps/s.

## Fuse image packing and side jobs into conv0 pair, upsampling into final select

The first FPN conv pair now reads the planar input images straight from the per-view pointers, so the separate pack kernel goes away. Extra workgroups in the same launch compute the relative projections and the stage-1 depth hypotheses. The final-stage deconv+select kernel also gains rider workgroups that bilinearly upsample the three coarse confidence maps, which drops the separate multi-upsample launch. This removes launches and an intermediate packed buffer, at the cost of more complex kernels and extra per-launch argument marshalling.

```diff
diff --git a/include/mvster_hip.h b/include/mvster_hip.h
--- a/include/mvster_hip.h
+++ b/include/mvster_hip.h
@@ -106,6 +106,12 @@
                             const float* scale2, const float* shift2, float* out, int NB, int H, int W, int relu1, int relu2,
                             int wpc, void* stream);
 
+int mvster_conv_narrow_pair_planes(const float* const* imgs, int N, int B, int H, int W, const float* w1, const float* scale1,
+                                   const float* shift1, const float* w2, const float* scale2, const float* shift2, float* out,
+                                   int relu1, int relu2, int wpc, const float* const* proj_matrices, int nstage, float* rt,
+                                   const float* depth_values, int ndv, float* hypo, int D, int h, int w, int inverse,
+                                   void* stream);
+
 int mvster_deconv_small(const float* in, const float* w, const float* scale, const float* shift, const float* skip,
                         const float* prob_w, const float* prob_b, float* out, int NB, int Hi, int Wi, int cin,
                         int cout, int relu, void* stream);
@@ -114,6 +120,12 @@
                          const float* prob_w, const float* prob_b, const float* hypo, float* attn, float* depth, float* conf,
                          float* inv_min, float* inv_max, float* logits_out, int B, int D, int Hi, int Wi, int cin, int relu,
                          float split_itv, void* stream);
+
+int mvster_deconv_select_riders(const float* in, const float* w, const float* scale, const float* shift, const float* skip,
+                                const float* prob_w, const float* prob_b, const float* hypo, float* attn, float* depth,
+                                float* conf, float* inv_min, float* inv_max, float* logits_out, int B, int D, int Hi, int Wi,
+                                int cin, int relu, float split_itv, const float* const* up_ins, float* const* up_outs,
+                                const int* up_his, const int* up_wis, int n, int ho, int wo, void* stream);
 
 int mvster_fpn_tail_gather(const float* G, const float* vb, float* P, float* workspace, int NB, int H, int W,
                            int CO, void* stream);
diff --git a/mvster_amd/_lib.py b/mvster_amd/_lib.py
--- a/mvster_amd/_lib.py
+++ b/mvster_amd/_lib.py
@@ -41,7 +41,9 @@
     "mvster_conv_narrow": [_f, _f, _f, _f, _f, _f, _i, _i, _i, _i, _i, _i, _i, _f],
     "mvster_conv_narrow4": [_f, _f, _f, _f, _f, _i, _i, _i, _i, _i, _i, _f],
     "mvster_conv_narrow_pair": [_f, _f, _f, _f, _f, _f, _f, _f, _i, _i, _i, _i, _i, _i, _f],
+    "mvster_conv_narrow_pair_planes": [_f] + [_i] * 4 + [_f] * 7 + [_i] * 3 + [_f, _i, _f, _f, _i, _f] + [_i] * 4 + [_f],
     "mvster_deconv_select": [_f] * 14 + [_i] * 6 + [_fl, _f],
+    "mvster_deconv_select_riders": [_f] * 14 + [_i] * 6 + [_fl] + [_f] * 4 + [_i] * 3 + [_f],
     "mvster_deconv_small": [_f, _f, _f, _f, _f, _f, _f, _f, _i, _i, _i, _i, _i, _i, _f],
     "mvster_fpn_tail_gather": [_f, _f, _f, _f, _i, _i, _i, _i, _f],
     "mvster_fpn_lateral_up": [_f, _f, _f, _f, _f, _i, _i, _i, _i, _i, _f],
diff --git a/mvster_amd/conv_plan.py b/mvster_amd/conv_plan.py
--- a/mvster_amd/conv_plan.py
+++ b/mvster_amd/conv_plan.py
@@ -565,7 +565,10 @@
     return ConvLayer(ct.weight, True, ct.stride, ct.padding, bn=bn, relu=True, prob=prob)
 
 
-def fused_conv11_select(L, t, c0, hypo, split_itv, inverse_depth, want_logits=False):
+RIDER_DEPTHS = (4, 8)
+
+
+def fused_conv11_select(L, t, c0, hypo, split_itv, inverse_depth, want_logits=False, upsample=None, up_size=None):
     B, D, hi, wi, _ = t.shape
     dev = t.device
     hypo = hypo.contiguous()
@@ -575,13 +578,37 @@
     imin = torch.empty_like(depth) if inverse_depth else None
     imax = torch.empty_like(depth) if inverse_depth else None
     lo = torch.empty_like(attn) if want_logits else None
-    rc = _lib.load().mvster_deconv_select(
-        t.data_ptr(), L.w_deconv.data_ptr(), L.scale.data_ptr(), L.shift.data_ptr(), c0.data_ptr(),
-        L.prob[0].data_ptr(), L.prob[1].data_ptr(), hypo.data_ptr(), attn.data_ptr(), depth.data_ptr(), conf.data_ptr(),
-        None if imin is None else imin.data_ptr(), None if imax is None else imax.data_ptr(),
-        None if lo is None else lo.data_ptr(), B, D, hi, wi, L.cin, int(L.relu), float(split_itv), ops._stream())
+    args = (t.data_ptr(), L.w_deconv.data_ptr(), L.scale.data_ptr(), L.shift.data_ptr(), c0.data_ptr(),
+            L.prob[0].data_ptr(), L.prob[1].data_ptr(), hypo.data_ptr(), attn.data_ptr(), depth.data_ptr(), conf.data_ptr(),
+            None if imin is None else imin.data_ptr(), None if imax is None else imax.data_ptr(),
+            None if lo is None else lo.data_ptr(), B, D, hi, wi, L.cin, int(L.relu), float(split_itv))
+    ups = None
+    if upsample:
+        import ctypes
+        xs = [x.contiguous() for x in upsample]
+        H, W = up_size
+        n = len(xs)
+        for i, x in enumerate(xs):
+            if x.dim() != 3 or x.shape[0] != B or x.device != dev or x.dtype != torch.float32 or x.shape[1] < 1 or x.shape[2] < 1:
+                raise RuntimeError("fused_conv11_select: upsample[%d] is %s %s on %s, expected float32 [%d,h,w] on %s"
+                                   % (i, x.dtype, tuple(x.shape), x.device, B, dev))
+        if n > 3 or H < 1 or W < 1 or D not in RIDER_DEPTHS:
+            raise RuntimeError("fused_conv11_select: %d maps to %dx%d beside D = %d: at most 3 maps, D in %s"
+                               % (n, H, W, D, RIDER_DEPTHS))
+        ups = [torch.empty(B, H, W, device=dev, dtype=torch.float32) for _ in xs]
+        ip = (ctypes.c_void_p * n)(*[x.data_ptr() for x in xs])
+        op = (ctypes.c_void_p * n)(*[o.data_ptr() for o in ups])
+        hs = (ctypes.c_int * n)(*[x.shape[1] for x in xs])
+        ws = (ctypes.c_int * n)(*[x.shape[2] for x in xs])
+        rc = _lib.load().mvster_deconv_select_riders(*args, ctypes.cast(ip, ctypes.c_void_p), ctypes.cast(op, ctypes.c_void_p),
+                                                     ctypes.cast(hs, ctypes.c_void_p), ctypes.cast(ws, ctypes.c_void_p), n, H, W,
+                                                     ops._stream())
+    else:
+        rc = _lib.load().mvster_deconv_select(*args, ops._stream())
     _lib.check(rc, "deconv_select")
     out = {"attn_weight": attn, "depth": depth, "conf": conf}
+    if ups is not None:
+        out["upsampled"] = ups
     if inverse_depth:
         out["inverse_min_depth"], out["inverse_max_depth"] = imin, imax
     if want_logits:
@@ -614,7 +641,7 @@
         t = self.conv9(t, skip=c2, skip_mode=SKIP_ADD)
         return self.conv11(t, skip=c0, skip_mode=SKIP_ADD)
 
-    def select(self, x, hypo, split_itv, inverse_depth, want_logits=False):
+    def select(self, x, hypo, split_itv, inverse_depth, want_logits=False, upsample=None, up_size=None):
         c0 = self.conv0(x)
         c2 = self.conv2(self.conv1(c0))
         c4 = self.conv4(self.conv3(c2))
@@ -625,6 +652,8 @@
         B, D, hi, wi, _ = t.shape
         if (FUSE_SELECT and L.w_deconv is not None and L.prob is not None and L.cin == 16 and FORCE_VARIANT in (None, 4)
                 and 2 <= D <= 16 and t.is_contiguous() and c0.is_contiguous()):
+            if upsample and D in RIDER_DEPTHS and len(upsample) <= 3:
+                return fused_conv11_select(L, t, c0, hypo, split_itv, inverse_depth, want_logits, upsample=upsample, up_size=up_size)
             return fused_conv11_select(L, t, c0, hypo, split_itv, inverse_depth, want_logits)
         res = self.conv11(t, skip=c0, skip_mode=SKIP_ADD)
         if self.fused_prob:
@@ -718,8 +747,9 @@
             x = l(x)
         return x
 
-    def trunk(self, x):
-        c0 = self._conv0(x)
+    def trunk(self, x, c0=None):
+        if c0 is None:
+            c0 = self._conv0(x)
         c1 = self._seq(self.conv1, c0)
         c2 = self._seq(self.conv2, c1)
         c3 = self._seq(self.conv3, c2)
@@ -740,6 +770,52 @@
             return out
         return self._seq(self.conv0, x)
 
+    def conv0_planes(self, imgs, side=None):
+        import ctypes
+        a, b = self.conv0
+        x0 = imgs[0]
+        if not (FUSE_CONV0 and FORCE_VARIANT is None and a.w_small is not None and b.w_small is not None and a.cin == 4 and b.cin == 8
+                and 1 <= len(imgs) <= 8 and x0.dim() == 4 and x0.shape[1] == 3 and x0.is_cuda and a.w_small.device == x0.device
+                and hasattr(_lib.load(), "mvster_conv_narrow_pair_planes")):
+            return None
+        B, _, H, W = x0.shape
+        N = len(imgs)
+        if N * B * H * W < NARROW_PAIR_MIN_PIXELS:
+            return None
+        for im in imgs:
+            if im.shape != x0.shape or im.device != x0.device or im.dtype != torch.float32 or not im.is_contiguous():
+                return None
+        dev = x0.device
+        out = torch.empty((N * B, 1, H, W, 8), device=dev, dtype=torch.float32)
+        ip = (ctypes.c_void_p * N)(*[im.data_ptr() for im in imgs])
+        rt = hypo = pp = None
+        nstage = ndv = D = h = w = inverse = 0
+        if side is not None:
+            proj_list, dv, D, h, w, inverse = side
+            pms = [p.contiguous() for p in proj_list]
+            dv = dv.contiguous()
+            for k, pm in enumerate(pms):
+                if tuple(pm.shape) != (B, N, 2, 4, 4) or pm.device != dev or pm.dtype != torch.float32:
+                    raise RuntimeError("conv0_planes: proj_list[%d] is %s %s, expected float32 [%d,%d,2,4,4]"
+                                       % (k, pm.dtype, tuple(pm.shape), B, N))
+            if dv.dim() != 2 or dv.shape[0] != B or dv.shape[1] < 2 or dv.device != dev or dv.dtype != torch.float32:
+                raise RuntimeError("conv0_planes: depth_values is %s %s, expected float32 [%d, >= 2]" % (dv.dtype, tuple(dv.shape), B))
+            if N < 2 or not 1 <= len(pms) <= 8 or D < 2 or h < 1 or w < 1:
+                raise RuntimeError("conv0_planes: bad side jobs (%d views, %d stages, hypothesis volume %dx%dx%d)"
+                                   % (N, len(pms), D, h, w))
+            nstage, ndv = len(pms), dv.shape[1]
+            rt = torch.empty(nstage, B, N - 1, 12, device=dev, dtype=torch.float32)
+            hypo = torch.empty(B, D, h, w, device=dev, dtype=torch.float32)
+            pp = (ctypes.c_void_p * nstage)(*[p.data_ptr() for p in pms])
+        rc = _lib.load().mvster_conv_narrow_pair_planes(
+            ctypes.cast(ip, ctypes.c_void_p), N, B, H, W, a.w_small.data_ptr(), a.scale.data_ptr(), a.shift.data_ptr(),
+            b.w_small.data_ptr(), b.scale.data_ptr(), b.shift.data_ptr(), out.data_ptr(), int(a.relu), int(b.relu), NARROW_PAIR_WPC,
+            None if pp is None else ctypes.cast(pp, ctypes.c_void_p), nstage, None if rt is None else rt.data_ptr(),
+            None if side is None else dv.data_ptr(), ndv, None if hypo is None else hypo.data_ptr(), D, h, w, int(bool(inverse)),
+            ops._stream())
+        _lib.check(rc, "conv_narrow_pair_planes")
+        return out, rt, hypo
+
     def coarse(self, c3, f1):
         return self.out1(c3), self.out2(f1)
 
diff --git a/mvster_amd/csrc/conv_args.hpp b/mvster_amd/csrc/conv_args.hpp
--- a/mvster_amd/csrc/conv_args.hpp
+++ b/mvster_amd/csrc/conv_args.hpp
@@ -114,9 +114,17 @@
 int dispatch_b3(const ConvArgs& a, int mt, int wpc, hipStream_t s);
 int dispatch_1x1(const ConvArgs& a, int mt, int wpc, hipStream_t s);
 
+constexpr int UP_PPT = 4;
+struct UpRiders {
+    const float* in[3] = {nullptr, nullptr, nullptr};
+    float* out[3] = {nullptr, nullptr, nullptr};
+    int hi[3] = {0, 0, 0}, wi[3] = {0, 0, 0};
+    int n = 0, ho = 0, wo = 0;
+    unsigned per_map = 1, nwg = 0;
+};
 int dispatch_deconv_select_mfma(const float* in, const float* w, const float* scale, const float* shift, const float* skip,
                                 const float* prob_w, const float* prob_b, const float* hypo, float* attn, float* depth,
                                 float* conf, float* inv_min, float* inv_max, float* logits_out, int B, int D, int Hi, int Wi,
-                                int relu, float split_itv, hipStream_t s);
+                                int relu, float split_itv, const UpRiders* up, hipStream_t s);
 
 }
diff --git a/mvster_amd/csrc/conv_narrow.hip b/mvster_amd/csrc/conv_narrow.hip
--- a/mvster_amd/csrc/conv_narrow.hip
+++ b/mvster_amd/csrc/conv_narrow.hip
@@ -1,3 +1,5 @@
+#include <type_traits>
+
 #include "conv_args.hpp"
 
 namespace {
@@ -248,6 +250,40 @@
     FastDiv tiles_x, tiles_y;
 };
 
+struct NarrowPlanesArgs : NarrowPairArgs {
+    const float* img[8];
+    FastDiv bdiv;
+    unsigned img_bytes;
+    unsigned nside, nproj;
+    const float* pm[8];
+    float* rt;
+    const float* dv;
+    float* hypo;
+    int nstage, N, B, ndv, D, hw, inverse;
+};
+
+__device__ __forceinline__ void pair_side_jobs(const NarrowPlanesArgs& a, unsigned sb) {
+    if (sb < a.nproj) {
+        const int p = (int)(sb * 512 + threadIdx.x);
+        const int NV = a.N - 1;
+        const int per = a.B * NV;
+        if (p >= a.nstage * per) return;
+        const int s = p / per, r = p - s * per;
+        const int b = r / NV, v = r - b * NV;
+        mv::RT m;
+        mv::relative_projection(a.pm[s] + ((long)b * a.N) * 32, a.pm[s] + ((long)b * a.N + v + 1) * 32, m);
+        float* o = a.rt + (long)p * 12;
+        for (int k = 0; k < 9; ++k) o[k] = m.r[k];
+        for (int k = 0; k < 3; ++k) o[9 + k] = m.t[k];
+    } else {
+        const int p = (int)((sb - a.nproj) * 512 + threadIdx.x);
+        if (p >= a.hw) return;
+        for (int b = 0; b < a.B; ++b)
+            mv::init_range_pixel(a.dv[b * a.ndv], a.dv[b * a.ndv + a.ndv - 1], a.hypo + (long)b * a.D * a.hw, a.D, a.hw, p,
+                                 a.inverse);
+    }
+}
+
 struct PairGeom {
     static constexpr int TY = 14, TX = 64;
     static constexpr int MH = TY + 2, MW = TX + 2;
@@ -260,8 +296,8 @@
     static constexpr size_t LDS = (size_t)(R * STAGE + MID + 8) * 16;
 };
 
-template <int DBG>
-__global__ void __launch_bounds__(512, 4) conv_narrow_pair_kernel(NarrowPairArgs a) {
+template <int DBG, bool PLANES = false>
+__global__ void __launch_bounds__(512, 4) conv_narrow_pair_kernel(std::conditional_t<PLANES, NarrowPlanesArgs, NarrowPairArgs> a) {
     using G = PairGeom;
     constexpr int TY = G::TY, PW = G::PW, MW = G::MW, NIW = G::NIW;
     static_assert(G::MH == 16, "the extra pixel pairs of the mid tile's rows form exactly one 16-row MFMA unit");
@@ -274,8 +310,16 @@
     const int wave = wave8 & 3;
     const bool loader = wave8 >= 4;
     const int lm = lane & 15, lq = lane >> 4;
-    const unsigned nwg = gridDim.x;
-    unsigned tile = xcd_remap(blockIdx.x, nwg);
+    unsigned nwg = gridDim.x, bid = blockIdx.x;
+    if constexpr (PLANES) {
+        if (bid < a.nside) {
+            pair_side_jobs(a, bid);
+            return;
+        }
+        bid -= a.nside;
+        nwg -= a.nside;
+    }
+    unsigned tile = xcd_remap(bid, nwg);
     if (PAIR_DBG & 16) tile = a.ntiles;
 
     auto decode = [&](unsigned t, int& nb, int& y0, int& x0) {
@@ -285,7 +329,64 @@
         x0 = (int)txu * G::TX;
     };
 
-    if (loader) {
+    if constexpr (PLANES) {
+        if (loader) {
+            int dpos[NIW];
+            unsigned dpix[NIW];
+#pragma unroll
+            for (int n = 0; n < NIW; ++n) {
+                const int s = (wave + 4 * n) * 64 + lane;
+                const int prow = s / PW, pl = s - prow * PW;
+                dpos[n] = s < G::PSLOTS ? (pl | (prow << 8)) : -1;
+                dpix[n] = (unsigned)((prow * a.W + pl) * 4);
+            }
+            const unsigned plane = (unsigned)(a.H * a.W * 4);
+            unsigned px[NIW][3];
+            auto load_tile = [&](unsigned t) {
+                int nb, y0, x0;
+                decode(t, nb, y0, x0);
+                unsigned bu;
+                const unsigned v = __builtin_amdgcn_readfirstlane(fdivmod((unsigned)nb, a.bdiv, bu));
+                const __amdgpu_buffer_rsrc_t rsrc =
+                    __builtin_amdgcn_make_buffer_rsrc(const_cast<float*>(a.img[v]), (short)0, (int)a.img_bytes, 0x00020000);
+                const unsigned porigin = (unsigned)(((((int)bu * 3 * a.H + y0 - 2) * a.W) + x0 - 2) * 4);
+#pragma unroll
+                for (int n = 0; n < NIW; ++n) {
+                    const int ix = x0 + (dpos[n] & 255) - 2, iy = y0 + (dpos[n] >> 8) - 2;
+                    const bool ok = dpos[n] >= 0 && (unsigned)iy < (unsigned)a.H && (unsigned)ix < (unsigned)a.W && !(PAIR_DBG & 8);
+                    const unsigned off = ok ? dpix[n] + porigin : 0x80000000u;
+#pragma unroll
+                    for (int c = 0; c < 3; ++c) {
+                        const int offc = (int)(off + (unsigned)c * plane);
+                        px[n][c] = __builtin_amdgcn_raw_buffer_load_b32(rsrc, offc, 0, 0);
+                    }
+                }
+            };
+            auto write_tile = [&](int stage) {
+                f32x4v* const dst0 = lds + stage * G::STAGE;
+#pragma unroll
+                for (int n = 0; n < NIW; ++n)
+                    dst0[(wave + 4 * n) * 64 + lane] = (f32x4v){__builtin_bit_cast(float, px[n][0]), __builtin_bit_cast(float, px[n][1]),
+                                                                __builtin_bit_cast(float, px[n][2]), 0.0f};
+            };
+            if (tile < a.ntiles) {
+                load_tile(tile);
+                write_tile(0);
+            }
+            if (tile + nwg < a.ntiles) load_tile(tile + nwg);
+            __builtin_amdgcn_s_waitcnt(0xc07f);
+            int st = 1;
+            for (; tile < a.ntiles; tile += nwg) {
+                __builtin_amdgcn_s_barrier();
+                if (tile + nwg < a.ntiles) write_tile(st);
+                st ^= 1;
+                if (tile + 2u * nwg < a.ntiles) load_tile(tile + 2u * nwg);
+                __builtin_amdgcn_s_waitcnt(0xc07f);
+                __builtin_amdgcn_s_barrier();
+            }
+            return;
+        }
+    } else if (loader) {
         const __amdgpu_buffer_rsrc_t in_rsrc =
             __builtin_amdgcn_make_buffer_rsrc(const_cast<float*>(a.in), (short)0, (int)a.in_bytes, 0x00020000);
         unsigned dbase[NIW];
@@ -528,23 +629,8 @@
     }
 }
 
-int launch_narrow_pair(NarrowPairArgs& a, int wpc, hipStream_t s) {
+int pair_grid(NarrowPairArgs& a, int wpc, long& gx) {
     using G = PairGeom;
-    auto kern = conv_narrow_pair_kernel<0>;
-    int slot = 0;
-#ifdef MVSTER_PROBES
-    switch (a.dbg) {
-#define PAIR_CASE(n, m) case m: kern = conv_narrow_pair_kernel<m>; slot = n; break;
-        PAIR_CASE(1, 1) PAIR_CASE(2, 2) PAIR_CASE(3, 3) PAIR_CASE(4, 4) PAIR_CASE(5, 8) PAIR_CASE(6, 12) PAIR_CASE(7, 15)
-        PAIR_CASE(8, 16) PAIR_CASE(9, 32) PAIR_CASE(10, 35) PAIR_CASE(11, 47) PAIR_CASE(12, 44)
-#undef PAIR_CASE
-        case 0: break;
-        default: return MVSTER_ERR_UNSUPPORTED;
-    }
-#endif
-    static unsigned long attr_done_all[13] = {0};
-    unsigned long& attr_done = attr_done_all[slot];
-    if (G::LDS > 64 * 1024 && !mvconv::allow_big_lds(reinterpret_cast<const void*>(kern), attr_done)) return MVSTER_ERR_LAUNCH;
     const int ncu = mvconv::num_cus();
     if (ncu <= 0) return MVSTER_ERR_LAUNCH;
     const unsigned tx = (unsigned)((a.W + G::TX - 1) / G::TX), ty = (unsigned)((a.H + G::TY - 1) / G::TY);
@@ -560,9 +646,43 @@
     if (per_cu < 1) per_cu = 1;
     const long gmax = (long)ncu * per_cu;
     const long rounds = (ntiles + gmax - 1) / gmax;
-    const long gx = (ntiles + rounds - 1) / rounds;
+    gx = (ntiles + rounds - 1) / rounds;
+    return MVSTER_OK;
+}
+
+int launch_narrow_pair(NarrowPairArgs& a, int wpc, hipStream_t s) {
+    using G = PairGeom;
+    auto kern = conv_narrow_pair_kernel<0>;
+    int slot = 0;
+#ifdef MVSTER_PROBES
+    switch (a.dbg) {
+#define PAIR_CASE(n, m) case m: kern = conv_narrow_pair_kernel<m>; slot = n; break;
+        PAIR_CASE(1, 1) PAIR_CASE(2, 2) PAIR_CASE(3, 3) PAIR_CASE(4, 4) PAIR_CASE(5, 8) PAIR_CASE(6, 12) PAIR_CASE(7, 15)
+        PAIR_CASE(8, 16) PAIR_CASE(9, 32) PAIR_CASE(10, 35) PAIR_CASE(11, 47) PAIR_CASE(12, 44)
+#undef PAIR_CASE
+        case 0: break;
+        default: return MVSTER_ERR_UNSUPPORTED;
+    }
+#endif
+    static unsigned long attr_done_all[13] = {0};
+    unsigned long& attr_done = attr_done_all[slot];
+    if (G::LDS > 64 * 1024 && !mvconv::allow_big_lds(reinterpret_cast<const void*>(kern), attr_done)) return MVSTER_ERR_LAUNCH;
+    long gx;
+    if (const int rc = pair_grid(a, wpc, gx)) return rc;
     MV_NOTE_KERNEL("conv_narrow_pair_kernel");
     hipLaunchKernelGGL(kern, dim3((unsigned)gx), dim3(512), G::LDS, s, a);
+    return mv_check_launch();
+}
+
+int launch_narrow_pair_planes(NarrowPlanesArgs& a, int wpc, hipStream_t s) {
+    using G = PairGeom;
+    auto kern = conv_narrow_pair_kernel<0, true>;
+    static unsigned long attr_done = 0;
+    if (G::LDS > 64 * 1024 && !mvconv::allow_big_lds(reinterpret_cast<const void*>(kern), attr_done)) return MVSTER_ERR_LAUNCH;
+    long gx;
+    if (const int rc = pair_grid(a, wpc, gx)) return rc;
+    MV_NOTE_KERNEL("conv_narrow_pair_kernel<0, true>");
+    hipLaunchKernelGGL(kern, dim3((unsigned)(gx + a.nside)), dim3(512), G::LDS, s, a);
     return mv_check_launch();
 }
 
@@ -623,3 +743,43 @@
     a.dbg = wpc >> 4;
     return launch_narrow_pair(a, wpc & 15, (hipStream_t)stream);
 }
+
+extern "C" int mvster_conv_narrow_pair_planes(const float* const* imgs, int N, int B, int H, int W, const float* w1,
+                                              const float* scale1, const float* shift1, const float* w2, const float* scale2,
+                                              const float* shift2, float* out, int relu1, int relu2, int wpc,
+                                              const float* const* proj_matrices, int nstage, float* rt,
+                                              const float* depth_values, int ndv, float* hypo, int D, int h, int w, int inverse,
+                                              void* stream) {
+    if (!imgs || !w1 || !scale1 || !shift1 || !w2 || !scale2 || !shift2 || !out) return MVSTER_ERR_NULL;
+    if (N < 1 || N > 8 || B <= 0 || H <= 0 || W <= 0) return MVSTER_ERR_SHAPE;
+    const long img_bytes = (long)B * 3 * H * W * 4, out_bytes = (long)N * B * H * W * 32;
+    if (img_bytes >= (1L << 31) || out_bytes >= (1L << 31)) return MVSTER_ERR_SHAPE;
+    NarrowPlanesArgs a;
+    for (int v = 0; v < 8; ++v) {
+        if (v < N && !imgs[v]) return MVSTER_ERR_NULL;
+        if (v < N && ((uintptr_t)imgs[v] & 3)) return MVSTER_ERR_SHAPE;
+        a.img[v] = imgs[v < N ? v : 0];
+    }
+    a.in = nullptr; a.w1 = w1; a.scale1 = scale1; a.shift1 = shift1; a.w2 = w2; a.scale2 = scale2; a.shift2 = shift2; a.out = out;
+    a.NB = N * B; a.H = H; a.W = W; a.relu1 = relu1; a.relu2 = relu2; a.dbg = 0;
+    a.in_bytes = 0; a.out_bytes = (unsigned)out_bytes;
+    a.bdiv = mv_fastdiv((unsigned)B); a.img_bytes = (unsigned)img_bytes;
+    a.nside = a.nproj = 0;
+    for (int s = 0; s < 8; ++s) a.pm[s] = nullptr;
+    a.rt = nullptr; a.dv = nullptr; a.hypo = nullptr;
+    a.nstage = 0; a.N = N; a.B = B; a.ndv = 0; a.D = 0; a.hw = 0; a.inverse = 0;
+    if (proj_matrices) {
+        if (!rt || !depth_values || !hypo) return MVSTER_ERR_NULL;
+        if (N < 2 || nstage < 1 || nstage > 8 || D < 2 || h <= 0 || w <= 0 || ndv < 1 || (long)h * w >= (1L << 30))
+            return MVSTER_ERR_SHAPE;
+        for (int s = 0; s < nstage; ++s) {
+            if (!proj_matrices[s]) return MVSTER_ERR_NULL;
+            a.pm[s] = proj_matrices[s];
+        }
+        a.rt = rt; a.dv = depth_values; a.hypo = hypo;
+        a.nstage = nstage; a.ndv = ndv; a.D = D; a.hw = h * w; a.inverse = inverse;
+        a.nproj = (unsigned)(((long)nstage * B * (N - 1) + 511) / 512);
+        a.nside = a.nproj + (unsigned)((a.hw + 511) / 512);
+    }
+    return launch_narrow_pair_planes(a, wpc & 15, (hipStream_t)stream);
+}
diff --git a/mvster_amd/csrc/conv_small.hip b/mvster_amd/csrc/conv_small.hip
--- a/mvster_amd/csrc/conv_small.hip
+++ b/mvster_amd/csrc/conv_small.hip
@@ -305,10 +305,10 @@
     return mv_check_launch();
 }
 
-extern "C" int mvster_deconv_select(const float* in, const float* w, const float* scale, const float* shift, const float* skip,
-                                    const float* prob_w, const float* prob_b, const float* hypo, float* attn, float* depth,
-                                    float* conf, float* inv_min, float* inv_max, float* logits_out, int B, int D, int Hi,
-                                    int Wi, int cin, int relu, float split_itv, void* stream) {
+static int deconv_select_impl(const float* in, const float* w, const float* scale, const float* shift, const float* skip,
+                              const float* prob_w, const float* prob_b, const float* hypo, float* attn, float* depth,
+                              float* conf, float* inv_min, float* inv_max, float* logits_out, int B, int D, int Hi, int Wi,
+                              int cin, int relu, float split_itv, const mvconv::UpRiders* up, void* stream) {
     if (!in || !w || !scale || !shift || !prob_w || !prob_b || !hypo || !attn || !depth) return MVSTER_ERR_NULL;
     if ((inv_min == nullptr) != (inv_max == nullptr)) return MVSTER_ERR_NULL;
     if (B <= 0 || D < 2 || D > mv::kSelMaxD || Hi <= 0 || Wi <= 0 || (inv_min && D < 3)) return MVSTER_ERR_SHAPE;
@@ -317,8 +317,8 @@
     if (in_elems >= (1L << 30) || (long)B * D * Hi * Wi * 4 * 8 >= (1L << 31)) return MVSTER_ERR_SHAPE;
     {
         const int rc = mvconv::dispatch_deconv_select_mfma(in, w, scale, shift, skip, prob_w, prob_b, hypo, attn, depth, conf, inv_min,
-                                                           inv_max, logits_out, B, D, Hi, Wi, relu, split_itv, (hipStream_t)stream);
-        if (rc != MVSTER_ERR_UNSUPPORTED) return rc;
+                                                           inv_max, logits_out, B, D, Hi, Wi, relu, split_itv, up, (hipStream_t)stream);
+        if (rc != MVSTER_ERR_UNSUPPORTED || up) return rc;
     }
     DeconvArgs a;
     a.in = in; a.w = w; a.scale = scale; a.shift = shift; a.skip = skip; a.prob_w = prob_w; a.prob_b = prob_b;
@@ -330,3 +330,30 @@
     hipLaunchKernelGGL(deconv_select_kernel<16>, dim3((Hi * Wi + 63) / 64, B), dim3(64, D), 0, (hipStream_t)stream, a, so);
     return mv_check_launch();
 }
+
+extern "C" int mvster_deconv_select(const float* in, const float* w, const float* scale, const float* shift, const float* skip,
+                                    const float* prob_w, const float* prob_b, const float* hypo, float* attn, float* depth,
+                                    float* conf, float* inv_min, float* inv_max, float* logits_out, int B, int D, int Hi,
+                                    int Wi, int cin, int relu, float split_itv, void* stream) {
+    return deconv_select_impl(in, w, scale, shift, skip, prob_w, prob_b, hypo, attn, depth, conf, inv_min, inv_max, logits_out, B, D,
+                              Hi, Wi, cin, relu, split_itv, nullptr, stream);
+}
+
+extern "C" int mvster_deconv_select_riders(const float* in, const float* w, const float* scale, const float* shift,
+                                           const float* skip, const float* prob_w, const float* prob_b, const float* hypo,
+                                           float* attn, float* depth, float* conf, float* inv_min, float* inv_max,
+                                           float* logits_out, int B, int D, int Hi, int Wi, int cin, int relu, float split_itv,
+                                           const float* const* up_ins, float* const* up_outs, const int* up_his,
+                                           const int* up_wis, int n, int ho, int wo, void* stream) {
+    if (!up_ins || !up_outs || !up_his || !up_wis) return MVSTER_ERR_NULL;
+    if (n < 1 || n > 3 || ho <= 0 || wo <= 0 || B <= 0 || (long)B * ho * wo >= (1L << 31)) return MVSTER_ERR_SHAPE;
+    mvconv::UpRiders up;
+    for (int k = 0; k < n; ++k) {
+        if (!up_ins[k] || !up_outs[k]) return MVSTER_ERR_NULL;
+        if (up_his[k] <= 0 || up_wis[k] <= 0) return MVSTER_ERR_SHAPE;
+        up.in[k] = up_ins[k]; up.out[k] = up_outs[k]; up.hi[k] = up_his[k]; up.wi[k] = up_wis[k];
+    }
+    up.n = n; up.ho = ho; up.wo = wo;
+    return deconv_select_impl(in, w, scale, shift, skip, prob_w, prob_b, hypo, attn, depth, conf, inv_min, inv_max, logits_out, B, D,
+                              Hi, Wi, cin, relu, split_itv, &up, stream);
+}
diff --git a/mvster_amd/csrc/deconv_select.hip b/mvster_amd/csrc/deconv_select.hip
--- a/mvster_amd/csrc/deconv_select.hip
+++ b/mvster_amd/csrc/deconv_select.hip
@@ -13,6 +13,7 @@
     float split_itv;
     unsigned in_bytes, skip_bytes, ntiles;
     FastDiv tiles_x, tiles_y;
+    mvconv::UpRiders up;
 };
 
 template <int D, int RI, int R>
@@ -45,7 +46,19 @@
     const bool loader = wave8 >= 4;
     const int lm = lane & 15, lq = lane >> 4;
     const int Ho = 2 * a.Hi, Wo = 2 * a.Wi;
-    const unsigned nwg = gridDim.x;
+    const unsigned nwg = gridDim.x - a.up.nwg;
+    if (blockIdx.x >= nwg) {
+        const int npix = a.up.ho * a.up.wo;
+        const unsigned r = blockIdx.x - nwg, k = r / a.up.per_map, c = r - k * a.up.per_map;
+#pragma unroll
+        for (int i = 0; i < mvconv::UP_PPT; ++i) {
+            const long q = ((long)c * mvconv::UP_PPT + i) * 512 + threadIdx.x;
+            if (q >= (long)a.B * npix) break;
+            const int b = (int)(q / npix), p = (int)(q - (long)b * npix);
+            a.up.out[k][q] = mv::upsample_pixel(a.up.in[k] + (long)b * a.up.hi[k] * a.up.wi[k], a.up.hi[k], a.up.wi[k], a.up.ho, a.up.wo, p);
+        }
+        return;
+    }
     unsigned tile = xcd_remap(blockIdx.x, nwg);
 
     auto decode = [&](unsigned t, int& b, int& i0, int& j0) {
@@ -237,8 +250,12 @@
     const long gmax = (long)ncu * per_cu;
     const long rounds = (ntiles + gmax - 1) / gmax;
     const long gx = (ntiles + rounds - 1) / rounds;
+    if (a.up.n > 0) {
+        a.up.per_map = (unsigned)(((long)a.B * a.up.ho * a.up.wo + 512 * mvconv::UP_PPT - 1) / (512 * mvconv::UP_PPT));
+        a.up.nwg = a.up.per_map * (unsigned)a.up.n;
+    }
     MV_NOTE_KERNEL("deconv_select_mfma_kernel<%d, %d, %d>", D, RI, R);
-    hipLaunchKernelGGL(kern, dim3((unsigned)gx), dim3(512), G::LDS, s, a);
+    hipLaunchKernelGGL(kern, dim3((unsigned)gx + a.up.nwg), dim3(512), G::LDS, s, a);
     return mv_check_launch();
 }
 
@@ -249,7 +266,7 @@
 int dispatch_deconv_select_mfma(const float* in, const float* w, const float* scale, const float* shift, const float* skip,
                                 const float* prob_w, const float* prob_b, const float* hypo, float* attn, float* depth,
                                 float* conf, float* inv_min, float* inv_max, float* logits_out, int B, int D, int Hi, int Wi,
-                                int relu, float split_itv, hipStream_t s) {
+                                int relu, float split_itv, const UpRiders* up, hipStream_t s) {
     const long in_bytes = (long)B * D * Hi * Wi * 64, skip_bytes = (long)B * D * Hi * Wi * 4 * 32;
     if (in_bytes >= (1L << 31) || skip_bytes >= (1L << 31)) return MVSTER_ERR_UNSUPPORTED;
     DselArgs a;
@@ -257,6 +274,9 @@
     a.attn = attn; a.depth = depth; a.conf = conf; a.inv_min = inv_min; a.inv_max = inv_max; a.logits_out = logits_out;
     a.B = B; a.Hi = Hi; a.Wi = Wi; a.relu = relu; a.split_itv = split_itv;
     a.in_bytes = (unsigned)in_bytes; a.skip_bytes = (unsigned)skip_bytes;
+    a.up = UpRiders();
+    if (up) a.up = *up;
+    a.up.nwg = 0;
     const int ncu = num_cus();
     if (D == 4) {
         const long t4 = (long)((Wi + 15) / 16) * ((Hi + 3) / 4) * B;
diff --git a/mvster_amd/net.py b/mvster_amd/net.py
--- a/mvster_amd/net.py
+++ b/mvster_amd/net.py
@@ -241,13 +241,17 @@
             depth_interval = (depth_values[:, -1] - depth_values[:, 0]) / depth_values.size(1)
         names = ["stage%d" % (s + 1) for s in range(self.num_stage)]
         pms = [proj_matrices[n].to(dev, torch.float32) for n in names]
-        hypo0 = None
+        hypo0 = packed = c0 = None
         if self.merge_launches and (teacher is None or "stage1" not in teacher) and not self.fuse_hypotheses:
-            packed, rts, hypo0 = ops.forward_prologue(imgs, pms, depth_values, self.stage_splits[0], H // 8, W // 8,
-                                                      self.inverse_depth)
+            jobs = (pms, depth_values, self.stage_splits[0], H // 8, W // 8, self.inverse_depth)
+            fused = fpn.conv0_planes(imgs, jobs)
+            if fused is not None:
+                c0, rts, hypo0 = fused
+            else:
+                packed, rts, hypo0 = ops.forward_prologue(imgs, *jobs)
         else:
             packed, rts = ops.pack_images(imgs), ops.relative_projection_multi(pms)
-        c0, c1, c3, f1 = fpn.trunk(packed)
+        c0, c1, c3, f1 = fpn.trunk(packed, c0=c0)
         main = torch.cuda.current_stream()
         side = None
         if self.overlap_streams and self.num_stage > 2:
@@ -276,6 +280,7 @@
                       capture=None, join=None, views=None, nsrc=None):
         outputs = {}
         prev = None
+        ups = None
         for s in range(self.num_stage):
             name = "stage%d" % (s + 1)
             if s == 2 and join is not None:
@@ -314,7 +319,12 @@
             plan = regs[s]
             want_logits = capture is not None
             if isinstance(plan, Reg2dPlan):
-                sel = plan.select(cor, hypo, self.depth_interals_ratio[s], self.inverse_depth, want_logits=want_logits)
+                riders = None
+                if self.merge_launches and s == 3 and s == self.num_stage - 1:
+                    riders = [outputs["stage%d" % (k + 1)]["photometric_confidence"] for k in range(3)]
+                sel = plan.select(cor, hypo, self.depth_interals_ratio[s], self.inverse_depth, want_logits=want_logits,
+                                  upsample=riders, up_size=(H, W))
+                ups = sel.get("upsampled", ups)
             elif plan.fused_prob:
                 sel = ops.select_depth(hypo, self.depth_interals_ratio[s], self.inverse_depth, feat_cl=plan(cor),
                                        prob_w=plan.prob_w, prob_b=plan.prob_b, want_logits=want_logits)
@@ -341,7 +351,8 @@
             outputs.update(st)
         if self.merge_launches:
             coarse = [outputs["stage%d" % (k + 1)] for k in range(min(3, self.num_stage))]
-            ups = ops.upsample_bilinear_multi([st["photometric_confidence"] for st in coarse], H, W)
+            if ups is None:
+                ups = ops.upsample_bilinear_multi([st["photometric_confidence"] for st in coarse], H, W)
             for st, u in zip(coarse, ups):
                 st["photometric_confidence"] = u
             if self.num_stage < 4:
```

Result: faster. 1184 depth-maps/s (median of 6 runs) (+1.1%).
